# zrc0622/HIRL4UCAV

Hardware: AMD Instinct MI355X
Metric: env steps/sec (whole node) + HIRL update steps/sec at 4096 envs/GPU (higher is better)
Workload: dtype f32

## Files before the change

hirl4ucav_amd/_lib.py:

```python
import ctypes
import os

_HERE = os.path.dirname(os.path.abspath(__file__))
SO_PATH = os.environ.get("HX_LIBRARY") or os.path.join(_HERE, "libhx_mi355.so")

ENV_WORDS, OBS_DIM, ACT_DIM, ROW_WORDS = 37, 13, 4, 32
STAT_NAMES = ("episodes", "kills", "fire_success_episodes", "time_limit", "fires", "good_fires", "locked_steps", "env_steps", "nonfinite_actions")
STAT_WAYS, STAT_PITCH = 32, 16

F_LOCKED_PREV, F_LOCKED, F_SLOT_PREV, F_SLOT, F_FIRED, F_FIRE_SUCCESS, F_EPISODE_SUCCESS, F_DONE = (1 << i for i in range(8))
F_SCEN_SHIFT = 8
F_SERP_POS, F_SERP_LONG, F_M_ACTIVE, F_M_GUIDED, F_SIM_SLOT = (1 << i for i in range(10, 15))

_vp, _i32, _i64, _u32, _u64, _f32 = ctypes.c_void_p, ctypes.c_int32, ctypes.c_int64, ctypes.c_uint32, ctypes.c_uint64, ctypes.c_float


class HxStepOpts(ctypes.Structure):
    _fields_ = [("max_step", _i32), ("auto_reset", _i32), ("randomize", _i32), ("env_id0", _u32), ("seed", _u64),
                ("episode_ctr", _vp), ("ring", _vp), ("ring_success", _vp), ("cap", _i64), ("total", _vp), ("stats", _vp),
                ("ev_start", _vp), ("ev_stop", _vp), ("layout", _i32)]


LAYOUT_ORDERED_SLOTS = 1 << 16


def layout(pair, envs_per_block):
    return ((1 if pair else 0) << 8) | (int(envs_per_block) // 4)


class HxError(RuntimeError):
    pass


_SIGNATURES = {
    "hx_env_reset": [_vp, _i64, _i64, _vp, _vp, _i32, _i32, _u64, _u32, _vp, _vp, _vp],
    "hx_env_step": [_vp, _i64, _i64, _vp, _vp, _vp, _vp, _vp, ctypes.POINTER(HxStepOpts), _vp],
    "hx_env_rearm": [_vp, _i64, _i64, _vp, _vp],
    "hx_label_transitions": [_vp, _vp, _vp, _i64, _vp, _vp, _vp, _vp],
    "hx_event_destroy": [_vp],
    "hx_event_elapsed_us": [_vp, _vp, ctypes.POINTER(ctypes.c_float)],
}

_lib = None
ABI_VERSION = 117
_ABI_STRUCTS = {}


def check_struct(index, cls):
    sizes = (ctypes.c_int32 * 8)()
    L = load()
    L.hx_abi_sizes.argtypes = [ctypes.POINTER(ctypes.c_int32)]
    if L.hx_abi_sizes(sizes) != 0 or sizes[index] != ctypes.sizeof(cls):
        raise HxError(f"ABI mismatch: {cls.__name__} is {ctypes.sizeof(cls)} bytes here, {sizes[index]} in {SO_PATH}")
    if sizes[7] != STAT_WAYS * STAT_PITCH:
        raise HxError(f"ABI mismatch: a statistics buffer is {STAT_WAYS * STAT_PITCH} words here, {sizes[7]} in {SO_PATH}")


def load():
    global _lib
    if _lib is not None:
        return _lib
    if not os.path.exists(SO_PATH):
        raise HxError(f"{SO_PATH} not found: the HIP extension is not built (run __graft_entry__.build() or "
                      f"`make -C hirl4ucav_amd/csrc`). There is no CPU fallback.")
    import torch

    L = ctypes.CDLL(SO_PATH)
    L.hx_last_error.restype = ctypes.c_char_p
    L.hx_version.restype = ctypes.c_int
    if L.hx_version() != ABI_VERSION:
        raise HxError(f"{SO_PATH} implements ABI version {L.hx_version()}, this binding was written for {ABI_VERSION} (include/hirl4ucav.h "
                      f"HX_ABI_VERSION): rebuild the library (make -C hirl4ucav_amd/csrc)")
    L.hx_event_create.restype = ctypes.c_void_p
    L.hx_event_create.argtypes = []
    for name, args in _SIGNATURES.items():
        fn = getattr(L, name)
        fn.argtypes = args
        fn.restype = ctypes.c_int
    _lib = L
    return L


def register(name, argtypes):
    _SIGNATURES[name] = argtypes
    if _lib is not None:
        fn = getattr(_lib, name)
        fn.argtypes = argtypes
        fn.restype = ctypes.c_int


def call(name, *args):
    L = load()
    rc = getattr(L, name)(*args)
    if rc != 0:
        raise HxError(f"{name} failed ({rc}): {L.hx_last_error().decode()}")


def ptr(t):
    return None if t is None else t.data_ptr()


def stream_ptr():
    import torch

    return torch.cuda.current_stream().cuda_stream
```

hirl4ucav_amd/agents/engine.py:

```python
import ctypes
import os

import numpy as np
import torch

from .. import _lib

H1, H2 = 256, 512
_vp, _i32, _f32 = ctypes.c_void_p, ctypes.c_int32, ctypes.c_float


class HxBatch(ctypes.Structure):
    _fields_ = [("rows", _vp), ("bc_rows", _vp), ("batch", _i32), ("noise", _vp)]


class HxSample(ctypes.Structure):
    _fields_ = [("total", _vp), ("cap", ctypes.c_int64), ("ring", _vp), ("expert_ring", _vp), ("expert_len", ctypes.c_int64),
                ("bc_table", _vp), ("bc_len", ctypes.c_int64), ("n_main", _i32), ("seed", ctypes.c_uint64), ("call", ctypes.c_uint32),
                ("sigma", _f32), ("idx", _vp), ("idx_bc", _vp), ("guard", ctypes.c_uint32)]


class HxFront(ctypes.Structure):
    _fields_ = [("flags", _vp), ("status", _vp), ("epoch", ctypes.c_uint32), ("with_c", ctypes.c_uint32)]


class HxNets(ctypes.Structure):
    _fields_ = [(k, _vp) for k in ("actor", "critic", "target_actor", "target_critic", "bc_actor", "grad_actor", "grad_critic",
                                   "m_actor", "v_actor", "m_critic", "v_critic", "losses", "soft_count", "wstate", "ws", "actor_w2_bf16", "actor_w2_f32i",
                                   "w2_bf16_all", "xchg_status", "actor_w2_x9")]


class HxHyper(ctypes.Structure):
    _fields_ = [(k, _f32) for k in ("gamma", "tau", "lr_actor", "lr_critic", "slope", "noise_clamp", "loss_lambda")] + [("use_bc", _i32), ("no_layernorm", _i32)]


_P = ctypes.POINTER
_lib.register("hx_actor_act", [_vp, _vp, ctypes.c_int64, _vp, _i32, _vp, _f32, ctypes.c_uint64, ctypes.c_uint32, ctypes.c_uint32, _f32, _vp, _vp])
_lib.register("hx_actor_act_step", [_vp, _vp, ctypes.c_int64, ctypes.c_int64, _vp, _vp, _i32, _vp, _f32, ctypes.c_uint64, ctypes.c_uint32,
                                     ctypes.c_uint32, _f32, _vp, _vp, _vp, _P(_lib.HxStepOpts), _vp])
_lib.register("hx_pack_w2_bf16", [_vp, _i32, _vp, _vp])
_lib.register("hx_pack_w2_f32i", [_vp, _i32, _vp, _vp])
_lib.register("hx_pack_update_images", [_P(HxNets), _vp])
_lib.register("hx_pack_w2_x9", [_vp, _i32, _vp, _vp])
_lib.register("hx_actor_act_x9", [_vp, _vp, _vp, ctypes.c_int64, _vp, _i32, _vp, _f32, ctypes.c_uint64, ctypes.c_uint32, ctypes.c_uint32, _f32, _vp])
_lib.register("hx_actor_act_step_x9", [_vp, _vp, _vp, ctypes.c_int64, ctypes.c_int64, _vp, _vp, _i32, _vp, _f32, ctypes.c_uint64, ctypes.c_uint32,
                                        ctypes.c_uint32, _f32, _vp, _vp, _vp, _P(_lib.HxStepOpts), _vp])
_lib.register("hx_actor_act_f32i", [_vp, _vp, _vp, ctypes.c_int64, _vp, _i32, _vp, _f32, ctypes.c_uint64, ctypes.c_uint32, ctypes.c_uint32, _f32, _vp])
_lib.register("hx_actor_act_step_f32i", [_vp, _vp, _vp, ctypes.c_int64, ctypes.c_int64, _vp, _vp, _i32, _vp, _f32, ctypes.c_uint64, ctypes.c_uint32,
                                          ctypes.c_uint32, _f32, _vp, _vp, _vp, _P(_lib.HxStepOpts), _vp])
_lib.register("hx_actor_act_bf16", [_vp, _vp, _vp, ctypes.c_int64, _vp, _i32, _vp, _f32, ctypes.c_uint64, ctypes.c_uint32, ctypes.c_uint32, _f32, _vp])
_lib.register("hx_actor_act_step_bf16", [_vp, _vp, _vp, ctypes.c_int64, ctypes.c_int64, _vp, _vp, _i32, _vp, _f32, ctypes.c_uint64, ctypes.c_uint32,
                                          ctypes.c_uint32, _f32, _vp, _vp, _vp, _P(_lib.HxStepOpts), _vp])
_lib.register("hx_hirl_critic_grads", [_P(HxNets), _P(HxBatch), _P(HxHyper), _i32, _vp])
_lib.register("hx_hirl_actor_backward", [_P(HxNets), _P(HxBatch), _P(HxHyper), _i32, _i32, _vp])
_lib.register("hx_hirl_actor_wgrad", [_P(HxNets), _P(HxHyper), _i32, _i32, _i32, _f32, _f32, _vp])
_lib.register("hx_adam", [_P(HxNets), _P(HxHyper), _i32, _i32, _f32, _i32, _f32, _f32, _i32, _vp])
_lib.register("hx_polyak", [_P(HxNets), _P(HxHyper), _vp])
_lib.register("hx_hirl_actor_wgrad_split", [_P(HxNets), _P(HxHyper), _i32, _vp, _vp])
_lib.register("hx_adam_mixed", [_P(HxNets), _P(HxHyper), _i32, _i32, _f32, _i32, _f32, _f32, _i32, _vp, _vp])
from .exchange import OneShotExchange, RcclDirect, _DeviceWords, negotiate_rccl_direct


_lib.register("hx_bc_train_actor", [_P(HxNets), _P(HxBatch), _P(HxHyper), _i32, _vp])
_lib.register("hx_hirl_learn", [_P(HxNets), _P(HxBatch), _P(HxHyper), _i32, _i32, _i32, _i32, _i32, _f32, _f32, _vp])
_lib.register("hx_hirl_learn_sampled", [_P(HxNets), _P(HxBatch), _P(HxHyper), _P(HxSample), _i32, _i32, _i32, _i32, _i32, _f32, _f32, _vp])
_lib.register("hx_hirl_front", [_vp, ctypes.c_int64, ctypes.c_int64, _vp, _vp, _i32, _vp, _f32, ctypes.c_uint64, ctypes.c_uint32, ctypes.c_uint32, _vp, _vp, _vp,
                                 _P(_lib.HxStepOpts), _P(HxNets), _P(HxBatch), _P(HxHyper), _i32, _i32, _P(HxFront), _vp])
_lib.register("hx_hirl_learn_back", [_P(HxNets), _P(HxBatch), _P(HxHyper), _i32, _i32, _i32, _i32, _i32, _f32, _f32, _P(HxSample), _P(HxBatch), _i32, _vp])
_lib.register("hx_hirl_critic_grads_back", [_P(HxNets), _P(HxBatch), _P(HxHyper), _P(HxSample), _P(HxBatch), _i32, _vp])
_lib.register("hx_sample_batch_guarded", [_vp, ctypes.c_int64, _vp, _vp, ctypes.c_int64, _vp, ctypes.c_int64, _i32, _i32, _i32, ctypes.c_uint64,
                                           ctypes.c_uint32, _f32, _vp, _vp, _vp, _vp, _vp, ctypes.c_uint32, _vp])
_lib.register("hx_hirl_critic_grads_sampled", [_P(HxNets), _P(HxBatch), _P(HxHyper), _P(HxSample), _i32, _vp])
_lib.register("hx_sample_batch", [_vp, ctypes.c_int64, _vp, _vp, ctypes.c_int64, _vp, ctypes.c_int64, _i32, _i32, _i32, ctypes.c_uint64,
                                   ctypes.c_uint32, _f32, _vp, _vp, _vp, _vp, _vp, _vp])



def _block_layout(in_dim, out_dim, names):
    fa, la, fb, lb, fin = names
    shapes = [(fa + ".weight", (H1, in_dim)), (fa + ".bias", (H1,)), (la + ".weight", (H1,)), (la + ".bias", (H1,)),
              (fb + ".weight", (H2, H1)), (fb + ".bias", (H2,)), (lb + ".weight", (H2,)), (lb + ".bias", (H2,)),
              (fin + ".weight", (out_dim, H2)), (fin + ".bias", (out_dim,))]
    out, off = [], 0
    for k, shp in shapes:
        out.append((k, off, shp))
        off += int(np.prod(shp))
    return out, off


ACTOR_LAYOUT, ACTOR_SIZE = _block_layout(13, 4, ("full1", "layernorm1", "full2", "layernorm2", "final"))
_q1, _qsize = _block_layout(17, 1, ("full1", "layernorm1", "full2", "layernorm2", "final1"))
_q2, _ = _block_layout(17, 1, ("full3", "layernorm3", "full4", "layernorm4", "final2"))
Q_PADDED = (_qsize + 3) & ~3
CRITIC_LAYOUT = _q1 + [(k, off + Q_PADDED, shp) for k, off, shp in _q2]
CRITIC_SIZE = 2 * Q_PADDED


def pack(params, layout, size, device):
    flat = torch.zeros(size, dtype=torch.float32, device=device)
    for k, off, shp in layout:
        v = torch.as_tensor(np.asarray(params[k].detach().cpu() if torch.is_tensor(params[k]) else params[k]), dtype=torch.float32)
        assert tuple(v.shape) == tuple(shp), (k, v.shape, shp)
        flat[off:off + v.numel()] = v.reshape(-1).to(device)
    return flat


def unpack(flat, layout):
    return {k: flat[off:off + int(np.prod(shp))].reshape(shp) for k, off, shp in layout}


def force_plain_layernorm(flat, layout):
    for k, off, shp in layout:
        if k.startswith("layernorm"):
            flat[off:off + int(np.prod(shp))] = 1.0 if k.endswith(".weight") else 0.0


def len_of(replay):
    return 0 if replay is None else int(getattr(replay, "fixed_len", replay.capacity))


def carve(sizes, device):
    offs, tot = [], 0
    for n in sizes:
        offs.append(tot)
        tot += (n + 63) & ~63
    arena = torch.zeros(tot, dtype=torch.float32, device=device)
    return arena, [arena[o:o + n] for o, n in zip(offs, sizes)]


def _noise_mode(noise, sigma):
    if noise is not None:
        return 1 if noise.numel() == 4 else 2
    return 3 if sigma > 0 else 0


def _bc_weight_kind(bc_weight_now):
    if bc_weight_now is None:
        return 2, 0.0
    if bc_weight_now == 100:
        return 1, 0.0
    return 0, float(bc_weight_now)


class HirlEngine:
    def __init__(self, batch=128, lr_actor=1e-3, lr_critic=1e-3, tau=0.005, gamma=0.99, slope=0.0, use_bc=True,
                 device="cuda", group=None, layer_norm=True):
        self.device = torch.device(device)
        if self.device.type != "cuda":
            raise _lib.HxError("HirlEngine runs on the GPU only (no CPU path in the product)")
        L = _lib.load()
        for i, cls in ((0, _lib.HxStepOpts), (1, HxNets), (2, HxHyper), (3, HxBatch), (4, HxSample)):
            _lib.check_struct(i, cls)
        assert L.hx_actor_param_count() == ACTOR_SIZE and L.hx_critic_param_count() == CRITIC_SIZE
        L.hx_hirl_workspace_floats.restype = ctypes.c_int64
        self.batch = int(batch)
        ws_floats = int(L.hx_hirl_workspace_floats(self.batch))
        self.arena, views = carve([ACTOR_SIZE] * 3 + [CRITIC_SIZE] * 2 + [CRITIC_SIZE + ACTOR_SIZE] + [ACTOR_SIZE] * 2 + [CRITIC_SIZE] * 2 +
                                  [64, 64, 64, ws_floats, self.batch * 32, self.batch * 32, self.batch, self.batch, 64], self.device)
        (self.actor, self.target_actor, self.bc_actor, self.critic, self.target_critic, self.grad, self.m_actor, self.v_actor,
         self.m_critic, self.v_critic, self.losses, sc, self.wstate, self.ws, self.rows, self.bc_rows, ix, ixb, self._noise) = views
        self.grad_critic, self.grad_actor = self.grad[:CRITIC_SIZE], self.grad[CRITIC_SIZE:]
        self.soft_count, self._idx, self._idx_bc = sc.view(torch.int32), ix.view(torch.int32), ixb.view(torch.int32)
        self.losses, self.wstate, self._noise = self.losses[:8], self.wstate[:1], self._noise[:4]
        self.soft_count = self.soft_count[:1]
        self.sample_calls = 0
        self._pending = None
        self.front_c = False
        self._front = None
        self._front_enqueued = False
        self.needs_reload = False
        self._front_epoch = 0
        self._front_c_epoch = 0
        self._front_tiles = None
        self._front_drawn = None
        self.nets = HxNets(*(t.data_ptr() for t in (self.actor, self.critic, self.target_actor, self.target_critic, self.bc_actor,
                                                     self.grad_actor, self.grad_critic, self.m_actor, self.v_actor, self.m_critic,
                                                     self.v_critic, self.losses, self.soft_count, self.wstate, self.ws)), None, None, None, None, None)
        self.act_dtype, self.w2_bf16, self.w2_x9, self._x9_live = "f32", None, None, False
        self.x9_rows = 4096
        self.front_x9 = True
        self.update_dtype, self.images = "f32", None
        self.w2_f32i = torch.zeros(H2 * H1, dtype=torch.float32, device=self.device)
        self.nets.actor_w2_f32i = self.w2_f32i.data_ptr()
        self.layer_norm = bool(layer_norm)
        self._mode_bits = 0 if self.layer_norm else 16
        self.hyper = HxHyper(gamma, tau, lr_actor, lr_critic, slope, 0.5, 10000.0, int(use_bc), 0 if self.layer_norm else 1)
        self.use_bc, self.slope = bool(use_bc), float(slope)
        self.actor_trainable, self.update_count = True, 0
        self.critic_step, self.actor_step = 0, 0
        self.target_update_freq = 3
        self.group = group
        self.world = torch.distributed.get_world_size(group) if (torch.distributed.is_available() and torch.distributed.is_initialized()) else 1
        self.act_calls = 0
        self.staged = self.world > 1
        self.actor_msg = torch.zeros(int(L.hx_actor_message_floats()), dtype=torch.float32, device=self.device) if self.world > 1 else None
        self.sharded_sequence = False
        self.exchange_name, self.xchg, self.rccl = "rccl", None, None

    def load_params(self, actor, critic, bc_actor=None, hard_update_targets=True):
        self.actor.copy_(pack(actor, ACTOR_LAYOUT, ACTOR_SIZE, self.device))
        self.critic.copy_(pack(critic, CRITIC_LAYOUT, CRITIC_SIZE, self.device))
        if bc_actor is not None:
            self.bc_actor.copy_(pack(bc_actor, ACTOR_LAYOUT, ACTOR_SIZE, self.device))
        if not self.layer_norm:
            for flat, layout in ((self.actor, ACTOR_LAYOUT), (self.critic, CRITIC_LAYOUT), (self.bc_actor, ACTOR_LAYOUT)):
                force_plain_layernorm(flat, layout)
        if hard_update_targets:
            self.target_actor.copy_(self.actor)
            self.target_critic.copy_(self.critic)
        self.refresh_bf16()

    def set_act_dtype(self, dtype):
        if dtype not in ("f32", "bf16", "f32x9"):
            raise ValueError(dtype)
        if dtype == "f32x9" and self.update_dtype != "f32":
            raise ValueError("act dtype f32x9 goes with the fp32 update path")
        self.act_dtype = dtype
        self._bind_images()
        self.refresh_bf16()

    def set_update_dtype(self, dtype):
        if dtype not in ("f32", "bf16"):
            raise ValueError(dtype)
        if dtype == "bf16" and self.act_dtype == "f32x9":
            raise ValueError("act dtype f32x9 goes with the fp32 update path")
        self.update_dtype = dtype
        self._bind_images()
        self.refresh_bf16()

    def _bind_images(self):
        self.nets.actor_w2_x9 = None
        self._x9_live = False
        if self.update_dtype == "bf16":
            if self.images is None:
                L = _lib.load()
                L.hx_bf16_images_elems.restype = ctypes.c_int64
                self.images = torch.zeros(int(L.hx_bf16_images_elems()), dtype=torch.bfloat16, device=self.device)
            self.nets.w2_bf16_all = self.images.data_ptr()
            self.w2_bf16 = self.images[:H2 * H1]
            self.nets.actor_w2_bf16 = self.w2_bf16.data_ptr() if self.act_dtype == "bf16" else None
            return
        self.nets.w2_bf16_all = None
        if self.act_dtype == "f32x9":
            if self.w2_x9 is None:
                self.w2_x9 = torch.zeros(3 * H2 * H1, dtype=torch.bfloat16, device=self.device)
            self.nets.actor_w2_x9 = self.w2_x9.data_ptr()
            self.nets.actor_w2_bf16 = None
            return
        if self.act_dtype == "bf16":
            if self.w2_bf16 is None or (self.images is not None and self.w2_bf16.data_ptr() == self.images.data_ptr()):
                self.w2_bf16 = torch.zeros(H2 * H1, dtype=torch.bfloat16, device=self.device)
            self.nets.actor_w2_bf16 = self.w2_bf16.data_ptr()
        else:
            self.nets.actor_w2_bf16 = None

    def refresh_bf16(self):
        _lib.call("hx_pack_w2_f32i", self.actor.data_ptr(), 13, self.w2_f32i.data_ptr(), _lib.stream_ptr())
        if self.update_dtype == "bf16":
            _lib.call("hx_pack_update_images", ctypes.byref(self.nets), _lib.stream_ptr())
        elif self.act_dtype == "bf16":
            _lib.call("hx_pack_w2_bf16", self.actor.data_ptr(), 13, self.w2_bf16.data_ptr(), _lib.stream_ptr())
        elif self.act_dtype == "f32x9" or (self.act_dtype == "f32" and self._x9_live):
            _lib.call("hx_pack_w2_x9", self.actor.data_ptr(), 13, self.w2_x9.data_ptr(), _lib.stream_ptr())

    def _x9_for(self, n, front=False):
        if self.act_dtype == "f32x9":
            return True
        if self.act_dtype != "f32" or self.update_dtype != "f32":
            return False
        if not (front and self.front_x9) and (self.x9_rows is None or n < self.x9_rows):
            return False
        if not self._x9_live:
            if self.w2_x9 is None:
                self.w2_x9 = torch.zeros(3 * H2 * H1, dtype=torch.bfloat16, device=self.device)
            self.nets.actor_w2_x9 = self.w2_x9.data_ptr()
            _lib.call("hx_pack_w2_x9", self.actor.data_ptr(), 13, self.w2_x9.data_ptr(), _lib.stream_ptr())
            self._x9_live = True
        return True

    def _act_format(self, n):
        if self.act_dtype == "bf16":
            return "_bf16", self.w2_bf16.data_ptr()
        if self._x9_for(n):
            return "_x9", self.w2_x9.data_ptr()
        return "_f32i", self.w2_f32i.data_ptr()

    refresh_images = refresh_bf16

    def acting_format(self):
        return {"act_dtype": self.act_dtype, "update_dtype": self.update_dtype, "x9_rows": self.x9_rows, "front_x9": bool(self.front_x9), "x9_terms": 6}

    def replica_checksum(self):
        if self.xchg is not None:
            self.xchg.check()
        t = torch.cat([self.actor, self.target_actor, self.critic, self.target_critic, self.m_actor, self.v_actor, self.m_critic, self.v_critic])
        return int(t.view(torch.int32).to(torch.int64).sum().item())

    def close(self):
        if self.rccl is not None:
            r, self.rccl = self.rccl, None
            r.close()
        if self.xchg is not None:
            x, self.xchg = self.xchg, None
            self.nets.xchg_status = None
            try:
                x.check()
            finally:
                x.close()

    def state_dicts(self):
        return {"actor": unpack(self.actor, ACTOR_LAYOUT), "critic": unpack(self.critic, CRITIC_LAYOUT),
                "targetActor": unpack(self.target_actor, ACTOR_LAYOUT), "targetCritic": unpack(self.target_critic, CRITIC_LAYOUT),
                "bc_actor": unpack(self.bc_actor, ACTOR_LAYOUT)}

    def act(self, obs, noise=None, sigma=0.0, seed=0, row0=0, out=None, net=None):
        n = obs.shape[0]
        if out is None:
            out = torch.empty((n, 4), dtype=torch.float32, device=self.device)
        mode = _noise_mode(noise, sigma) | self._mode_bits
        self.act_calls += 1
        if net is None:
            fmt, image = self._act_format(n)
            _lib.call("hx_actor_act" + fmt, self.actor.data_ptr(), image, obs.data_ptr(), n, out.data_ptr(), mode, _lib.ptr(noise), float(sigma), int(seed),
                      int(row0), self.act_calls, self.slope, _lib.stream_ptr())
            return out
        _lib.call("hx_actor_act", net.data_ptr(), obs.data_ptr(), n, out.data_ptr(), mode, _lib.ptr(noise), float(sigma), int(seed), int(row0), self.act_calls,
                  self.slope, None, _lib.stream_ptr())
        return out

    def act_step(self, env, noise=None, sigma=0.0, seed=0, out=None):
        n = env.n
        if out is None:
            out = torch.empty((n, 4), dtype=torch.float32, device=self.device)
        mode = _noise_mode(noise, sigma) | self._mode_bits
        self.act_calls += 1
        env.steps_issued += 1
        fmt, image = self._act_format(n)
        _lib.call("hx_actor_act_step" + fmt, self.actor.data_ptr(), image, env.state.data_ptr(), n, env.pitch, env.obs.data_ptr(), out.data_ptr(), mode,
                  _lib.ptr(noise), float(sigma), int(seed), int(env.env_id0), self.act_calls, self.slope, env.reward.data_ptr(), env.done.data_ptr(),
                  env.success.data_ptr(), ctypes.byref(env._opts), _lib.stream_ptr())
        return out, env.obs, env.reward, env.done, env.success

    def use_oneshot_exchange(self, timeout_ms=5000, two_stage=False, bf16=False):
        if self.world <= 1:
            return
        self.xchg = OneShotExchange({"critic": CRITIC_SIZE, "actor": self.actor_msg.numel()}, self.device, self.group, timeout_ms, two_stage, bf16)
        self.nets.xchg_status = self.xchg.status_ptr
        self.exchange_name = "oneshot" if not two_stage else ("twostage-bf16" if bf16 else "twostage")

    def use_rccl_direct(self, bf16=False):
        dist = torch.distributed
        if not (dist.is_available() and dist.is_initialized()):
            raise _lib.HxError("use_rccl_direct needs an initialised torch.distributed process group (it carries the communicator id)")
        import sys

        def connect(uid, world, rank):
            r = RcclDirect(uid, world, rank, bf16=bf16)
            r.probe(self.device)
            return r

        r, _why = negotiate_rccl_direct(self.group, self.device if dist.get_backend(self.group) == "nccl" else "cpu", connect=connect,
                                        log=lambda m: print(m, file=sys.stderr, flush=True))
        if r is None:
            return False
        self.rccl = r
        self.exchange_name = "rccl-direct-bf16" if bf16 else "rccl-direct"
        return True

    def _allreduce(self, t, kind=None):
        if self.world <= 1 and not (self.sharded_sequence and torch.distributed.is_available() and torch.distributed.is_initialized()):
            return t
        if self.xchg is not None and kind is not None:
            return self.xchg.allreduce(kind)
        if self.rccl is not None:
            return self.rccl.allreduce(t)
        torch.distributed.all_reduce(t, group=self.group)
        return t

    def assemble(self, ring, idx, expert_ring=None, n_main=None, bc_table=None, idx_bc=None):
        B = self.batch
        n_main = B if n_main is None else int(n_main)
        _lib.call("hx_sample_batch", None, 0, ring.data_ptr(), _lib.ptr(expert_ring), 0, _lib.ptr(bc_table), 0, B, n_main, 0, 0, 0, 0.0,
                  idx.data_ptr(), _lib.ptr(idx_bc), None, self.rows.data_ptr(), self.bc_rows.data_ptr() if bc_table is not None else None,
                  _lib.stream_ptr())

    def sample(self, replay, expert=None, bc_table=None, n_main=None, seed=0, sigma=0.2, defer=False):
        B = self.batch
        self.sample_calls += 1
        if defer:
            self._pending = (HxSample(replay.total.data_ptr(), replay.capacity, replay.ring.data_ptr(),
                                      expert.ring.data_ptr() if expert is not None else None, len_of(expert), _lib.ptr(bc_table),
                                      bc_table.shape[0] if bc_table is not None else 0, B if n_main is None else int(n_main), int(seed),
                                      self.sample_calls, float(sigma), self._idx.data_ptr(),
                                      self._idx_bc.data_ptr() if bc_table is not None else None), replay, expert, bc_table)
            return self._idx, self._idx_bc, self._noise
        self._pending = None
        _lib.call("hx_sample_batch", replay.total.data_ptr(), replay.capacity, replay.ring.data_ptr(),
                  expert.ring.data_ptr() if expert is not None else None, len_of(expert), _lib.ptr(bc_table),
                  bc_table.shape[0] if bc_table is not None else 0, B, B if n_main is None else int(n_main), 1, int(seed),
                  self.sample_calls, float(sigma), self._idx.data_ptr(), self._idx_bc.data_ptr() if bc_table is not None else None,
                  self._noise.data_ptr(), self.rows.data_ptr(), self.bc_rows.data_ptr() if bc_table is not None else None, _lib.stream_ptr())
        return self._idx, self._idx_bc, self._noise

    def learn(self, noise=None, bc_weight_now=0.0, bc_warm_up_weight=0.0, before_exchange=None):
        B = self.batch
        if self.needs_reload:
            raise _lib.HxError("this engine failed after a front launch had been enqueued: load a snapshot before learn()")
        st = _lib.stream_ptr()
        pending, self._pending = self._pending, None
        pipe = getattr(before_exchange, "__self__", None) if before_exchange is not None else None
        if pending is not None and pipe is not None and (getattr(pipe, "_armed", None) is not None or getattr(pipe, "issued", False)):
            raise _lib.HxError("sample(defer=True) cannot be combined with an armed VectorStepPipeline: use sample(defer=False) when the "
                               "next env step may run beside learn()")
        if pending is not None and noise is not None:
            raise _lib.HxError("learn(noise=...) after sample(defer=True): the deferred draw produces the smoothing noise itself")
        noise = self._noise if noise is None else noise
        batch = HxBatch(self.rows.data_ptr(), self.bc_rows.data_ptr() if self.use_bc else None, B, noise.data_ptr())
        smp = ctypes.byref(pending[0]) if pending is not None else None
        nets, hyper = ctypes.byref(self.nets), ctypes.byref(self.hyper)
        w_kind, w_given = _bc_weight_kind(bc_weight_now)
        actor_phase = self.actor_trainable
        self.critic_step += 1
        if actor_phase:
            self.actor_step += 1
            self.update_count += 1
        do_polyak = actor_phase and self.update_count % self.target_update_freq == 0
        if not self.staged:
            _lib.call("hx_hirl_learn_sampled", nets, ctypes.byref(batch), hyper, smp, self.critic_step, int(actor_phase), self.actor_step,
                      int(do_polyak), w_kind, w_given, float(bc_warm_up_weight), st)
        else:
            actor_fwd = (2 if w_kind == 1 else 1) if actor_phase else 0
            if smp is not None:
                grads = lambda: _lib.call("hx_hirl_critic_grads_sampled", nets, ctypes.byref(batch), hyper, smp, actor_fwd, st)
            else:
                grads = lambda: _lib.call("hx_hirl_critic_grads", nets, ctypes.byref(batch), hyper, actor_fwd, st)
            self._learn_staged(grads, batch, actor_phase, do_polyak, w_kind, w_given, bc_warm_up_weight, before_exchange)
        self.actor_trainable = not self.actor_trainable

    def _learn_staged(self, critic_grads, batch, actor_phase, do_polyak, w_kind, w_given, bc_warm_up_weight, before_exchange=None):
        B, st = self.batch, _lib.stream_ptr()
        nets, hyper = ctypes.byref(self.nets), ctypes.byref(self.hyper)
        gs = 1.0 / self.world
        own_critic = self.grad_critic.data_ptr()
        if self.xchg is not None:
            self.nets.grad_critic = self.xchg.write_buffer("critic").data_ptr()
        critic_grads()
        if before_exchange is not None:
            before_exchange()
        summed = self._allreduce(self.grad_critic, "critic")
        self.nets.grad_critic = summed.data_ptr()
        pk = 16 if do_polyak else 0
        _lib.call("hx_adam", nets, hyper, 0 | pk, self.critic_step, gs, 0, 0.0, 0.0, B, st)
        self.nets.grad_critic = own_critic
        if actor_phase:
            _lib.call("hx_hirl_actor_backward", nets, ctypes.byref(batch), hyper, int(w_kind == 1), 1, st)
            if self.world > 1 or self.sharded_sequence:
                if self.actor_msg is None:
                    self.actor_msg = torch.zeros(int(_lib.load().hx_actor_message_floats()), dtype=torch.float32, device=self.device)
                msg = self.xchg.write_buffer("actor") if self.xchg is not None else self.actor_msg
                _lib.call("hx_hirl_actor_wgrad_split", nets, hyper, B, msg.data_ptr(), st)
                summed = self._allreduce(msg, "actor")
                _lib.call("hx_adam_mixed", nets, hyper, int(do_polyak), self.actor_step, gs, w_kind, w_given, float(bc_warm_up_weight),
                          B * self.world, summed.data_ptr(), st)
            else:
                _lib.call("hx_hirl_actor_wgrad", nets, hyper, B, B, w_kind, w_given, float(bc_warm_up_weight), st)
                _lib.call("hx_adam", nets, hyper, 1 | pk, self.actor_step, gs, w_kind, w_given, float(bc_warm_up_weight), B, st)

    def step_learn(self, env, expert=None, bc_table=None, n_main=None, act_noise=None, act_sigma=0.0, act_seed=0, out=None, sample_seed=0,
                   smooth_sigma=0.2, bc_weight_now=0.0, bc_warm_up_weight=0.0):
        replay, n, B = env.replay, env.n, self.batch
        bf16 = self.update_dtype == "bf16"
        if replay is None or (self.act_dtype != "bf16" if bf16 else self.act_dtype not in ("f32", "f32x9")):
            raise _lib.HxError("step_learn: the front launch exists for the fp32 networks (acting format 'f32' or 'f32x9') and for the bf16 update path with "
                               "the bf16 acting format, with a replay ring attached to the env")
        if self._pending is not None:
            raise _lib.HxError("step_learn draws its own minibatch: a sample(defer=True) is still pending")
        if self._front is None:
            buf = torch.zeros(96, dtype=torch.int32, device=self.device)
            self._front = (buf[0:64], buf[64:65])
            second = torch.zeros(2 * B * 32 + 2 * B + 64, dtype=torch.float32, device=self.device)
            t2 = (second[:B * 32], second[B * 32:2 * B * 32], second[2 * B * 32:2 * B * 32 + B].view(torch.int32),
                  second[2 * B * 32 + B:2 * B * 32 + 2 * B].view(torch.int32), second[2 * B * 32 + 2 * B:2 * B * 32 + 2 * B + 4])
            self._front_tiles = [(self.rows, self.bc_rows, self._idx, self._idx_bc, self._noise), t2]
        flags, status = self._front
        cur, nxt = self._front_tiles
        n_main = B if n_main is None else int(n_main)
        if self.needs_reload:
            raise _lib.HxError("this engine failed after a front launch had been enqueued (host and device state may disagree): load a snapshot "
                               "(utils/checkpoint.load_run) before stepping it again")
        held = (self._front_epoch, self._front_c_epoch, self.critic_step, self.actor_step, self.update_count, self.sample_calls, self.act_calls, env.steps_issued)
        self._front_enqueued = False
        try:
            return self._step_learn(env, expert, bc_table, n_main, act_noise, act_sigma, act_seed, out, sample_seed, smooth_sigma, bc_weight_now,
                                    bc_warm_up_weight, bf16, flags, status, cur, nxt)
        except _lib.HxError:
            if self._front_enqueued:
                self.needs_reload = True
                raise
            (self._front_epoch, self._front_c_epoch, self.critic_step, self.actor_step, self.update_count, self.sample_calls, self.act_calls, env.steps_issued) = held
            self.front_reset()
            raise

    def _step_learn(self, env, expert, bc_table, n_main, act_noise, act_sigma, act_seed, out, sample_seed, smooth_sigma, bc_weight_now, bc_warm_up_weight,
                    bf16, flags, status, cur, nxt):
        replay, n, B = env.replay, env.n, self.batch
        self.sample_calls += 1

        def draw(tiles, call):
            return HxSample(replay.total.data_ptr(), replay.capacity, replay.ring.data_ptr(), expert.ring.data_ptr() if expert is not None else None,
                            len_of(expert), _lib.ptr(bc_table), bc_table.shape[0] if bc_table is not None else 0, n_main, int(sample_seed), call,
                            float(smooth_sigma), tiles[2].data_ptr(), tiles[3].data_ptr() if bc_table is not None else None, n)

        def tiles_of(t):
            return HxBatch(t[0].data_ptr(), t[1].data_ptr() if self.use_bc else None, B, t[4].data_ptr())

        want = (env, env.steps_issued, replay, expert, bc_table, n_main, int(sample_seed), float(smooth_sigma), self.sample_calls, n)
        if self._front_drawn != want:
            _lib.call("hx_sample_batch_guarded", replay.total.data_ptr(), replay.capacity, replay.ring.data_ptr(), expert.ring.data_ptr() if expert is not None else None,
                      len_of(expert), _lib.ptr(bc_table), bc_table.shape[0] if bc_table is not None else 0, B, n_main, 1, int(sample_seed), self.sample_calls,
                      float(smooth_sigma), cur[2].data_ptr(), cur[3].data_ptr() if bc_table is not None else None, cur[4].data_ptr(), cur[0].data_ptr(),
                      cur[1].data_ptr() if bc_table is not None else None, n, _lib.stream_ptr())
        if out is None:
            out = torch.empty((n, 4), dtype=torch.float32, device=self.device)
        mode = _noise_mode(act_noise, act_sigma) | self._mode_bits
        self.act_calls += 1
        if self._front_epoch >= 200_000_000:
            flags.zero_()
            self._front_epoch = self._front_c_epoch = 0
        self._front_epoch += 1
        batch, nets, hyper, st = tiles_of(cur), ctypes.byref(self.nets), ctypes.byref(self.hyper), _lib.stream_ptr()
        w_kind, w_given = _bc_weight_kind(bc_weight_now)
        actor_phase = self.actor_trainable
        self.critic_step += 1
        if actor_phase:
            self.actor_step += 1
            self.update_count += 1
        do_polyak = actor_phase and self.update_count % self.target_update_freq == 0
        with_c = int(self.front_c_for(n, actor_phase, w_kind, bf16))
        knob = os.environ.get("HX_FRONT_C")
        carries_c = knob == "1" or (bool(with_c) and knob != "0")
        if carries_c:
            self._front_c_epoch += 1
        front = HxFront(flags.data_ptr(), status.data_ptr(), self._front_epoch, self._front_c_epoch if carries_c else 0)
        _lib.call("hx_hirl_front", env.state.data_ptr(), n, env.pitch, env.obs.data_ptr(), out.data_ptr(), mode | (32 if (not bf16 and self._x9_for(n, front=True)) else 0),
                  _lib.ptr(act_noise), float(act_sigma), int(act_seed), int(env.env_id0), self.act_calls, env.reward.data_ptr(), env.done.data_ptr(),
                  env.success.data_ptr(), ctypes.byref(env._opts), nets, ctypes.byref(batch), hyper, int(actor_phase), w_kind, ctypes.byref(front), st)
        self._front_enqueued = True
        env.steps_issued += 1
        nxt_draw, nxt_tiles = draw(nxt, self.sample_calls + 1), tiles_of(nxt)
        if not self.staged:
            _lib.call("hx_hirl_learn_back", nets, ctypes.byref(batch), hyper, self.critic_step, int(actor_phase), self.actor_step, int(do_polyak), w_kind, w_given,
                      float(bc_warm_up_weight), ctypes.byref(nxt_draw), ctypes.byref(nxt_tiles), with_c, st)
        else:
            self._learn_staged(lambda: _lib.call("hx_hirl_critic_grads_back", nets, ctypes.byref(batch), hyper, ctypes.byref(nxt_draw), ctypes.byref(nxt_tiles), with_c, st),
                               batch, actor_phase, do_polyak, w_kind, w_given, bc_warm_up_weight)
        self._front_drawn = (env, env.steps_issued, replay, expert, bc_table, n_main, int(sample_seed), float(smooth_sigma), self.sample_calls + 1, n)
        self._front_tiles = [nxt, cur]
        self.rows, self.bc_rows, self._idx, self._idx_bc, self._noise = cur
        self.actor_trainable = not self.actor_trainable
        return out, env.obs, env.reward, env.done, env.success

    @staticmethod
    def front_waiting_workgroups(batch, with_c=False):
        tiles = (int(batch) + 15) // 16
        return 2 * tiles * 8 + (2 * ((int(batch) + 7) // 8) * 8 if with_c else 0)

    def front_c_for(self, n, actor_phase, w_kind, bf16):
        if self.front_c != "auto":
            return bool(self.front_c)
        if bf16 or not self._x9_for(n, front=True) or n < 8192 or n > 16384:
            return False
        acting = (n + 63) // 64
        jobs = (3 + 2) + (1 + (0 if not self.use_bc else (2 if w_kind == 1 else 1)))
        tiles = (self.batch + 15) // 16
        need = jobs * tiles * 8 * 6.0 + 2 * ((self.batch + 7) // 8) * 8 * 7.6
        return (256 - acting) * 37.0 >= need

    def front_reset(self):
        if self._front is not None:
            self._front[0].zero_()
            self._front[1].zero_()
        self._front_epoch = self._front_c_epoch = 0
        self._front_drawn = None

    def front_status(self):
        return 0 if self._front is None else int(self._front[1].item())

    def front_check(self):
        code = self.front_status()
        if code != 0:
            which = [w for bit, w in ((1, "launch B for the target actor's rows (launch A)"), (2, "launch C for the rows of launches A / B")) if code & bit]
            raise _lib.HxError(f"front launch: an in-launch wait timed out (status word {code}: " + "; ".join(which) + ") - the minibatches read since are "
                               "suspect; the reference-order loop (train_all --loop reference) has no in-launch waits")

    def bc_train_actor(self):
        batch = HxBatch(self.rows.data_ptr(), self.bc_rows.data_ptr(), self.batch, self._noise.data_ptr())
        self.actor_step += 1
        _lib.call("hx_bc_train_actor", ctypes.byref(self.nets), ctypes.byref(batch), ctypes.byref(self.hyper), self.actor_step, _lib.stream_ptr())

    def losses_host(self):
        v = self.losses.tolist()
        return v[0], v[1], v[2], v[3], v[4], v[5]
```

hirl4ucav_amd/csrc/hx_core.hip:

```cpp
#include "hx_common.h"

namespace hx {
char* error_buffer() {
    static thread_local char buf[512] = "";
    return buf;
}
}

__global__ void calib_copy_dword(const float* __restrict__ src, float* __restrict__ dst, long long n) {
    const long long i = (long long)blockIdx.x * blockDim.x + threadIdx.x;
    if (i < n) dst[i] = src[i];
}

extern "C" {
int hx_debug_stamps(float* host_out) {
#ifdef HX_STAMPS
    if (hipDeviceSynchronize() != hipSuccess) return -2;
    for (int i = 0; i < 80; ++i) host_out[i] = 0.0f;
    if (int rc = hx::dbg_stamps_fwdbwd(host_out)) return rc;
    if (int rc = hx::dbg_stamps_wgrad(host_out)) return rc;
    return hx::dbg_stamps_act(host_out);
#else
    (void)host_out;
    return -1;
#endif
}
int hx_debug_stamps_actp(float* host_out) {
#ifdef HX_STAMPS
    if (hipDeviceSynchronize() != hipSuccess) return -2;
    for (int i = 0; i < 80; ++i) host_out[i] = 0.0f;
    return hx::dbg_stamps_actp(host_out);
#else
    (void)host_out;
    return -1;
#endif
}
int hx_debug_stamps_front(float* host_out) {
#ifdef HX_STAMPS
    if (hipDeviceSynchronize() != hipSuccess) return -2;
    for (int i = 0; i < 80; ++i) host_out[i] = 0.0f;
    return hx::dbg_stamps_front(host_out);
#else
    (void)host_out;
    return -1;
#endif
}
int hx_debug_spans(unsigned long long* host_spans , unsigned* host_tags , unsigned* host_n) {
#ifdef HX_STAMPS
    if (hipDeviceSynchronize() != hipSuccess) return -2;
    *host_n = 0;
    if (int rc = hx::dbg_spans_fwdbwd(host_spans, host_tags, host_n, 8192u)) return rc;
    if (int rc = hx::dbg_spans_wgrad(host_spans, host_tags, host_n, 8192u)) return rc;
    if (int rc = hx::dbg_spans_front(host_spans, host_tags, host_n, 8192u)) return rc;
    return hx::dbg_spans_act(host_spans, host_tags, host_n, 8192u);
#else
    (void)host_spans; (void)host_tags; (void)host_n;
    return -1;
#endif
}
int hx_debug_copy_dword(const float* src, float* dst, int64_t n, void* stream) {
    HX_REQUIRE(src && dst && n > 0, "hx_debug_copy_dword: bad arguments");
    hipLaunchKernelGGL(calib_copy_dword, dim3((unsigned)((n + 255) / 256)), dim3(256), 0, (hipStream_t)stream, src, dst, (long long)n);
    HX_CHECK_LAUNCH("hx_debug_copy_dword");
    return 0;
}
void* hx_event_create(void) {
    hipEvent_t e = nullptr;
    if (hipEventCreate(&e) != hipSuccess) {
        hx::fail(HX_ERR_ARG, "hx_event_create: hipEventCreate failed");
        return nullptr;
    }
    return (void*)e;
}
int hx_event_destroy(void* ev) {
    HX_REQUIRE(ev, "hx_event_destroy: null event");
    HX_REQUIRE(hipEventDestroy((hipEvent_t)ev) == hipSuccess, "hx_event_destroy: hipEventDestroy failed");
    return 0;
}
int hx_event_elapsed_us(void* start, void* stop, float* us) {
    HX_REQUIRE(start && stop && us, "hx_event_elapsed_us: bad arguments");
    float ms = 0.0f;
    HX_REQUIRE(hipEventElapsedTime(&ms, (hipEvent_t)start, (hipEvent_t)stop) == hipSuccess, "hx_event_elapsed_us: events not complete");
    *us = ms * 1000.0f;
    return 0;
}
const char* hx_last_error(void) { return hx::error_buffer(); }
int hx_version(void) { return HX_ABI_VERSION; }
int hx_abi_sizes(int32_t* sizes8) {
    HX_REQUIRE(sizes8, "hx_abi_sizes: null");
    const int32_t v[8] = {(int32_t)sizeof(HxStepOpts), (int32_t)sizeof(HxNets), (int32_t)sizeof(HxHyper), (int32_t)sizeof(HxBatch), (int32_t)sizeof(HxSample),
                          (int32_t)sizeof(HxSacNets), (int32_t)sizeof(HxSacBatch), HX_STAT_WAYS * HX_STAT_PITCH};
    for (int i = 0; i < 8; ++i) sizes8[i] = v[i];
    return 0;
}
}
```

hirl4ucav_amd/csrc/hx_hirl.hip:

```cpp
#include <cmath>

#include "hx_act.h"

using namespace hxnn;
using namespace hxu;

extern "C" {

int hx_actor_param_count(void) { return kActor.size(); }
int hx_critic_param_count(void) { return 2 * kQ.padded(); }
int64_t hx_hirl_workspace_floats(int32_t batch) { return (int64_t)S_COUNT * kSlotFloats * batch + 64; }
int64_t hx_actor_message_floats(void) { return 2 * (int64_t)kActor.padded() + 64; }
int64_t hx_bf16_images_elems(void) { return (int64_t)IM_COUNT * (int64_t)kImgElems; }

int hx_pack_update_images(const HxNets* N, void* stream) {
    HX_REQUIRE(N && N->w2_bf16_all && (reinterpret_cast<uintptr_t>(N->w2_bf16_all) & 15u) == 0, "hx_pack_update_images: w2_bf16_all must be a 16-byte aligned buffer");
    HX_REQUIRE(N->actor && N->critic && N->target_actor && N->target_critic, "hx_pack_update_images: null network");
    hipStream_t st = (hipStream_t)stream;
    uint16_t* im = N->w2_bf16_all;
    launch_pack_bf16(N->actor + kActor.W2(), im + IM_ACTOR * kImgElems, false, st);
    launch_pack_bf16(N->actor + kActor.W2(), im + IM_ACTOR_T * kImgElems, true, st);
    launch_pack_bf16(N->target_actor + kActor.W2(), im + IM_TA * kImgElems, false, st);
    if (N->bc_actor) launch_pack_bf16(N->bc_actor + kActor.W2(), im + IM_BC * kImgElems, false, st);
    for (int h = 0; h < 2; ++h) {
        launch_pack_bf16(N->critic + h * kQ.padded() + kQ.W2(), im + (IM_C1 + h) * kImgElems, false, st);
        launch_pack_bf16(N->critic + h * kQ.padded() + kQ.W2(), im + (IM_C1_T + h) * kImgElems, true, st);
        launch_pack_bf16(N->target_critic + h * kQ.padded() + kQ.W2(), im + (IM_TC1 + h) * kImgElems, false, st);
    }
    HX_CHECK_LAUNCH("hx_pack_update_images");
    return 0;
}

static void make_slots(const HxNets* N, int B, Slot* s) {
    for (int i = 0; i < S_COUNT; ++i) s[i] = carve_slot(N->ws + (size_t)i * kSlotFloats * B, B);
}

static WgAdam make_adam(const HxNets* N, const HxHyper* Hy, float lr, int step, bool finish_actor) {
    WgAdam a{};
    set_adam_scalars(a, lr, step);
    a.tau = Hy->tau;
    a.finish_actor = finish_actor ? 1 : 0;
    a.use_bc = Hy->use_bc;
    a.losses = N->losses;
    a.wstate = N->wstate;
    return a;
}

static void make_launch_a(const HxNets* N, const HxBatch* Bt, const HxHyper* Hy, int32_t actor_fwd, FwdArgs& F) {
    const Mlp mA{13, 4, Hy->no_layernorm ? 1 : 0}, mQ{17, 1, Hy->no_layernorm ? 1 : 0};
    const int B = Bt->batch;
    Slot s[S_COUNT];
    make_slots(N, B, s);
    const RowSrc src{Bt->rows, nullptr, nullptr, 0, 32};
    F = FwdArgs{};
    F.njobs = 3; F.slope = Hy->slope;
    F.zero_f = N->losses; F.zero_nf = 1;
    F.job[0] = FwdJob{N->target_actor, mA, src, 17, 0, Head{}, nullptr, 0.f, s[S_TA], B, 0, IM_TA};
    F.job[1] = FwdJob{N->critic, mQ, src, 0, 0, Head{}, nullptr, 0.f, s[S_C1], B, 1, IM_C1};
    F.job[2] = FwdJob{N->critic + mQ.padded(), mQ, src, 0, 0, Head{}, nullptr, 0.f, s[S_C2], B, 1, IM_C2};
    if (actor_fwd) {
        F.zero_nf = 5; F.zero_i = N->soft_count;
        F.job[3] = FwdJob{N->actor, mA, src, 0, 0, Head{}, nullptr, 0.f, s[S_API], B, 1, IM_ACTOR};
        F.njobs = 4;
    }
    F.images = N->w2_bf16_all;
}
static void make_launch_b(const HxNets* N, const HxBatch* Bt, const HxHyper* Hy, int32_t actor_fwd, FwdArgs& F) {
    const Mlp mA{13, 4, Hy->no_layernorm ? 1 : 0}, mQ{17, 1, Hy->no_layernorm ? 1 : 0};
    const int B = Bt->batch;
    Slot s[S_COUNT];
    make_slots(N, B, s);
    const RowSrc src{Bt->rows, nullptr, nullptr, 0, 32};
    const float* tc1 = N->target_critic;
    const float* tc2 = N->target_critic + mQ.padded();
    F = FwdArgs{};
    F.njobs = 2; F.slope = Hy->slope;
    const Head prev{N->target_actor, mA, s[S_TA]};
    F.job[0] = FwdJob{tc1, mQ, src, 17, 1, prev, Bt->noise, Hy->noise_clamp, s[S_TC1], B, 0, IM_TC1};
    F.job[1] = FwdJob{tc2, mQ, src, 17, 1, prev, Bt->noise, Hy->noise_clamp, s[S_TC2], B, 0, IM_TC2};
    if (actor_fwd && Hy->use_bc) {
        const RowSrc bcsrc{Bt->bc_rows ? Bt->bc_rows : Bt->rows, nullptr, nullptr, 0, 32};
        int n = 2;
        F.job[n++] = FwdJob{N->actor, mA, bcsrc, 0, 0, Head{}, nullptr, 0.f, s[S_ABC], B, 1, IM_ACTOR};
        if (actor_fwd == 2) F.job[n++] = FwdJob{N->bc_actor, mA, src, 0, 0, Head{}, nullptr, 0.f, s[S_BCS], B, 0, IM_BC};
        F.njobs = n;
    }
    F.images = N->w2_bf16_all;
}
static void make_launch_c(const HxNets* N, const HxBatch* Bt, const HxHyper* Hy, BwdArgs& G) {
    const Mlp mQ{17, 1, Hy->no_layernorm ? 1 : 0};
    const int B = Bt->batch;
    Slot s[S_COUNT];
    make_slots(N, B, s);
    const RowSrc src{Bt->rows, nullptr, nullptr, 0, 32};
    const float* tc1 = N->target_critic;
    const float* tc2 = N->target_critic + mQ.padded();
    G = BwdArgs{};
    G.njobs = 2; G.slope = Hy->slope; G.inv_batch = 1.0f / B; G.losses = N->losses; G.soft_count = N->soft_count;
    for (int h = 0; h < 2; ++h) {
        BwdJob& J = G.job[h];
        J = BwdJob{};
        J.net = N->critic + h * mQ.padded(); J.m = mQ; J.ws = s[S_C1 + h]; J.rows = B; J.mode = BM_CRITIC_TD;
        J.t1 = Head{tc1, mQ, s[S_TC1]}; J.t2 = Head{tc2, mQ, s[S_TC2]}; J.src = src; J.gamma = Hy->gamma;
        J.img_t = IM_C1_T + h;
    }
    G.images = N->w2_bf16_all;
}
static bool front_has_c(bool asked) {
    static const int force = getenv("HX_FRONT_C") ? atoi(getenv("HX_FRONT_C")) : -1;
    return force < 0 ? asked : force != 0;
}
static int critic_back(const HxNets* N, const HxBatch* Bt, const HxHyper* Hy, void* stream, int adam_step, bool polyak, const SampleDev* predraw = nullptr, bool skip_c = false) {
    hipStream_t st = (hipStream_t)stream;
    const Mlp mQ{17, 1, Hy->no_layernorm ? 1 : 0};
    const int B = Bt->batch;
    Slot s[S_COUNT];
    make_slots(N, B, s);
    if (!skip_c) {
        BwdArgs G;
        make_launch_c(N, Bt, Hy, G);
        launch_bwd(0, G, st);
    }
    {
        WgArgs W{};
        W.njobs = 2; W.slope = Hy->slope; W.w_kind = 0; W.w_given = 0.f; W.inv_batch = 1.0f / B;
        W.soft_count = N->soft_count; W.wstate = N->wstate;
        for (int h = 0; h < 2; ++h) {
            WgJob& J = W.job[h];
            J = WgJob{};
            J.net = N->critic + h * mQ.padded(); J.grad = N->grad_critic + h * mQ.padded(); J.m = mQ;
            J.ws[0] = s[S_C1 + h]; J.rows[0] = B; J.nslots = 1; J.wmode[0] = 0;
            if (adam_step > 0) {
                J.p = N->critic + h * mQ.padded();
                J.mom = N->m_critic + h * mQ.padded(); J.var = N->v_critic + h * mQ.padded();
                J.target = polyak ? N->target_critic + h * mQ.padded() : nullptr;
                if (uint16_t* im = N->w2_bf16_all) {
                    J.w2b = im + (IM_C1 + h) * kImgElems; J.w2tb = im + (IM_C1_T + h) * kImgElems; J.tgt_w2b = im + (IM_TC1 + h) * kImgElems;
                }
            }
        }
        W.bf16 = N->w2_bf16_all != nullptr;
        W.predraw = predraw; W.predraw_batch = B;
        if (adam_step > 0) {
            W.ad = make_adam(N, Hy, Hy->lr_critic, adam_step, false);
            launch_wg(W, true, st);
        } else {
            launch_wg(W, false, st);
        }
    }
    HX_CHECK_LAUNCH("hx_hirl_critic_grads");
    return 0;
}
static int critic_grads_impl(const HxNets* N, const HxBatch* Bt, const HxHyper* Hy, int32_t actor_fwd, void* stream, int adam_step, bool polyak,
                             const HxSample* S = nullptr) {
    HX_REQUIRE(N && Bt && Hy && Bt->batch > 0 && Bt->batch % 16 == 0, "hx_hirl_critic_grads: batch must be a positive multiple of 16");
    hipStream_t st = (hipStream_t)stream;
    const int B = Bt->batch;
    SampleDev SD{};
    bool fused = false;
    if (S) {
        HX_REQUIRE(Bt->noise, "hx_hirl_*_sampled: the draw needs the output word noise[4]");
        if (int rc = prepare_draw(S, B, const_cast<float*>(Bt->rows), const_cast<float*>(Bt->bc_rows), const_cast<float*>(Bt->noise), stream, &SD, &fused)) return rc;
    }
    FwdArgs F;
    make_launch_a(N, Bt, Hy, actor_fwd, F);
    F.sample = fused ? &SD : nullptr;
    launch_fwd(F, st);
    make_launch_b(N, Bt, Hy, actor_fwd, F);
    launch_fwd(F, st);
    return critic_back(N, Bt, Hy, stream, adam_step, polyak);
}
int hx_hirl_critic_grads(const HxNets* N, const HxBatch* Bt, const HxHyper* Hy, int32_t actor_fwd, void* stream) {
    return critic_grads_impl(N, Bt, Hy, actor_fwd, stream, 0, false);
}
int hx_hirl_critic_grads_sampled(const HxNets* N, const HxBatch* Bt, const HxHyper* Hy, const HxSample* S, int32_t actor_fwd, void* stream) {
    HX_REQUIRE(S, "hx_hirl_critic_grads_sampled: null sample description");
    return critic_grads_impl(N, Bt, Hy, actor_fwd, stream, 0, false, S);
}

int hx_hirl_actor_backward(const HxNets* N, const HxBatch* Bt, const HxHyper* Hy, int32_t estimate_soft, int32_t fwd_done, void* stream) {
    HX_REQUIRE(N && Bt && Hy && Bt->batch > 0 && Bt->batch % 16 == 0, "hx_hirl_actor_backward: batch must be a positive multiple of 16");
    hipStream_t st = (hipStream_t)stream;
    const Mlp mA{13, 4, Hy->no_layernorm ? 1 : 0}, mQ{17, 1, Hy->no_layernorm ? 1 : 0};
    (void)mA; (void)mQ;
    const int B = Bt->batch;
    Slot s[S_COUNT];
    make_slots(N, B, s);
    const RowSrc src{Bt->rows, nullptr, nullptr, 0, 32};
    const RowSrc bcsrc{Bt->bc_rows ? Bt->bc_rows : Bt->rows, nullptr, nullptr, 0, 32};
    const bool bc = Hy->use_bc != 0, soft = bc && estimate_soft;
    if (!fwd_done) {
        FwdArgs F{};
        F.slope = Hy->slope;
        F.zero_f = N->losses + 1; F.zero_nf = 4; F.zero_i = N->soft_count;
        int n = 0;
        F.job[n++] = FwdJob{N->actor, mA, src, 0, 0, Head{}, nullptr, 0.f, s[S_API], B, 1, IM_ACTOR};
        if (bc) F.job[n++] = FwdJob{N->actor, mA, bcsrc, 0, 0, Head{}, nullptr, 0.f, s[S_ABC], B, 1, IM_ACTOR};
        if (soft) F.job[n++] = FwdJob{N->bc_actor, mA, src, 0, 0, Head{}, nullptr, 0.f, s[S_BCS], B, 0, IM_BC};
        F.njobs = n;
        F.images = N->w2_bf16_all;
        launch_fwd(F, st);
    }
    {
        FwdArgs F{};
        F.slope = Hy->slope;
        int n = 0;
        F.job[n++] = FwdJob{N->critic, mQ, src, 0, 1, Head{N->actor, mA, s[S_API]}, nullptr, 0.f, s[S_CPI], B, 1, IM_C1};
        if (soft) F.job[n++] = FwdJob{N->critic, mQ, src, 0, 1, Head{N->bc_actor, mA, s[S_BCS]}, nullptr, 0.f, s[S_CSOFT], B, 0, IM_C1};
        F.njobs = n;
        F.images = N->w2_bf16_all;
        launch_fwd(F, st);
    }
    {
        BwdArgs G{};
        G.njobs = 1; G.slope = Hy->slope; G.inv_batch = 1.0f / B; G.losses = N->losses; G.soft_count = N->soft_count;
        BwdJob& J = G.job[0];
        J = BwdJob{};
        J.net = N->critic; J.m = mQ; J.ws = s[S_CPI]; J.rows = B; J.mode = BM_CRITIC_PI;
        if (soft) J.soft = Head{N->critic, mQ, s[S_CSOFT]};
        J.img_t = IM_C1_T;
        G.images = N->w2_bf16_all;
        launch_bwd(1, G, st);
    }
    {
        BwdArgs G{};
        G.slope = Hy->slope; G.inv_batch = 1.0f / B; G.losses = N->losses; G.soft_count = N->soft_count;
        int n = 0;
        {
            BwdJob& J = G.job[n++];
            J = BwdJob{};
            J.net = N->actor; J.m = mA; J.ws = s[S_API]; J.rows = B; J.mode = BM_ACTOR_PI;
            J.crit = Head{N->critic, mQ, s[S_CPI]};
            J.img_t = IM_ACTOR_T;
        }
        if (bc) {
            BwdJob& J = G.job[n++];
            J = BwdJob{};
            J.net = N->actor; J.m = mA; J.ws = s[S_ABC]; J.rows = B; J.mode = BM_ACTOR_BC;
            J.src = bcsrc; J.lambda = Hy->loss_lambda;
            J.img_t = IM_ACTOR_T;
        }
        G.njobs = n;
        G.images = N->w2_bf16_all;
        launch_bwd(2, G, st);
    }
    HX_CHECK_LAUNCH("hx_hirl_actor_backward");
    return 0;
}

static int actor_wgrad_impl(const HxNets* N, const HxHyper* Hy, int32_t batch, int32_t count_batch, int32_t w_kind, float w_given,
                            float warm, void* stream, int adam_step, bool polyak) {
    HX_REQUIRE(N && Hy && batch > 0 && count_batch > 0, "hx_hirl_actor_wgrad: bad arguments");
    const Mlp mA{13, 4, Hy->no_layernorm ? 1 : 0}, mQ{17, 1, Hy->no_layernorm ? 1 : 0};
    (void)mA; (void)mQ;
    Slot s[S_COUNT];
    make_slots(N, batch, s);
    const bool bc = Hy->use_bc != 0;
    WgArgs W{};
    W.njobs = 1; W.slope = Hy->slope; W.w_kind = bc ? w_kind : 0; W.w_given = bc ? w_given : 0.0f; W.warm = warm;
    W.inv_batch = 1.0f / count_batch; W.soft_count = N->soft_count; W.wstate = N->wstate;
    WgJob& J = W.job[0];
    J = WgJob{};
    J.net = N->actor; J.grad = N->grad_actor; J.m = mA;
    J.ws[0] = s[S_API]; J.rows[0] = batch; J.wmode[0] = 1;
    J.nslots = 1;
    if (bc) { J.ws[1] = s[S_ABC]; J.rows[1] = batch; J.wmode[1] = 2; J.nslots = 2; }
    W.bf16 = N->w2_bf16_all != nullptr;
    if (adam_step > 0) {
        J.p = N->actor; J.mom = N->m_actor; J.var = N->v_actor;
        J.target = polyak ? N->target_actor : nullptr;
        J.w2b = N->actor_w2_bf16;
        J.w2f = N->actor_w2_f32i;
        if (N->actor_w2_x9) {
            HX_REQUIRE(!N->actor_w2_bf16 && !N->w2_bf16_all, "hx_hirl_learn: actor_w2_x9 excludes the plain bf16 images (one acting format at a time)");
            J.w2b = N->actor_w2_x9; J.w2b_x9 = 1;
        }
        if (uint16_t* im = N->w2_bf16_all) {
            HX_REQUIRE(!N->actor_w2_bf16 || N->actor_w2_bf16 == im + IM_ACTOR * kImgElems, "hx_hirl_learn: with w2_bf16_all set, actor_w2_bf16 must be NULL or its first image");
            J.w2b = im + IM_ACTOR * kImgElems; J.w2tb = im + IM_ACTOR_T * kImgElems; J.tgt_w2b = im + IM_TA * kImgElems;
        }
        W.ad = make_adam(N, Hy, Hy->lr_actor, adam_step, true);
        launch_wg(W, true, (hipStream_t)stream);
    } else {
        launch_wg(W, false, (hipStream_t)stream);
    }
    HX_CHECK_LAUNCH("hx_hirl_actor_wgrad");
    return 0;
}
int hx_hirl_actor_wgrad(const HxNets* N, const HxHyper* Hy, int32_t batch, int32_t count_batch, int32_t w_kind, float w_given,
                        float warm, void* stream) {
    return actor_wgrad_impl(N, Hy, batch, count_batch, w_kind, w_given, warm, stream, 0, false);
}

int hx_hirl_actor_wgrad_split(const HxNets* N, const HxHyper* Hy, int32_t batch, float* msg, void* stream) {
    HX_REQUIRE(N && Hy && batch > 0 && msg && (reinterpret_cast<uintptr_t>(msg) & 15u) == 0, "hx_hirl_actor_wgrad_split: bad arguments");
    const Mlp mA{13, 4, Hy->no_layernorm ? 1 : 0}, mQ{17, 1, Hy->no_layernorm ? 1 : 0};
    (void)mA; (void)mQ;
    Slot s[S_COUNT];
    make_slots(N, batch, s);
    const bool bc = Hy->use_bc != 0;
    WgArgs W{};
    W.njobs = bc ? 2 : 1; W.slope = Hy->slope; W.w_kind = 0; W.w_given = 0.0f; W.inv_batch = 1.0f / batch;
    W.soft_count = N->soft_count; W.wstate = N->wstate;
    for (int j = 0; j < W.njobs; ++j) {
        WgJob& J = W.job[j];
        J = WgJob{};
        J.net = N->actor; J.grad = msg + j * mA.padded(); J.m = mA;
        J.ws[0] = s[j == 0 ? S_API : S_ABC]; J.rows[0] = batch; J.wmode[0] = 0; J.nslots = 1;
    }
    W.bf16 = N->w2_bf16_all != nullptr;
    W.soft_count = bc ? N->soft_count : nullptr;
    W.count_out = msg + 2 * mA.padded();
    launch_wg(W, false, (hipStream_t)stream);
    HX_CHECK_LAUNCH("hx_hirl_actor_wgrad_split");
    return 0;
}

int hx_hirl_learn(const HxNets* N, const HxBatch* Bt, const HxHyper* Hy, int32_t critic_step, int32_t actor_phase,
                  int32_t actor_step, int32_t do_polyak, int32_t w_kind, float w_given, float warm, void* stream) {
    return hx_hirl_learn_sampled(N, Bt, Hy, nullptr, critic_step, actor_phase, actor_step, do_polyak, w_kind, w_given, warm, stream);
}
int hx_hirl_learn_sampled(const HxNets* N, const HxBatch* Bt, const HxHyper* Hy, const HxSample* S, int32_t critic_step, int32_t actor_phase,
                          int32_t actor_step, int32_t do_polyak, int32_t w_kind, float w_given, float warm, void* stream) {
    HX_REQUIRE(critic_step >= 1 && (!actor_phase || actor_step >= 1), "hx_hirl_learn: Adam steps are 1-based");
    int rc = critic_grads_impl(N, Bt, Hy, actor_phase ? (w_kind == 1 ? 2 : 1) : 0, stream, critic_step, do_polyak != 0, S);
    if (rc || !actor_phase) return rc;
    if ((rc = hx_hirl_actor_backward(N, Bt, Hy, w_kind == 1, 1, stream))) return rc;
    return actor_wgrad_impl(N, Hy, Bt->batch, Bt->batch, w_kind, w_given, warm, stream, actor_step, do_polyak != 0);
}

int hx_hirl_front(float* state, int64_t n, int64_t stride, float* obs_io, float* actions, int32_t noise_mode, const float* noise,
                  float sigma, uint64_t seed, uint32_t row0, uint32_t call, float* reward, uint8_t* done, int8_t* success, const HxStepOpts* opts,
                  const HxNets* N, const HxBatch* Bt, const HxHyper* Hy, int32_t actor_phase, int32_t w_kind, const HxFront* front, void* stream) {
    HX_REQUIRE(N && Bt && Hy && front && opts && Bt->batch > 0 && Bt->batch % 16 == 0 && Bt->batch <= kFusedBatchMax && Bt->rows && Bt->noise,
               "hx_hirl_front: the minibatch tiles (a positive multiple of 16 rows, at most 256) and noise[4] must be there");
    HX_REQUIRE(front->flags && front->status && front->epoch >= 1, "hx_hirl_front: flags, status and a 1-based epoch are required");
    const bool bf16 = N->w2_bf16_all != nullptr;
    HX_REQUIRE(bf16 ? N->actor_w2_bf16 != nullptr : (!N->actor_w2_bf16 && (N->actor_w2_f32i || N->actor_w2_x9)),
               "hx_hirl_front: fp32 networks with HxNets.actor_w2_f32i / actor_w2_x9, or the bf16 update path (w2_bf16_all) with actor_w2_bf16");
    const int actor_fwd = actor_phase ? (w_kind == 1 ? 2 : 1) : 0;
    FwdArgs FA, FB;
    make_launch_a(N, Bt, Hy, actor_fwd, FA);
    make_launch_b(N, Bt, Hy, actor_fwd, FB);
    const bool x9 = !bf16 && (noise_mode & 32) != 0;
    HX_REQUIRE(bf16 || (x9 ? N->actor_w2_x9 != nullptr : N->actor_w2_f32i != nullptr), "hx_hirl_front: the image of the chosen acting format is missing from HxNets");
    noise_mode &= ~32;
    BwdArgs GC;
    const bool with_c = front_has_c(front->with_c != 0);
    HX_REQUIRE(!with_c || front->with_c != 0, "hx_hirl_front: HX_FRONT_C=1 needs a caller that counts its launches with launch C (HxFront.with_c = 1, 2, ...)");
    if (with_c) make_launch_c(N, Bt, Hy, GC);
    if (int rc = hxact::check_noise_mode(noise_mode, noise, "hx_hirl_front")) return rc;
    const hxact::ActEnv E{state, stride, reward, done, success, *opts};
    if (int rc = hxact::check_step_args(obs_io, n, actions, E, "hx_hirl_front")) return rc;
    const hxact::ActImages im{(x9 || bf16) ? nullptr : N->actor_w2_f32i, x9 ? N->actor_w2_x9 : nullptr, bf16 ? N->actor_w2_bf16 : nullptr};
    return launch_front(hxact::act_args_det(N->actor, obs_io, n, actions, noise_mode, noise, sigma, seed, row0, call, Hy->slope, im, &E), FA, FB, with_c ? &GC : nullptr,
                        *front, (hipStream_t)stream);
}
static int make_predraw(const HxNets* N, const HxBatch* Bt, const HxSample* next, const HxBatch* next_tiles, void* stream, SampleDev* SD) {
    HX_REQUIRE(next_tiles && next_tiles->batch == Bt->batch && next_tiles->rows && next_tiles->noise && next_tiles->rows != Bt->rows && next_tiles->noise != Bt->noise,
               "hx_hirl_learn_back: the next minibatch needs tiles of its own (this call still reads the current ones)");
    (void)N;
    bool fused = false;
    if (int rc = prepare_draw(next, Bt->batch, const_cast<float*>(next_tiles->rows), const_cast<float*>(next_tiles->bc_rows), const_cast<float*>(next_tiles->noise),
                              stream, SD, &fused, false)) return rc;
    HX_REQUIRE(fused, "hx_hirl_learn_back: the predraw covers minibatches of at most 256 rows");
    return 0;
}
int hx_hirl_critic_grads_back(const HxNets* N, const HxBatch* Bt, const HxHyper* Hy, const HxSample* next, const HxBatch* next_tiles, int32_t c_in_front,
                              void* stream) {
    HX_REQUIRE(N && Bt && Hy && Bt->batch > 0 && Bt->batch % 16 == 0, "hx_hirl_critic_grads_back: batch must be a positive multiple of 16");
    SampleDev SD{};
    if (next) if (int rc = make_predraw(N, Bt, next, next_tiles, stream, &SD)) return rc;
    return critic_back(N, Bt, Hy, stream, 0, false, next ? &SD : nullptr, front_has_c(c_in_front != 0));
}
int hx_hirl_learn_back(const HxNets* N, const HxBatch* Bt, const HxHyper* Hy, int32_t critic_step, int32_t actor_phase, int32_t actor_step, int32_t do_polyak,
                       int32_t w_kind, float w_given, float warm, const HxSample* next, const HxBatch* next_tiles, int32_t c_in_front, void* stream) {
    HX_REQUIRE(N && Bt && Hy && Bt->batch > 0 && Bt->batch % 16 == 0, "hx_hirl_learn_back: batch must be a positive multiple of 16");
    HX_REQUIRE(critic_step >= 1 && (!actor_phase || actor_step >= 1), "hx_hirl_learn_back: Adam steps are 1-based");
    SampleDev SD{};
    if (next) if (int rc = make_predraw(N, Bt, next, next_tiles, stream, &SD)) return rc;
    int rc = critic_back(N, Bt, Hy, stream, critic_step, do_polyak != 0, next ? &SD : nullptr, front_has_c(c_in_front != 0));
    if (rc || !actor_phase) return rc;
    if ((rc = hx_hirl_actor_backward(N, Bt, Hy, w_kind == 1, 1, stream))) return rc;
    return actor_wgrad_impl(N, Hy, Bt->batch, Bt->batch, w_kind, w_given, warm, stream, actor_step, do_polyak != 0);
}

int hx_bc_train_actor(const HxNets* N, const HxBatch* Bt, const HxHyper* Hy, int32_t step, void* stream) {
    HX_REQUIRE(N && Bt && Hy && Bt->bc_rows && Bt->batch > 0 && Bt->batch % 16 == 0 && step >= 1, "hx_bc_train_actor: bad arguments");
    hipStream_t st = (hipStream_t)stream;
    const Mlp mA{13, 4, Hy->no_layernorm ? 1 : 0}, mQ{17, 1, Hy->no_layernorm ? 1 : 0};
    (void)mA; (void)mQ;
    const int B = Bt->batch;
    Slot s[S_COUNT];
    make_slots(N, B, s);
    const RowSrc bcsrc{Bt->bc_rows, nullptr, nullptr, 0, 32};
    {
        FwdArgs F{};
        F.njobs = 1; F.slope = Hy->slope;
        F.zero_f = N->losses + 1; F.zero_nf = 4;
        F.job[0] = FwdJob{N->actor, mA, bcsrc, 0, 0, Head{}, nullptr, 0.f, s[S_ABC], B, 1, IM_ACTOR};
        F.images = N->w2_bf16_all;
        launch_fwd(F, st);
    }
    {
        BwdArgs G{};
        G.njobs = 1; G.slope = Hy->slope; G.inv_batch = 1.0f / B; G.losses = N->losses; G.soft_count = N->soft_count;
        BwdJob& J = G.job[0];
        J = BwdJob{};
        J.net = N->actor; J.m = mA; J.ws = s[S_ABC]; J.rows = B; J.mode = BM_ACTOR_BC; J.src = bcsrc; J.lambda = 1.0f;
        J.img_t = IM_ACTOR_T;
        G.images = N->w2_bf16_all;
        launch_bwd(2, G, st);
    }
    {
        WgArgs W{};
        W.njobs = 1; W.slope = Hy->slope; W.w_kind = 0; W.w_given = 0.f; W.inv_batch = 1.0f / B;
        W.soft_count = N->soft_count; W.wstate = N->wstate;
        WgJob& J = W.job[0];
        J = WgJob{};
        J.net = N->actor; J.grad = N->grad_actor; J.m = mA; J.ws[0] = s[S_ABC]; J.rows[0] = B; J.nslots = 1; J.wmode[0] = 0;
        W.bf16 = N->w2_bf16_all != nullptr;
        launch_wg(W, false, st);
    }
    HX_CHECK_LAUNCH("hx_bc_train_actor");
    return hx_adam(N, Hy, 2, step, 1.0f, 0, 0.0f, 0.0f, B, stream);
}

}
```

hirl4ucav_amd/csrc/hx_update.h:

```cpp
#pragma once
#include <cmath>
#include <cstdlib>
#include <type_traits>

#include "hx_common.h"
#include "hx_nn.h"

#ifdef HX_STAMPS
static __device__ float hx_dbg[80];
#define STAMP_DECL unsigned long long TS_[16]; int tsn_ = 0
#define STAMP() TS_[tsn_++] = __builtin_amdgcn_s_memrealtime()
#define STAMP_FLUSH(base, cond) do { if (cond) { for (int i_ = 1; i_ < tsn_; ++i_) hx_dbg[(base) + i_] = (float)(TS_[i_] - TS_[i_ - 1]); hx_dbg[(base)] = (float)tsn_; } } while (0)
constexpr int kSpanCap = 8192;
static __device__ unsigned long long hx_span[kSpanCap][2];
static __device__ unsigned hx_span_tag[kSpanCap];
static __device__ unsigned hx_span_n;
#define SPAN_LOG(tag) do { if (threadIdx.x == 0) { const unsigned long long e_ = __builtin_amdgcn_s_memrealtime(); const unsigned i_ = atomicAdd(&hx_span_n, 1u); \
    if (i_ < (unsigned)kSpanCap) { hx_span[i_][0] = TS_[0]; hx_span[i_][1] = e_; hx_span_tag[i_] = (unsigned)(tag) | (blockIdx.x << 8) | (blockIdx.y << 24); } } } while (0)
#define HX_DEFINE_DEBUG_COLLECTORS(name, lo, hi) \
    namespace hx { \
    int dbg_stamps_##name(float* host80) { \
        float tmp[80]; \
        if (hipMemcpyFromSymbol(tmp, HIP_SYMBOL(hx_dbg), sizeof(tmp)) != hipSuccess) return -2; \
        for (int i = (lo); i < (hi); ++i) host80[i] = tmp[i]; \
        return 0; \
    } \
    int dbg_spans_##name(unsigned long long* spans, unsigned* tags, unsigned* n, unsigned cap) { \
        unsigned k = 0, zero = 0u; \
        if (hipMemcpyFromSymbol(&k, HIP_SYMBOL(hx_span_n), sizeof(unsigned)) != hipSuccess) return -2; \
        if (k > (unsigned)kSpanCap) k = kSpanCap; \
        if (k > cap - *n) k = cap - *n; \
        if (k && hipMemcpyFromSymbol(spans + 2 * (size_t)*n, HIP_SYMBOL(hx_span), sizeof(unsigned long long) * 2 * k) != hipSuccess) return -2; \
        if (k && hipMemcpyFromSymbol(tags + *n, HIP_SYMBOL(hx_span_tag), sizeof(unsigned) * k) != hipSuccess) return -2; \
        *n += k; \
        return hipMemcpyToSymbol(HIP_SYMBOL(hx_span_n), &zero, sizeof(unsigned)) == hipSuccess ? 0 : -2; \
    } \
    }
#else
#define STAMP_DECL
#define STAMP()
#define STAMP_FLUSH(base, cond)
#define SPAN_LOG(tag)
#define HX_DEFINE_DEBUG_COLLECTORS(name, lo, hi)
#endif
enum { HX_SPAN_FWD = 1, HX_SPAN_ACT = 2, HX_SPAN_BWD = 3, HX_SPAN_WGRAD = 4, HX_SPAN_FRONT_A = 5, HX_SPAN_FRONT_B = 6 };

namespace hxu {
using namespace hxnn;

constexpr int kThreads = 256;
constexpr int kWide = 1024;
constexpr int kNT = 64;
constexpr int kNTB = 32, kCTB = kNTB / 16, kKSB = 16 / kCTB, kColWgB = H1 / kNTB;
constexpr int OW = 8;

struct RowSrc {
    const float* main;
    const float* exp;
    const int* idx;
    int nb;
    int pitch;
};
__device__ __forceinline__ const float* src_row(const RowSrc& s, int r) {
    if (!s.idx) return s.main + (size_t)r * s.pitch;
    const int i = s.idx[r];
    return (r < s.nb ? s.main : s.exp) + (size_t)i * s.pitch;
}

struct Slot {
    float* x;
    float* z1;
    float* st1;
    float* h1;
    float* z2;
    float* st2;
    float* outv;
    float* dz2;
    float* dh1;
    float* dout;
    float* lnp;
};

__host__ __device__ inline Slot carve_slot(float* base, int rows) {
    Slot s;
    float* p = base;
    s.x = p; p += (size_t)rows * XP;
    s.z1 = p; p += (size_t)rows * H1;
    s.st1 = p; p += (size_t)rows * 2;
    s.h1 = p; p += (size_t)rows * H1;
    s.z2 = p; p += (size_t)rows * H2;
    s.st2 = p; p += (size_t)rows * 2;
    s.outv = p; p += (size_t)rows * OW;
    s.dz2 = p; p += (size_t)rows * H2;
    s.dh1 = p; p += (size_t)rows * H1;
    s.dout = p; p += (size_t)rows * OW;
    s.lnp = p; p += (size_t)rows * (2 * kColWgB);
    return s;
}
__host__ __device__ inline uint32_t mlp_bits(const Mlp& m) { return (uint32_t)m.in | ((uint32_t)m.out << 5) | ((uint32_t)(m.no_ln ? 1 : 0) << 9); }
__host__ __device__ inline Mlp mlp_of(uint32_t b) { return Mlp{(int)(b & 31u), (int)((b >> 5) & 15u), (int)((b >> 9) & 1u)}; }

struct Head {
    const float* net;
    Mlp m;
    Slot ws;
};

__device__ __forceinline__ float ld_agent(const float* p) { return __hip_atomic_load(p, __ATOMIC_RELAXED, __HIP_MEMORY_SCOPE_AGENT); }
__device__ __forceinline__ void st_agent(float* p, float v) { __hip_atomic_store(p, v, __ATOMIC_RELAXED, __HIP_MEMORY_SCOPE_AGENT); }

template <int N>
struct RowReg {
    static constexpr int PER4 = N / 256;
    float v[PER4 * 4];
    __device__ __forceinline__ void load(const float* __restrict__ p) {
        const int lane = threadIdx.x & 63;
#pragma unroll
        for (int i = 0; i < PER4; ++i) {
            const float4 t = reinterpret_cast<const float4*>(p)[i * 64 + lane];
            v[4 * i] = t.x; v[4 * i + 1] = t.y; v[4 * i + 2] = t.z; v[4 * i + 3] = t.w;
        }
    }
    __device__ __forceinline__ void load_agent(const float* p) {
        const int lane = threadIdx.x & 63;
#pragma unroll
        for (int i = 0; i < PER4; ++i)
#pragma unroll
            for (int c = 0; c < 4; ++c) v[4 * i + c] = ld_agent(p + (i * 64 + lane) * 4 + c);
    }
    __device__ __forceinline__ void store(float* __restrict__ p) const {
        const int lane = threadIdx.x & 63;
#pragma unroll
        for (int i = 0; i < PER4; ++i) reinterpret_cast<float4*>(p)[i * 64 + lane] = make_float4(v[4 * i], v[4 * i + 1], v[4 * i + 2], v[4 * i + 3]);
    }
    __device__ __forceinline__ void store_lds(float* p) const { store(p); }
};

template <int OUTMAX, bool RELU, bool AGENT = false>
__device__ __forceinline__ void head_row(const float* __restrict__ z2row, const float* __restrict__ net, const Mlp m, float slope,
                                         RowReg<H2>& xhat, RowReg<H2>& y, float& mean, float& rstd, float (&o)[OUTMAX]) {
    RowReg<H2> z, g, be;
    if (AGENT) z.load_agent(z2row);
    else z.load(z2row);
    row_stats<8>(z.v, H2, mean, rstd);
    if (m.no_ln) { mean = 0.0f; rstd = 1.0f; }
    g.load(net + m.g2());
    be.load(net + m.be2());
#pragma unroll
    for (int i = 0; i < 8; ++i) {
        xhat.v[i] = (z.v[i] - mean) * rstd;
        y.v[i] = g.v[i] * xhat.v[i] + be.v[i];
    }
#pragma unroll
    for (int j = 0; j < OUTMAX; ++j) {
        float acc = 0.0f;
        if (j < m.out) {
            RowReg<H2> w;
            w.load(net + m.W3() + j * H2);
#pragma unroll
            for (int i = 0; i < 8; ++i) acc += act_f<RELU>(y.v[i], slope) * w.v[i];
            acc = wave_sum(acc) + net[m.b3() + j];
        }
        o[j] = acc;
    }
}

template <bool RELU, bool AGENT = false>
__device__ __forceinline__ void head_row4(const float* __restrict__ z2row, const float* __restrict__ net, const Mlp m, float slope,
                                          RowReg<H2>& xhat, RowReg<H2>& y, float& mean, float& rstd, float (&o)[4]) {
    RowReg<H2> z, g, be, w0, w1, w2, w3;
    if (AGENT) z.load_agent(z2row);
    else z.load(z2row);
    g.load(net + m.g2());
    be.load(net + m.be2());
    w0.load(net + m.W3());
    w1.load(net + m.W3() + H2);
    w2.load(net + m.W3() + 2 * H2);
    w3.load(net + m.W3() + 3 * H2);
    const int lane = threadIdx.x & 63;
    const float b3 = net[m.b3() + (lane & 3)];
    row_stats<8>(z.v, H2, mean, rstd);
    if (m.no_ln) { mean = 0.0f; rstd = 1.0f; }
    float a0 = 0.f, a1 = 0.f, a2 = 0.f, a3 = 0.f;
#pragma unroll
    for (int i = 0; i < 8; ++i) {
        xhat.v[i] = (z.v[i] - mean) * rstd;
        y.v[i] = g.v[i] * xhat.v[i] + be.v[i];
    }
#pragma unroll
    for (int i = 0; i < 8; ++i) a0 += act_f<RELU>(y.v[i], slope) * w0.v[i];
#pragma unroll
    for (int i = 0; i < 8; ++i) a1 += act_f<RELU>(y.v[i], slope) * w1.v[i];
#pragma unroll
    for (int i = 0; i < 8; ++i) a2 += act_f<RELU>(y.v[i], slope) * w2.v[i];
#pragma unroll
    for (int i = 0; i < 8; ++i) a3 += act_f<RELU>(y.v[i], slope) * w3.v[i];
    o[0] = wave_sum(a0) + __shfl(b3, 0);
    o[1] = wave_sum(a1) + __shfl(b3, 1);
    o[2] = wave_sum(a2) + __shfl(b3, 2);
    o[3] = wave_sum(a3) + __shfl(b3, 3);
}

__device__ __forceinline__ void philox4x32_10(uint32_t c0, uint32_t c1, uint32_t c2, uint32_t c3, uint32_t k0, uint32_t k1, uint32_t out[4]) {
#pragma unroll
    for (int r = 0; r < 10; ++r) {
        const uint32_t h0 = __umulhi(0xD2511F53u, c0), l0 = 0xD2511F53u * c0;
        const uint32_t h1 = __umulhi(0xCD9E8D57u, c2), l1 = 0xCD9E8D57u * c2;
        const uint32_t n0 = h1 ^ c1 ^ k0, n2 = h0 ^ c3 ^ k1;
        c0 = n0; c1 = l1; c2 = n2; c3 = l0;
        k0 += 0x9E3779B9u; k1 += 0xBB67AE85u;
    }
    out[0] = c0; out[1] = c1; out[2] = c2; out[3] = c3;
}
__device__ __forceinline__ float u01(uint32_t u) { return ((float)(u >> 8) + 0.5f) * (1.0f / 16777216.0f); }

struct SampleDev {
    const unsigned long long* total;
    const float* ring; const float* expert_ring; const float* bc_table;
    float* rows; float* bc_rows; float* noise; int* idx; int* idx_bc;
    long long cap;
    uint32_t expert_len, bc_len;
    int32_t n_main;
    uint32_t call;
    uint64_t seed;
    float sigma;
    uint32_t guard;
};
struct DrawMap {
    uint32_t live, e0, h, jump;
};
__device__ __forceinline__ DrawMap draw_map(unsigned long long tot, unsigned long long cap, uint32_t guard) {
    DrawMap m;
    if (guard == 0u) {
        m.live = (uint32_t)(tot < cap ? tot : cap);
        m.e0 = 0u; m.h = 0xFFFFFFFFu; m.jump = 0u;
        return m;
    }
    if (tot < cap) {
        const unsigned long long over = tot + guard > cap ? tot + guard - cap : 0ull;
        m.e0 = (uint32_t)(over < tot ? over : tot);
        m.live = (uint32_t)tot - m.e0;
        m.h = 0xFFFFFFFFu; m.jump = 0u;
    } else {
        const uint32_t g = guard < cap ? guard : (uint32_t)cap;
        m.h = (uint32_t)(tot % cap);
        const unsigned long long over = (unsigned long long)m.h + g > cap ? (unsigned long long)m.h + g - cap : 0ull;
        m.e0 = (uint32_t)over;
        m.live = (uint32_t)cap - g;
        m.jump = g - m.e0;
        if (g == 0u) m.h = 0xFFFFFFFFu;
    }
    return m;
}
__device__ __forceinline__ uint32_t slot_of_draw(const DrawMap& m, uint32_t k) {
    uint32_t s = k + m.e0;
    if (s >= m.h) s += m.jump;
    return s;
}
template <typename S>
__device__ __forceinline__ float smoothing_noise(const S& SA, int k) {
    uint32_t uu[4];
    philox4x32_10(0xFFFFFFF0u, SA.call, 2u, 0u, (uint32_t)SA.seed, (uint32_t)(SA.seed >> 32), uu);
    const float ua = u01(uu[k & 2]), ub = u01(uu[(k & 2) + 1]);
    const float rad = sqrtf(-2.0f * __logf(ua)), ang = 6.28318530717958647692f * ub;
    return SA.sigma * ((k & 1) ? rad * __sinf(ang) : rad * __cosf(ang));
}
constexpr int kFusedSlots = 1024, kFusedBatchMax = 256;
__device__ __forceinline__ uint32_t fused_hash(uint32_t k) { return (k * 2654435761u) >> 22; }

__device__ __forceinline__ void draw_fused(const SampleDev& S, int B, uint32_t (*hkey)[kFusedSlots], int (*hown)[kFusedSlots], int (*fin)[kFusedBatchMax]) {
    const int tid = threadIdx.x;
    const int t = tid & 511, stream = tid >> 9;
    const unsigned long long tot = *S.total;
    const DrawMap dm = draw_map(tot, (unsigned long long)S.cap, S.guard);
    const uint32_t len_main = dm.live;
    const uint32_t k0 = (uint32_t)S.seed, k1 = (uint32_t)(S.seed >> 32);
    const bool live = (stream == 0 || S.idx_bc != nullptr) && t < B;
    const bool main_grp = t < S.n_main;
    const uint32_t len = stream == 1 ? S.bc_len : (main_grp ? len_main : S.expert_len);
    const uint32_t grp = (stream == 1 || main_grp) ? 0u : 0x80000000u;
    uint32_t* keys = hkey[stream];
    int* owns = hown[stream];
    for (int e = t; e < kFusedSlots; e += 512) {
        keys[e] = 0xFFFFFFFFu;
        owns[e] = 0x7FFFFFFF;
    }
    __syncthreads();
    uint32_t key = 0;
    bool dup = live;
    for (int round = 0; round < 128; ++round) {
        if (dup) {
            uint32_t u[4];
            philox4x32_10((uint32_t)t, S.call, (uint32_t)stream, (uint32_t)round, k0, k1, u);
            key = grp | (len ? __umulhi(u[0], len) : 0u);
            uint32_t h = fused_hash(key);
            for (int probe = 0; probe < kFusedSlots; ++probe) {
                const uint32_t k = atomicCAS(&keys[h], 0xFFFFFFFFu, key);
                if (k == 0xFFFFFFFFu || k == key) break;
                h = (h + 1) & (kFusedSlots - 1);
            }
            atomicMin(&owns[h], t);
        }
        __syncthreads();
        if (live) {
            uint32_t h = fused_hash(key);
            for (int probe = 0; probe < kFusedSlots && keys[h] != key; ++probe) h = (h + 1) & (kFusedSlots - 1);
            dup = owns[h] != t;
        }
        if (!__syncthreads_or(dup)) break;
    }
    if (live) fin[stream][t] = (stream == 0 && main_grp) ? (int)slot_of_draw(dm, key & 0x7FFFFFFFu) : (int)(key & 0x7FFFFFFFu);
    __syncthreads();
}

__device__ __forceinline__ void predraw_wg(const SampleDev& S, int B, float* scratch) {
    auto hkey = reinterpret_cast<uint32_t (*)[kFusedSlots]>(scratch);
    auto hown = reinterpret_cast<int (*)[kFusedSlots]>(scratch + 2 * kFusedSlots);
    auto fin = reinterpret_cast<int (*)[kFusedBatchMax]>(scratch + 4 * kFusedSlots);
    draw_fused(S, B, hkey, hown, fin);
    const int tid = threadIdx.x;
    if (tid < B) {
        S.idx[tid] = fin[0][tid];
        if (S.idx_bc) S.idx_bc[tid] = fin[1][tid];
    }
    if (tid < 4 && S.noise) S.noise[tid] = smoothing_noise(S, tid);
    const bool bc = S.bc_rows && S.bc_table && S.idx_bc;
    for (int e = tid; e < B * 8; e += kWide) {
        const int r = e >> 3, c = e & 7;
        const float4 m = reinterpret_cast<const float4*>((r < S.n_main ? S.ring : S.expert_ring) + (size_t)fin[0][r] * 32)[c];
        float4 q = make_float4(0.f, 0.f, 0.f, 0.f);
        if (bc) q = reinterpret_cast<const float4*>(S.bc_table + (size_t)fin[1][r] * 32)[c];
        reinterpret_cast<float4*>(S.rows)[e] = m;
        if (bc) reinterpret_cast<float4*>(S.bc_rows)[e] = q;
    }
}

struct FwdJob {
    const float* net;
    Mlp m;
    RowSrc src;
    int col0;
    int act_mode;
    Head prev;
    const float* noise;
    float noise_clamp;
    Slot ws;
    int rows;
    int save;
    int img;
};
struct FwdArgs {
    FwdJob job[6];
    int njobs;
    float slope;
    float* zero_f;
    int zero_nf;
    int* zero_i;
    const SampleDev* sample;
    const uint16_t* images;
};

template <int OUTMAX>
struct HeadImage {
    static constexpr int kStride = (2 + OUTMAX) * H2 + 8;
    static constexpr int kPer = ((2 + OUTMAX) * (H2 / 4) + kWide - 1) / kWide;
    v4f v[kPer];
    float b3v;
    __device__ __forceinline__ void fetch(const float* __restrict__ net, const Mlp& m, int tid) {
        const int w0 = __builtin_amdgcn_readfirstlane(tid);
        if (w0 < m.out) b3v = net[m.b3() + (tid < m.out ? tid : 0)];
#pragma unroll
        for (int i = 0; i < kPer; ++i) {
            const int e = tid + i * kWide;
            if (w0 + i * kWide < (2 + m.out) * (H2 / 4)) v[i] = reinterpret_cast<const v4f*>(net + m.g2())[e < (2 + m.out) * (H2 / 4) ? e : 0];
        }
    }
    __device__ __forceinline__ void store(float* hp, const float* __restrict__ net, const Mlp& m, int tid) const {
#pragma unroll
        for (int i = 0; i < kPer; ++i) {
            const int e = tid + i * kWide;
            if (e < (2 + m.out) * (H2 / 4)) reinterpret_cast<v4f*>(hp)[e] = v[i];
        }
        (void)net;
        if (tid < m.out) hp[(2 + OUTMAX) * H2 + tid] = b3v;
    }
};
template <int OUTMAX, int IMG, bool RELU>
__device__ __forceinline__ void head_regs(const RowReg<H2>& z, const float* hp, int out, float slope, RowReg<H2>& xhat, RowReg<H2>& y,
                                          float& mean, float& rstd, float (&o)[OUTMAX], int no_ln = 0) {
    RowReg<H2> g, be;
    row_stats<8>(z.v, H2, mean, rstd);
    if (no_ln) { mean = 0.0f; rstd = 1.0f; }
    g.load(hp);
    be.load(hp + H2);
#pragma unroll
    for (int i = 0; i < 8; ++i) {
        xhat.v[i] = (z.v[i] - mean) * rstd;
        y.v[i] = g.v[i] * xhat.v[i] + be.v[i];
    }
#pragma unroll
    for (int j = 0; j < OUTMAX; ++j) {
        float acc = 0.0f;
        if (j < out) {
            RowReg<H2> w;
            w.load(hp + (2 + j) * H2);
#pragma unroll
            for (int i = 0; i < 8; ++i) acc += act_f<RELU>(y.v[i], slope) * w.v[i];
            acc = wave_sum(acc) + hp[(2 + IMG) * H2 + j];
        }
        o[j] = acc;
    }
}

typedef __bf16 v8bf __attribute__((ext_vector_type(8)));
__host__ __device__ inline uint32_t w2f_image_index(uint32_t col, uint32_t k) {
    return ((((col >> 4) * 16u + (k >> 4)) * 4u + ((k >> 2) & 3u)) * 16u + (col & 15u)) * 4u + (k & 3u);
}
__host__ __device__ inline uint32_t w2_image_index(uint32_t col, uint32_t k) {
    return ((((col >> 4) * 8u + (k >> 5)) * 4u + ((k >> 3) & 3u)) * 16u + (col & 15u)) * 8u + (k & 7u);
}
__host__ __device__ inline uint32_t w2t_image_index(uint32_t k1, uint32_t n) {
    return ((((k1 >> 4) * 16u + (n >> 5)) * 4u + ((n >> 3) & 3u)) * 16u + (k1 & 15u)) * 8u + (n & 7u);
}
constexpr int LDB1 = H1 + 16;
constexpr int LDB2 = H2 + 16;
enum { IM_ACTOR = 0, IM_C1, IM_C2, IM_TA, IM_TC1, IM_TC2, IM_BC, IM_ACTOR_T, IM_C1_T, IM_C2_T, IM_COUNT };
constexpr size_t kImgElems = (size_t)H2 * H1;
__device__ __forceinline__ void split3_bf16(float x, uint16_t& hi, uint16_t& mid, uint16_t& lo) {
    const __bf16 h = (__bf16)x;
    const float r1 = x - (float)h;
    const __bf16 m = (__bf16)r1;
    const float r2 = r1 - (float)m;
    const __bf16 l = (__bf16)r2;
    hi = __builtin_bit_cast(uint16_t, h); mid = __builtin_bit_cast(uint16_t, m); lo = __builtin_bit_cast(uint16_t, l);
}
__device__ __forceinline__ v8bf as_v8bf(const uint4& q) { return __builtin_bit_cast(v8bf, q); }
__device__ __forceinline__ v4f mfma16_bf16(const uint4& a, const uint4& b, v4f c) {
    return __builtin_amdgcn_mfma_f32_16x16x32_bf16(as_v8bf(a), as_v8bf(b), c, 0, 0, 0);
}
__device__ __forceinline__ uint4 pack8_bf16(const float (&v)[8]) {
    typedef __bf16 v2bf __attribute__((ext_vector_type(2)));
    uint4 q;
    q.x = __builtin_bit_cast(unsigned, v2bf{(__bf16)v[0], (__bf16)v[1]});
    q.y = __builtin_bit_cast(unsigned, v2bf{(__bf16)v[2], (__bf16)v[3]});
    q.z = __builtin_bit_cast(unsigned, v2bf{(__bf16)v[4], (__bf16)v[5]});
    q.w = __builtin_bit_cast(unsigned, v2bf{(__bf16)v[6], (__bf16)v[7]});
    return q;
}

enum { BM_CRITIC_TD = 0, BM_CRITIC_PI = 1, BM_ACTOR_PI = 2, BM_ACTOR_BC = 3, BM_GIVEN = 4,
       BM_SAC_QMIN = 5,
       BM_SAC_POLICY = 6 };

#pragma clang fp contract(off)
__device__ __forceinline__ void sac_policy_dout(float da, float a, float se, float mask, float ab, float& d_mean, float& d_logstd) {
    const float t = 1.0f - a * a;
    const float dHdx = (-2.0f * a * t) / (t + 1e-6f);
    const float dLdx = da * t - ab * dHdx;
    d_mean = dLdx;
    d_logstd = (dLdx * se - ab) * mask;
}
#pragma clang fp contract(fast)

struct BwdJob {
    const float* net;
    Mlp m;
    Slot ws;
    int rows;
    int mode;
    Head t1, t2;
    RowSrc src;
    float gamma;
    Head soft;
    Head crit;
    float lambda;
    const float* bonus;
    const float* bonus_scale;
    int loss_slot;
    int img_t;
};
struct BwdArgs {
    BwdJob job[2];
    int njobs;
    float slope;
    float inv_batch;
    float* losses;
    int* soft_count;
    const uint16_t* images;
};

struct WgJob {
    const float* net;
    float* grad;
    Mlp m;
    Slot ws[2];
    int rows[2];
    int nslots;
    int wmode[2];
    float* p; float* mom; float* var;
    float* target;
    uint16_t* w2b;
    float* w2f;
    uint16_t* w2tb;
    uint16_t* tgt_w2b;
    int w2b_x9;
};
struct WgAdam {
    float b1, b2, eps, step_size, bc2_sqrt, tau;
    int finish_actor, use_bc;
    float* losses;
    float* wstate;
    float* alpha_state;
    float target_entropy, alpha_step_size;
};
struct WgArgs {
    WgJob job[2];
    int njobs;
    float slope;
    WgAdam ad;
    int w_kind;
    float w_given, warm, inv_batch;
    const int* soft_count;
    const float* wstate;
    int bf16;
    float* count_out;
    const SampleDev* predraw;
    int predraw_batch;
};

#pragma clang fp contract(off)
__device__ __forceinline__ void adam_update(float& p, float& m, float& v, float g, float b1, float b2, float eps, float step_size, float bc2_sqrt) {
    m = __builtin_fmaf(g, 1.0f - b1, m * b1);
    v = __builtin_fmaf(g * g, 1.0f - b2, v * b2);
    const float denom = __builtin_amdgcn_sqrtf(v) * __builtin_amdgcn_rcpf(bc2_sqrt) + eps;
    p = p - step_size * (m * __builtin_amdgcn_rcpf(denom));
}
__device__ __forceinline__ float polyak_update(float target, float p, float tau) { return target * (1.0f - tau) + p * tau; }
#pragma clang fp contract(fast)
__device__ __forceinline__ float effective_w(int kind, float given, float warm, float inv_batch, const int* count, const float* wstate) {
    float w = given;
    if (kind == 1) w = (float)(*count) * inv_batch + warm;
    if (kind == 2) w = *wstate;
    return w > 1.0f ? 1.0f : w;
}

struct AdamArgs {
    float* p; const float* g; float* m; float* v;
    int n;
    float b1, b2, eps, step_size, bc2_sqrt, gscale;
    int finish_actor;
    int w_kind; float w_given, warm, inv_batch;
    const int* soft_count; float* wstate; float* losses; int use_bc;
    float* alpha_state;
    float target_entropy, alpha_step_size;
    float* target;
    float tau;
    uint16_t* w2b;
    float* w2f;
    int w2b_x9;
    int w2_lo;
    int nseg;
    int seg_lo[2];
    uint16_t* seg_w2b[2];
    uint16_t* seg_w2tb[2];
    uint16_t* seg_tgt_w2b[2];
    const float* g2;
    const float* countf;
    const uint32_t* guard;
};
template <typename A>
inline void set_adam_scalars(A& a, double lr, int step) {
    const double b1 = 0.9, b2 = 0.999;
    const double bc1 = 1.0 - pow(b1, step), bc2 = 1.0 - pow(b2, step);
    a.b1 = (float)b1; a.b2 = (float)b2; a.eps = 1e-8f;
    a.step_size = (float)(lr / bc1);
    a.bc2_sqrt = (float)sqrt(bc2);
}

constexpr size_t kSlotFloats = XP + H1 + 2 + H1 + H2 + 2 + OW + H2 + H1 + OW + 2 * kColWgB;

enum { S_TA = 0, S_C1, S_C2, S_TC1, S_TC2, S_API, S_ABC, S_BCS, S_CPI, S_CSOFT, S_COUNT };

const Mlp kActor{13, 4, 0};
const Mlp kQ{17, 1, 0};
const Mlp kPolicy{13, 8, 1};
const Mlp kQs{17, 1, 1};

__device__ __forceinline__ float pick8(const float (&o)[8], int i) {
    return i == 0 ? o[0] : i == 1 ? o[1] : i == 2 ? o[2] : i == 3 ? o[3] : i == 4 ? o[4] : i == 5 ? o[5] : i == 6 ? o[6] : o[7];
}

inline int prepare_draw(const HxSample* S, int B, float* rows, float* bc_rows, float* noise, void* stream, SampleDev* SD, bool* fused, bool launch_now = true) {
    HX_REQUIRE(S->total && S->cap > 0 && S->ring && S->idx && rows && S->n_main >= 0 && S->n_main <= B,
               "hx_*_sampled: the draw needs total, cap, ring, idx and the output tile rows");
    HX_REQUIRE(S->n_main == B || S->expert_ring, "hx_*_sampled: expert rows requested without an expert ring");
    HX_REQUIRE(!S->bc_table == !S->idx_bc && (!S->bc_table || bc_rows), "hx_*_sampled: bc_table, idx_bc and bc_rows go together");
    *fused = B <= kFusedBatchMax;
    HX_REQUIRE(!S->guard || *fused, "hx_*_sampled: HxSample.guard is honoured by the fused draw only (batch <= 256)");
    HX_REQUIRE(!S->guard || 2 * (int64_t)S->guard <= S->cap, "hx_*_sampled: a guard of more than half the ring leaves too little to draw from (cap >= 2 n)");
    if (*fused) {
        *SD = SampleDev{(const unsigned long long*)S->total, S->ring, S->expert_ring ? S->expert_ring : S->ring, S->bc_table, rows,
                        S->bc_table ? bc_rows : nullptr, noise, S->idx, S->idx_bc, (long long)S->cap, (uint32_t)S->expert_len, (uint32_t)S->bc_len,
                        S->n_main, S->call, S->seed, S->sigma, S->guard};
        return 0;
    }
    if (!launch_now) return 0;
    return hx_sample_batch(S->total, S->cap, S->ring, S->expert_ring, S->expert_len, S->bc_table, S->bc_len, B, S->n_main, 1, S->seed, S->call,
                           S->sigma, S->idx, S->idx_bc, noise, rows, S->bc_table ? bc_rows : nullptr, stream);
}

inline int sac_check_formats(const HxSacNets* N, const char* who) {
    const uint16_t* im = N->w2_bf16_all;
    HX_REQUIRE(!im || (reinterpret_cast<uintptr_t>(im) & 15u) == 0, "%s: w2_bf16_all must be a 16-byte aligned buffer", who);
    HX_REQUIRE(!N->policy_w2_bf16 || (reinterpret_cast<uintptr_t>(N->policy_w2_bf16) & 15u) == 0, "%s: policy_w2_bf16 must be 16-byte aligned", who);
    HX_REQUIRE(!im || (!N->policy_w2_x9 && !N->policy_w2_f32i && (!N->policy_w2_bf16 || N->policy_w2_bf16 == im + IM_ACTOR * kImgElems)),
               "%s: w2_bf16_all excludes policy_w2_x9 and policy_w2_f32i, and policy_w2_bf16 must be NULL or its first image (one acting format at a time)", who);
    HX_REQUIRE(!N->policy_w2_bf16 || !N->policy_w2_x9, "%s: policy_w2_bf16 excludes policy_w2_x9 (one acting format at a time)", who);
    return 0;
}
inline const uint16_t* sac_act_image(const HxSacNets* N) { return N->w2_bf16_all ? N->w2_bf16_all + IM_ACTOR * kImgElems : N->policy_w2_bf16; }

void launch_fwd(const FwdArgs& F, hipStream_t st);
void set_fwd_nt(int nt, int skip, int count);
int launch_bwd(int grp, const BwdArgs& G, hipStream_t st);
void launch_wg(const WgArgs& W, bool adam, hipStream_t st);
void launch_adam(const AdamArgs& A, hipStream_t st);
void launch_polyak(float* target, const float* source, int n, float tau, float* target2, const float* source2, int n2, hipStream_t st,
                   const uint32_t* guard = nullptr);
void launch_pack_bf16(const float* w2, uint16_t* image, bool transposed, hipStream_t st);

}
```

hirl4ucav_amd/csrc/hx_wgrad.hip:

```cpp
#include <cmath>

#include "hx_update.h"

using namespace hxnn;
using namespace hxu;

namespace {

struct WgJobC {
    const float* net; float* grad;
    float* ws0; float* ws1;
    float* mom; float* var; float* target; uint16_t* w2b; float* w2f;
    uint32_t cfg;
    int32_t rows0, rows1;
    float slope, w_given, warm, inv_batch;
    float b1, b2, eps, step_size, bc2_sqrt, tau;
    uint32_t pad_;
    const int* soft_count; float* wstate; float* losses;
    uint16_t* w2tb; uint16_t* tgt_w2b;
    float* count_out;
};
static_assert(sizeof(WgJobC) == 176, "WgJobC layout");
struct WgArgsC {
    WgJobC job[2];
    int has_pre, pre_batch;
    SampleDev pre;
};

struct AdamElem {
    float p, m, v, t;
    __device__ __forceinline__ void fetch(const WgJob& J, unsigned idx) {
        p = J.p[idx];
        m = J.mom[idx];
        v = J.var[idx];
        t = J.target ? J.target[idx] : 0.0f;
    }
    __device__ __forceinline__ void apply(const WgJob& J, const WgAdam& a, unsigned idx, float g) {
        adam_update(p, m, v, g, a.b1, a.b2, a.eps, a.step_size, a.bc2_sqrt);
        J.p[idx] = p;
        J.mom[idx] = m;
        J.var[idx] = v;
        if (J.target) {
            t = polyak_update(t, p, a.tau);
            J.target[idx] = t;
        }
    }
};

constexpr int kWgTilesPerBlock = 2 * (H2 / 16);
constexpr int kWgCols = 16;
constexpr int kWgVecWgs = H2 / kWgCols;
constexpr int kWgL1Wgs = H1 / kWgCols;
constexpr int kWgRG = kWide / kWgCols;
constexpr int kWgPerJob = kWgTilesPerBlock + kWgVecWgs + kWgL1Wgs;
constexpr int kWgRowChunk = 256;

constexpr int kRedP = 21;
__device__ __forceinline__ float sum_groups(const float* p, int half) {
    constexpr int N = kWgRG / 2;
    float v[N];
#pragma unroll
    for (int g = 0; g < N; ++g) v[g] = p[(2 * g + half) * kWgCols * kRedP];
#pragma unroll
    for (int w = 1; w < N; w *= 2)
#pragma unroll
        for (int g = 0; g < N; g += 2 * w) v[g] += v[g + w];
    const float other = __int_as_float(__builtin_amdgcn_mov_dpp(__float_as_int(v[0]), 0xB1, 0xf, 0xf, true));
    return half ? other + v[0] : v[0] + other;
}

__device__ __forceinline__ void expand_wg(const WgJobC& c, WgJob& J, WgArgs& A) {
    J.net = c.net; J.grad = c.grad; J.m = mlp_of(c.cfg & 1023u);
    J.nslots = (int)((c.cfg >> 10) & 3u);
    J.wmode[0] = (int)((c.cfg >> 12) & 3u); J.wmode[1] = (int)((c.cfg >> 14) & 3u);
    J.ws[0] = carve_slot(c.ws0, c.rows0); J.ws[1] = carve_slot(c.ws1, c.rows1);
    J.rows[0] = c.rows0; J.rows[1] = c.rows1;
    J.p = const_cast<float*>(c.net); J.mom = c.mom; J.var = c.var; J.target = c.target; J.w2b = c.w2b; J.w2f = c.w2f;
    J.w2tb = c.w2tb; J.tgt_w2b = c.tgt_w2b; J.w2b_x9 = (int)((c.cfg >> 20) & 1u);
    A.slope = c.slope; A.w_kind = (int)((c.cfg >> 16) & 3u); A.w_given = c.w_given; A.warm = c.warm; A.inv_batch = c.inv_batch;
    A.soft_count = c.soft_count; A.wstate = c.wstate;
    A.ad.b1 = c.b1; A.ad.b2 = c.b2; A.ad.eps = c.eps; A.ad.step_size = c.step_size; A.ad.bc2_sqrt = c.bc2_sqrt; A.ad.tau = c.tau;
    A.ad.finish_actor = (int)((c.cfg >> 18) & 1u); A.ad.use_bc = (int)((c.cfg >> 19) & 1u);
    A.ad.losses = c.losses; A.ad.wstate = c.wstate;
    A.count_out = c.count_out;
    A.ad.alpha_state = nullptr; A.ad.target_entropy = 0.0f; A.ad.alpha_step_size = 0.0f;
    if ((c.cfg >> 21) & 1u) {
        A.ad.alpha_state = c.wstate; A.ad.target_entropy = c.w_given; A.ad.alpha_step_size = c.warm;
        A.ad.wstate = nullptr; A.wstate = nullptr; A.w_given = 0.0f; A.warm = 0.0f;
    }
}
inline WgJobC pack_wg(const WgJob& J, const WgArgs& A) {
    WgJobC c{};
    c.net = J.net; c.grad = J.grad; c.ws0 = J.ws[0].x; c.ws1 = J.nslots > 1 ? J.ws[1].x : J.ws[0].x;
    c.mom = J.mom; c.var = J.var; c.target = J.target; c.w2b = J.w2b; c.w2f = J.w2f; c.w2tb = J.w2tb; c.tgt_w2b = J.tgt_w2b;
    c.cfg = mlp_bits(J.m) | ((uint32_t)J.nslots << 10) | ((uint32_t)J.wmode[0] << 12) | ((uint32_t)J.wmode[1] << 14) | ((uint32_t)A.w_kind << 16) |
            ((uint32_t)(A.ad.finish_actor ? 1 : 0) << 18) | ((uint32_t)(A.ad.use_bc ? 1 : 0) << 19) | ((uint32_t)(J.w2b_x9 ? 1 : 0) << 20) |
            ((uint32_t)(A.ad.alpha_state ? 1 : 0) << 21);
    c.rows0 = J.rows[0]; c.rows1 = J.nslots > 1 ? J.rows[1] : J.rows[0];
    c.slope = A.slope; c.w_given = A.w_given; c.warm = A.warm; c.inv_batch = A.inv_batch;
    c.b1 = A.ad.b1; c.b2 = A.ad.b2; c.eps = A.ad.eps; c.step_size = A.ad.step_size; c.bc2_sqrt = A.ad.bc2_sqrt; c.tau = A.ad.tau;
    c.soft_count = A.soft_count; c.wstate = const_cast<float*>(A.wstate); c.losses = A.ad.losses; c.count_out = A.count_out;
    if (A.ad.alpha_state) { c.wstate = A.ad.alpha_state; c.w_given = A.ad.target_entropy; c.warm = A.ad.alpha_step_size; }
    return c;
}

#ifdef HX_STAMPS_L1
#define STAMP_L1() STAMP()
#else
#define STAMP_L1()
#endif
template <bool ADAM, bool RELU, bool BF16 = false>
__global__ __launch_bounds__(kWide) void wgrad_kernel(WgArgsC AC) {
    __shared__ __attribute__((aligned(16))) float lds[kWgRowChunk * XP + kWgRowChunk * 12 + kWgRG * kWgCols * kRedP];
    float* xs = lds;
    float* rinfo = lds + kWgRowChunk * XP;
    float* red = rinfo + kWgRowChunk * 12;

    {
        static_assert(sizeof(lds) >= (4 * kFusedSlots + 2 * kFusedBatchMax) * 4, "predraw_wg's tables fit");
        if (AC.has_pre && blockIdx.x >= kWgPerJob) {
            if (blockIdx.x == kWgPerJob && blockIdx.y == 0) predraw_wg(AC.pre, AC.pre_batch, lds);
            return;
        }
    }
    const int j = blockIdx.y, b = blockIdx.x;
    WgJob J;
    WgArgs A;
    expand_wg(AC.job[j], J, A);
    const int tid = threadIdx.x, wave = tid >> 6, lane = tid & 63;
    const float slope = A.slope;
    STAMP_DECL;
    STAMP();
    const float w = effective_w(A.w_kind, A.w_given, A.warm, A.inv_batch, A.soft_count, A.wstate);
    float scale[2];
#pragma unroll
    for (int s = 0; s < 2; ++s) scale[s] = J.wmode[s] == 0 ? 1.0f : (J.wmode[s] == 1 ? 1.0f - w : w);
#ifdef HX_STAMPS
    asm volatile("" ::"v"(w));
    STAMP();
#endif
    if (A.count_out && blockIdx.x == 0 && blockIdx.y == 0 && tid == 0) *A.count_out = A.soft_count ? (float)*A.soft_count : 0.0f;
    if (ADAM && A.ad.finish_actor && blockIdx.x == 0 && blockIdx.y == 0 && tid == 0) {
        if (A.ad.use_bc) {
            A.ad.losses[1] = A.ad.losses[2] * w + A.ad.losses[3] * (1.0f - w);
            A.ad.losses[5] = w;
            *A.ad.wstate = w;
        } else {
            A.ad.losses[1] = A.ad.losses[3];
        }
    }
    if (ADAM && A.ad.alpha_state && blockIdx.x == 0 && blockIdx.y == 0 && tid == 0) {
        const float mean_h = A.ad.losses[4];
        float la = A.ad.alpha_state[0], m = A.ad.alpha_state[1], v = A.ad.alpha_state[2];
        A.ad.losses[3] = -(la * (A.ad.target_entropy - mean_h));
        adam_update(la, m, v, mean_h - A.ad.target_entropy, A.ad.b1, A.ad.b2, A.ad.eps, A.ad.alpha_step_size, A.ad.bc2_sqrt);
        A.ad.alpha_state[0] = la; A.ad.alpha_state[1] = m; A.ad.alpha_state[2] = v;
        A.ad.alpha_state[3] = expf(la);
        A.ad.losses[5] = A.ad.alpha_state[3];
    }

    if (b < kWgTilesPerBlock) {
        const int n0 = (b >> 1) * 16, k0 = (b & 1) * (H1 / 2) + (wave & 7) * 16, half = wave >> 3;
        const int r = lane & 15, g = lane >> 4;
        v4f acc = {0.f, 0.f, 0.f, 0.f};
        #pragma unroll
        for (int s = 0; s < 2; ++s) if (s < J.nslots) {
            const float sc = scale[s];
            const float* dz = J.ws[s].dz2;
            const float* h1 = J.ws[s].h1;
            const unsigned dzo = (unsigned)(n0 + r), h1o = (unsigned)(k0 + r);
            const int rows = J.rows[s];
            const int hr = ((rows + 7) >> 3) << 2;
            const int rbeg = half * hr, rend = min(rows, rbeg + hr);
            if constexpr (BF16) {
                v4f accs = {0.f, 0.f, 0.f, 0.f};
                for (int c0 = rbeg; c0 < rend; c0 += 64) {
                    float av[2][8], hv[2][8];
#pragma unroll
                    for (int m = 0; m < 2; ++m)
#pragma unroll
                        for (int j = 0; j < 8; ++j) {
                            const int row = c0 + 32 * m + 8 * g + j;
                            const unsigned rc = (unsigned)(row < rows ? row : rows - 1);
                            av[m][j] = dz[rc * (unsigned)H2 + dzo];
                            hv[m][j] = h1[rc * (unsigned)H1 + h1o];
                        }
#pragma unroll
                    for (int m = 0; m < 2; ++m) {
#pragma unroll
                        for (int j = 0; j < 8; ++j)
                            if (c0 + 32 * m + 8 * g + j >= rend) av[m][j] = 0.0f;
                        accs = mfma16_bf16(pack8_bf16(av[m]), pack8_bf16(hv[m]), accs);
                    }
                }
#pragma unroll
                for (int q = 0; q < 4; ++q) acc[q] = __builtin_fmaf(sc, accs[q], acc[q]);
            } else {
                for (int c0 = rbeg; c0 < rend; c0 += 64) {
                    float av[16], hv[16];
#pragma unroll
                    for (int i = 0; i < 16; ++i) {
                        const int row = c0 + 4 * i + g;
                        const unsigned rc = (unsigned)(row < rows ? row : rows - 1);
                        av[i] = dz[rc * (unsigned)H2 + dzo];
                        hv[i] = h1[rc * (unsigned)H1 + h1o];
                    }
#pragma unroll
                    for (int i = 0; i < 16; ++i) acc = mfma16(av[i] * (c0 + 4 * i + g < rend ? sc : 0.0f), hv[i], acc);
                }
            }
        }
        STAMP();
        const int q0 = 2 * half;
        AdamElem ae[2];
        if (ADAM) {
#pragma unroll
            for (int q = 0; q < 2; ++q) ae[q].fetch(J, J.m.W2() + (n0 + 4 * g + q0 + q) * H1 + k0 + r);
        }
        float2* xch = reinterpret_cast<float2*>(red);
        xch[((wave & 7) * 2 + half) * 64 + lane] = half ? make_float2(acc[0], acc[1]) : make_float2(acc[2], acc[3]);
        __syncthreads();
        const float2 got = xch[((wave & 7) * 2 + (half ^ 1)) * 64 + lane];
        const float fin[2] = {half ? got.x + acc[2] : acc[0] + got.x, half ? got.y + acc[3] : acc[1] + got.y};
        float* out = J.grad + J.m.W2();
#pragma unroll
        for (int q = 0; q < 2; ++q) out[(unsigned)((n0 + 4 * g + q0 + q) * H1 + k0 + r)] = fin[q];
        if (ADAM) {
#pragma unroll
            for (int q = 0; q < 2; ++q) {
                const int idx = J.m.W2() + (n0 + 4 * g + q0 + q) * H1 + k0 + r;
                ae[q].apply(J, A.ad, idx, fin[q]);
                if (J.w2b) {
                    const uint32_t ix = w2_image_index((uint32_t)(n0 + 4 * g + q0 + q), (uint32_t)(k0 + r));
                    uint16_t hi, mid, lo;
                    split3_bf16(ae[q].p, hi, mid, lo);
                    J.w2b[ix] = hi;
                    if (J.w2b_x9) { J.w2b[kImgElems + ix] = mid; J.w2b[2 * kImgElems + ix] = lo; }
                }
                if (J.w2f) J.w2f[w2f_image_index((uint32_t)(n0 + 4 * g + q0 + q), (uint32_t)(k0 + r))] = ae[q].p;
                if (J.w2tb) {
                    const __bf16 bv = (__bf16)ae[q].p;
                    J.w2tb[w2t_image_index((uint32_t)(k0 + r), (uint32_t)(n0 + 4 * g + q0 + q))] = __builtin_bit_cast(uint16_t, bv);
                }
                if (J.target && J.tgt_w2b) {
                    const __bf16 bv = (__bf16)ae[q].t;
                    J.tgt_w2b[w2_image_index((uint32_t)(n0 + 4 * g + q0 + q), (uint32_t)(k0 + r))] = __builtin_bit_cast(uint16_t, bv);
                }
            }
        }
        STAMP();
        STAMP_FLUSH(32, blockIdx.x == 0 && blockIdx.y == 0 && tid == 0);
        SPAN_LOG(HX_SPAN_WGRAD);
        return;
    }
    const int cl = lane & (kWgCols - 1);
    const int rg = tid / kWgCols;
    const int ohalf = tid & 1, oitem = (tid >> 1) / kWgCols, ocol = (tid >> 1) % kWgCols;
    if (b < kWgTilesPerBlock + kWgVecWgs) {
        constexpr int RP = 12;
        const int vb = b - kWgTilesPerBlock;
        const int n = vb * kWgCols + cl;
        const float g2 = J.net[J.m.g2() + n], be2 = J.net[J.m.be2() + n];
        float w3[OW];
#pragma unroll
        for (int jj = 0; jj < OW; ++jj) w3[jj] = jj < J.m.out ? J.net[J.m.W3() + jj * H2 + n] : 0.0f;
        float db2 = 0.f, dg = 0.f, dbe = 0.f, dw3[OW] = {}, db3 = 0.f;
        const int on = vb * kWgCols + ocol;
        const unsigned vidx = (unsigned)(oitem == 0 ? J.m.b2() + on : oitem == 1 ? J.m.g2() + on : oitem == 2 ? J.m.be2() + on : J.m.W3() + (oitem - 3) * H2 + on);
        const bool vlive = oitem < 3 + J.m.out;
        const bool b3live = vb == 0 && oitem == 3 + OW && ocol < J.m.out;
        const unsigned b3idx = (unsigned)(J.m.b3() + (ocol < J.m.out ? ocol : 0));
        AdamElem vae;
        bool vae_pending = ADAM && (vlive || b3live) && ohalf == 0;
        #pragma unroll
        for (int s = 0; s < 2; ++s) if (s < J.nslots) {
            const Slot& S = J.ws[s];
            const float sc = scale[s];
            for (int c0 = 0; c0 < J.rows[s]; c0 += kWgRowChunk) {
                const int nr = min(kWgRowChunk, J.rows[s] - c0);
                float zv[4], dv[4];
#pragma unroll
                for (int i = 0; i < 4; ++i) if (kWgRG * i < nr) {
                    const int r = rg + kWgRG * i;
                    const unsigned o = (unsigned)(c0 + (r < nr ? r : nr - 1)) * (unsigned)H2 + (unsigned)n;
                    zv[i] = S.z2[o];
                    dv[i] = S.dz2[o];
                }
                static_assert(kWgRowChunk <= kWide, "staging: one row per thread");
                const int er = tid < nr ? tid : 0;
                v2f st2v;
                v4f d4, d5;
                if (__builtin_amdgcn_readfirstlane(tid) < nr) {
                    st2v = *reinterpret_cast<const v2f*>(S.st2 + (size_t)(c0 + er) * 2);
                    d4 = *reinterpret_cast<const v4f*>(S.dout + (size_t)(c0 + er) * OW);
                    d5 = *reinterpret_cast<const v4f*>(S.dout + (size_t)(c0 + er) * OW + 4);
                }
                if (vae_pending) {
                    vae.fetch(J, b3live ? b3idx : vidx);
                    vae_pending = false;
                }
                __syncthreads();
                if (tid < nr) {
                    float4* r4 = reinterpret_cast<float4*>(rinfo + tid * RP);
                    r4[0] = make_float4(st2v[0], st2v[1], d4[0], d4[1]);
                    r4[1] = make_float4(d4[2], d4[3], d5[0], d5[1]);
                    r4[2] = make_float4(d5[2], d5[3], 0.0f, 0.0f);
                }
                __syncthreads();
                for (int rb0 = 0; rb0 < nr; rb0 += kWgRG * 4) {
                    const int rb = rg + rb0;
                    if (rb0 != 0) {
#pragma unroll
                        for (int i = 0; i < 4; ++i) if (rb0 + kWgRG * i < nr) {
                            const int r = rb + kWgRG * i;
                            const unsigned o = (unsigned)(c0 + (r < nr ? r : nr - 1)) * (unsigned)H2 + (unsigned)n;
                            zv[i] = S.z2[o];
                            dv[i] = S.dz2[o];
                        }
                    }
#pragma unroll
                    for (int i = 0; i < 4; ++i) {
                        const int r = rb + kWgRG * i;
                        if (r < nr) {
                            float ri[RP];
                            {
                                const float4* r4 = reinterpret_cast<const float4*>(rinfo + r * RP);
                                const float4 a = r4[0], b4 = r4[1], c4 = r4[2];
                                ri[0] = a.x; ri[1] = a.y; ri[2] = a.z; ri[3] = a.w; ri[4] = b4.x; ri[5] = b4.y; ri[6] = b4.z; ri[7] = b4.w;
                                ri[8] = c4.x; ri[9] = c4.y; ri[10] = c4.z; ri[11] = c4.w;
                            }
                            const float xh = (zv[i] - ri[0]) * ri[1];
                            const float y = g2 * xh + be2;
                            float dh2 = (ri[2] * w3[0] + ri[3] * w3[1]) + (ri[4] * w3[2] + ri[5] * w3[3]);
                            if (J.m.out > 4) dh2 += (ri[6] * w3[4] + ri[7] * w3[5]) + (ri[8] * w3[6] + ri[9] * w3[7]);
                            const float dy = act_bwd<RELU>(dh2, y, slope);
                            const float h2 = act_f<RELU>(y, slope);
                            db2 += sc * dv[i];
                            dbe += sc * dy;
                            dg += sc * dy * xh;
#pragma unroll
                            for (int jj = 0; jj < OW; ++jj) dw3[jj] += sc * ri[2 + jj] * h2;
                            if (vb == 0 && cl < J.m.out) db3 += sc * rinfo[r * RP + 2 + cl];
                        }
                    }
                }
            }
        }
        STAMP();
        float* my = red + (rg * kWgCols + cl) * kRedP;
        my[0] = db2; my[1] = dg; my[2] = dbe;
#pragma unroll
        for (int jj = 0; jj < OW; ++jj) my[3 + jj] = dw3[jj];
        my[3 + OW] = db3;
        __syncthreads();
        if (vlive || b3live) {
            float v = sum_groups(red + ocol * kRedP + oitem, ohalf);
            if ((oitem == 1 || oitem == 2) && J.m.no_ln) v = 0.0f;
            const unsigned idx = b3live ? b3idx : vidx;
            if (ohalf == 0) {
                J.grad[idx] = v;
                if (ADAM) vae.apply(J, A.ad, idx, v);
            }
        }
        STAMP();
        STAMP_FLUSH(40, b == kWgTilesPerBlock && j == 0 && tid == 0);
        SPAN_LOG(HX_SPAN_WGRAD);
        return;
    }
    {
        const int kb = (b - kWgTilesPerBlock - kWgVecWgs) * kWgCols;
        const int k = kb + cl;
        const int in = J.m.in;
        const float g1 = J.net[J.m.g1() + k], be1 = J.net[J.m.be1() + k];
        STAMP_L1();
        float db1 = 0.f, dg = 0.f, dbe = 0.f, dw1[17];
#pragma unroll
        for (int i = 0; i < 17; ++i) dw1[i] = 0.f;
        const int ok = kb + ocol;
        const unsigned lidx = (unsigned)(oitem == 0 ? J.m.b1() + ok : oitem == 1 ? J.m.g1() + ok : oitem == 2 ? J.m.be1() + ok : J.m.W1() + ok * in + (oitem - 3));
        const bool llive = oitem < 3 + in;
        AdamElem lae;
        bool lae_pending = ADAM && llive && ohalf == 0;
        #pragma unroll
        for (int s = 0; s < 2; ++s) if (s < J.nslots) {
            const Slot& S = J.ws[s];
            const float sc = scale[s];
            for (int c0 = 0; c0 < J.rows[s]; c0 += kWgRowChunk) {
                const int nr = min(kWgRowChunk, J.rows[s] - c0);
                float zv[4], dv[4];
#pragma unroll
                for (int i = 0; i < 4; ++i) if (kWgRG * i < nr) {
                    const int r = rg + kWgRG * i;
                    const unsigned o = (unsigned)(c0 + (r < nr ? r : nr - 1)) * (unsigned)H1 + (unsigned)k;
                    zv[i] = S.z1[o];
                    dv[i] = S.dh1[o];
                }
                STAMP_L1();
                static_assert(kWgRowChunk * XP <= 5 * kWide && kWgRowChunk <= kWide && kColWgB == 8, "staging: five words + one row per thread");
                const int w0 = __builtin_amdgcn_readfirstlane(tid);
                float xst[5];
#pragma unroll
                for (int q = 0; q < 5; ++q) {
                    const int e = tid + q * kWide;
                    if (w0 + q * kWide < nr * XP) xst[q] = S.x[(size_t)c0 * XP + (e < nr * XP ? e : 0)];
                }
                STAMP_L1();
                const int er = tid < nr ? tid : 0;
                v2f st1v;
                v4f l0, l1, l2, l3;
                if (w0 < nr) {
                    st1v = *reinterpret_cast<const v2f*>(S.st1 + (size_t)(c0 + er) * 2);
                    const v4f* lp4 = reinterpret_cast<const v4f*>(S.lnp + (size_t)(c0 + er) * (2 * kColWgB));
                    l0 = lp4[0]; l1 = lp4[1]; l2 = lp4[2]; l3 = lp4[3];
                }
                STAMP_L1();
                if (lae_pending) {
                    lae.fetch(J, lidx);
                    lae_pending = false;
                }
                STAMP_L1();
                __syncthreads();
                STAMP_L1();
#pragma unroll
                for (int q = 0; q < 5; ++q) {
                    const int e = tid + q * kWide;
                    if (e < nr * XP) xs[e] = xst[q];
                }
                if (tid < nr) {
                    const float s1 = ((l0[0] + l0[2]) + (l1[0] + l1[2])) + ((l2[0] + l2[2]) + (l3[0] + l3[2]));
                    const float s2 = ((l0[1] + l0[3]) + (l1[1] + l1[3])) + ((l2[1] + l2[3]) + (l3[1] + l3[3]));
                    *reinterpret_cast<float4*>(rinfo + tid * 8) = make_float4(st1v[0], st1v[1], s1 * (1.0f / H1), s2 * (1.0f / H1));
                }
                __syncthreads();
                STAMP_L1();
                for (int rb0 = 0; rb0 < nr; rb0 += kWgRG * 4) {
                    const int rb = rg + rb0;
                    if (rb0 != 0) {
#pragma unroll
                        for (int i = 0; i < 4; ++i) if (rb0 + kWgRG * i < nr) {
                            const int r = rb + kWgRG * i;
                            const unsigned o = (unsigned)(c0 + (r < nr ? r : nr - 1)) * (unsigned)H1 + (unsigned)k;
                            zv[i] = S.z1[o];
                            dv[i] = S.dh1[o];
                        }
                    }
#pragma unroll
                    for (int i = 0; i < 4; ++i) {
                        const int r = rb + kWgRG * i;
                        if (r < nr) {
                            const float4 ri = *reinterpret_cast<const float4*>(rinfo + r * 8);
                            const float xh = (zv[i] - ri.x) * ri.y;
                            const float dy = act_bwd<RELU>(dv[i], g1 * xh + be1, slope);
                            const float dz = sc * (ri.y * (dy * g1 - ri.z - xh * ri.w));
                            db1 += dz;
                            dbe += sc * dy;
                            dg += sc * dy * xh;
                            const float4* xr4 = reinterpret_cast<const float4*>(xs + r * XP);
#pragma unroll
                            for (int q = 0; q < 4; ++q) {
                                const float4 x4 = xr4[q];
                                dw1[4 * q] += dz * x4.x; dw1[4 * q + 1] += dz * x4.y; dw1[4 * q + 2] += dz * x4.z; dw1[4 * q + 3] += dz * x4.w;
                            }
                            dw1[16] += dz * xs[r * XP + 16];
                        }
                    }
                }
            }
        }
        STAMP_L1();
        float* my = red + (rg * kWgCols + cl) * kRedP;
        my[0] = db1; my[1] = dg; my[2] = dbe;
#pragma unroll
        for (int i = 0; i < 17; ++i) my[3 + i] = dw1[i];
        STAMP_L1();
        __syncthreads();
        STAMP_L1();
        if (llive) {
            float v = sum_groups(red + ocol * kRedP + oitem, ohalf);
            if ((oitem == 1 || oitem == 2) && J.m.no_ln) v = 0.0f;
#ifdef HX_STAMPS
            asm volatile("" ::"v"(v));
            STAMP_L1();
#endif
            if (ohalf == 0) {
                J.grad[lidx] = v;
                if (ADAM) lae.apply(J, A.ad, lidx, v);
            }
        }
        STAMP_L1();
        STAMP_FLUSH(48, b == kWgTilesPerBlock + kWgVecWgs && j == 0 && tid == 0);
        SPAN_LOG(HX_SPAN_WGRAD);
    }
}

__device__ __forceinline__ float adam_w(const AdamArgs& A) {
    if (A.countf && A.w_kind == 1) {
        const float w = *A.countf * A.inv_batch + A.warm;
        return w > 1.0f ? 1.0f : w;
    }
    return effective_w(A.w_kind, A.w_given, A.warm, A.inv_batch, A.soft_count, A.wstate);
}

__global__ __launch_bounds__(kThreads) void adam_kernel(AdamArgs A) {
    if (A.guard && __hip_atomic_load(A.guard, __ATOMIC_RELAXED, __HIP_MEMORY_SCOPE_SYSTEM) != 0u) return;
    if (A.alpha_state && blockIdx.x == 0 && threadIdx.x == 0) {
        const float mean_h = A.losses[4];
        float la = A.alpha_state[0], m = A.alpha_state[1], v = A.alpha_state[2];
        A.losses[3] = -(la * (A.target_entropy - mean_h));
        adam_update(la, m, v, mean_h - A.target_entropy, A.b1, A.b2, A.eps, A.alpha_step_size, A.bc2_sqrt);
        A.alpha_state[0] = la; A.alpha_state[1] = m; A.alpha_state[2] = v;
        A.alpha_state[3] = expf(la);
        A.losses[5] = A.alpha_state[3];
    }
    const float wmix = A.g2 ? adam_w(A) : 0.0f;
    if (A.finish_actor && blockIdx.x == 0 && threadIdx.x == 0) {
        if (A.use_bc) {
            const float w = adam_w(A);
            A.losses[1] = A.losses[2] * w + A.losses[3] * (1.0f - w);
            A.losses[5] = w;
            *A.wstate = w;
        } else {
            A.losses[1] = A.losses[3];
        }
    }
    const int i = (blockIdx.x * kThreads + threadIdx.x) * 4;
    if (i >= A.n) return;
    if (i + 4 <= A.n) {
        float4 p4 = *reinterpret_cast<const float4*>(A.p + i), g4 = *reinterpret_cast<const float4*>(A.g + i);
        float4 m4 = *reinterpret_cast<const float4*>(A.m + i), v4 = *reinterpret_cast<const float4*>(A.v + i);
        if (A.g2) {
            const float4 b4 = *reinterpret_cast<const float4*>(A.g2 + i);
            g4.x = wmix * b4.x + (1.0f - wmix) * g4.x;
            g4.y = wmix * b4.y + (1.0f - wmix) * g4.y;
            g4.z = wmix * b4.z + (1.0f - wmix) * g4.z;
            g4.w = wmix * b4.w + (1.0f - wmix) * g4.w;
        }
        adam_update(p4.x, m4.x, v4.x, g4.x * A.gscale, A.b1, A.b2, A.eps, A.step_size, A.bc2_sqrt);
        adam_update(p4.y, m4.y, v4.y, g4.y * A.gscale, A.b1, A.b2, A.eps, A.step_size, A.bc2_sqrt);
        adam_update(p4.z, m4.z, v4.z, g4.z * A.gscale, A.b1, A.b2, A.eps, A.step_size, A.bc2_sqrt);
        adam_update(p4.w, m4.w, v4.w, g4.w * A.gscale, A.b1, A.b2, A.eps, A.step_size, A.bc2_sqrt);
        *reinterpret_cast<float4*>(A.p + i) = p4;
        *reinterpret_cast<float4*>(A.m + i) = m4;
        *reinterpret_cast<float4*>(A.v + i) = v4;
        if (A.w2b && i >= A.w2_lo && i < A.w2_lo + H2 * H1) {
            typedef __bf16 v4bf __attribute__((ext_vector_type(4)));
            const v4bf r = {(__bf16)p4.x, (__bf16)p4.y, (__bf16)p4.z, (__bf16)p4.w};
            const uint32_t e = (uint32_t)(i - A.w2_lo);
            const uint32_t ix = w2_image_index(e / H1, e % H1);
            *reinterpret_cast<uint2*>(A.w2b + ix) = __builtin_bit_cast(uint2, r);
            if (A.w2b_x9) {
                const float pv[4] = {p4.x, p4.y, p4.z, p4.w};
                uint16_t md[4], lw[4];
#pragma unroll
                for (int q = 0; q < 4; ++q) { uint16_t h; split3_bf16(pv[q], h, md[q], lw[q]); }
                *reinterpret_cast<uint2*>(A.w2b + kImgElems + ix) = make_uint2((uint32_t)md[0] | ((uint32_t)md[1] << 16), (uint32_t)md[2] | ((uint32_t)md[3] << 16));
                *reinterpret_cast<uint2*>(A.w2b + 2 * kImgElems + ix) = make_uint2((uint32_t)lw[0] | ((uint32_t)lw[1] << 16), (uint32_t)lw[2] | ((uint32_t)lw[3] << 16));
            }
        }
        if (A.w2f && i >= A.w2_lo && i < A.w2_lo + H2 * H1) {
            const uint32_t e = (uint32_t)(i - A.w2_lo);
            *reinterpret_cast<float4*>(A.w2f + w2f_image_index(e / H1, e % H1)) = p4;
        }
        float4 t4 = make_float4(0.f, 0.f, 0.f, 0.f);
        if (A.target) {
            t4 = *reinterpret_cast<const float4*>(A.target + i);
            t4.x = polyak_update(t4.x, p4.x, A.tau);
            t4.y = polyak_update(t4.y, p4.y, A.tau);
            t4.z = polyak_update(t4.z, p4.z, A.tau);
            t4.w = polyak_update(t4.w, p4.w, A.tau);
            *reinterpret_cast<float4*>(A.target + i) = t4;
        }
        for (int sg = 0; sg < A.nseg; ++sg) {
            if (i < A.seg_lo[sg] || i >= A.seg_lo[sg] + H2 * H1) continue;
            typedef __bf16 v4bf __attribute__((ext_vector_type(4)));
            const uint32_t e = (uint32_t)(i - A.seg_lo[sg]), col = e / H1, k = e % H1;
            const v4bf r = {(__bf16)p4.x, (__bf16)p4.y, (__bf16)p4.z, (__bf16)p4.w};
            if (A.seg_w2b[sg]) *reinterpret_cast<uint2*>(A.seg_w2b[sg] + w2_image_index(col, k)) = __builtin_bit_cast(uint2, r);
            if (A.seg_w2tb[sg]) {
                const uint2 q = __builtin_bit_cast(uint2, r);
                uint16_t* tb = A.seg_w2tb[sg];
                tb[w2t_image_index(k, col)] = (uint16_t)(q.x & 0xFFFFu);
                tb[w2t_image_index(k + 1, col)] = (uint16_t)(q.x >> 16);
                tb[w2t_image_index(k + 2, col)] = (uint16_t)(q.y & 0xFFFFu);
                tb[w2t_image_index(k + 3, col)] = (uint16_t)(q.y >> 16);
            }
            if (A.target && A.seg_tgt_w2b[sg]) {
                const v4bf rt = {(__bf16)t4.x, (__bf16)t4.y, (__bf16)t4.z, (__bf16)t4.w};
                *reinterpret_cast<uint2*>(A.seg_tgt_w2b[sg] + w2_image_index(col, k)) = __builtin_bit_cast(uint2, rt);
            }
        }
        return;
    }
    for (int c = 0; c < A.n - i; ++c) {
        float pv = A.p[i + c], mv = A.m[i + c], vv = A.v[i + c];
        const float gv = A.g2 ? wmix * A.g2[i + c] + (1.0f - wmix) * A.g[i + c] : A.g[i + c];
        adam_update(pv, mv, vv, gv * A.gscale, A.b1, A.b2, A.eps, A.step_size, A.bc2_sqrt);
        A.p[i + c] = pv; A.m[i + c] = mv; A.v[i + c] = vv;
        if (A.target) A.target[i + c] = polyak_update(A.target[i + c], pv, A.tau);
    }
}

__global__ __launch_bounds__(kThreads) void polyak_kernel(float* target, const float* source, int n, float tau, float* target2 = nullptr,
                                                          const float* source2 = nullptr, int n2 = 0, const uint32_t* guard = nullptr) {
    if (guard && *guard != 0u) return;
    const int nb1 = (n / 4 + kThreads) / kThreads;
    int blk = blockIdx.x;
    if (blk >= nb1) {
        blk -= nb1; target = target2; source = source2; n = n2;
    }
    const int i = (blk * kThreads + threadIdx.x) * 4;
    if (i >= n) return;
    if (i + 4 <= n) {
        float4 t4 = *reinterpret_cast<const float4*>(target + i);
        const float4 s4 = *reinterpret_cast<const float4*>(source + i);
        t4.x = polyak_update(t4.x, s4.x, tau);
        t4.y = polyak_update(t4.y, s4.y, tau);
        t4.z = polyak_update(t4.z, s4.z, tau);
        t4.w = polyak_update(t4.w, s4.w, tau);
        *reinterpret_cast<float4*>(target + i) = t4;
        return;
    }
    for (int c = 0; c < n - i; ++c) target[i + c] = polyak_update(target[i + c], source[i + c], tau);
}

}

namespace hxu {

void launch_wg(const WgArgs& W, bool adam, hipStream_t st) {
    WgArgsC C{};
    for (int j = 0; j < W.njobs; ++j) C.job[j] = pack_wg(W.job[j], W);
    const bool pre = W.predraw != nullptr;
    C.has_pre = pre ? 1 : 0;
    if (pre) { C.pre = *W.predraw; C.pre_batch = W.predraw_batch; }
    const dim3 grid(kWgPerJob + (pre ? 8 : 0), W.njobs);
    const bool relu = W.slope == 0.0f;
#define HX_WG(ADAM_, RELU_, BF16_) hipLaunchKernelGGL((wgrad_kernel<ADAM_, RELU_, BF16_>), grid, dim3(kWide), 0, st, C)
    static const int dbg_off = getenv("HX_DBG_BF16_OFF") ? atoi(getenv("HX_DBG_BF16_OFF")) : 0;
    if (W.bf16 && !(dbg_off & 4)) {
        if (adam) { if (relu) HX_WG(true, true, true); else HX_WG(true, false, true); }
        else { if (relu) HX_WG(false, true, true); else HX_WG(false, false, true); }
    } else {
        if (adam) { if (relu) HX_WG(true, true, false); else HX_WG(true, false, false); }
        else { if (relu) HX_WG(false, true, false); else HX_WG(false, false, false); }
    }
#undef HX_WG
}
void launch_adam(const AdamArgs& A, hipStream_t st) {
    hipLaunchKernelGGL(adam_kernel, dim3((A.n / 4 + kThreads) / kThreads), dim3(kThreads), 0, st, A);
}
void launch_polyak(float* target, const float* source, int n, float tau, float* target2, const float* source2, int n2, hipStream_t st, const uint32_t* guard) {
    const int nb = (n / 4 + kThreads) / kThreads + (target2 ? (n2 / 4 + kThreads) / kThreads : 0);
    hipLaunchKernelGGL(polyak_kernel, dim3(nb), dim3(kThreads), 0, st, target, source, n, tau, target2, source2, n2, guard);
}

}

extern "C" {

static int adam_impl(const HxNets* N, const HxHyper* Hy, int32_t which, int32_t step, float grad_scale, int32_t w_kind, float w_given,
                     float warm, int32_t batch, const float* msg, void* stream) {
    const bool polyak = (which & 16) != 0;
    which &= 15;
    HX_REQUIRE(N && Hy && step >= 1 && which >= 0 && which <= 2, "hx_adam: bad arguments");
    AdamArgs A{};
    A.n = which == 0 ? 2 * kQ.padded() : kActor.size();
    A.p = which == 0 ? N->critic : N->actor;
    A.g = which == 0 ? N->grad_critic : N->grad_actor;
    A.m = which == 0 ? N->m_critic : N->m_actor;
    A.v = which == 0 ? N->v_critic : N->v_actor;
    set_adam_scalars(A, which == 0 ? Hy->lr_critic : Hy->lr_actor, step);
    A.gscale = grad_scale;
    A.finish_actor = which == 1;
    A.w_kind = w_kind; A.w_given = w_given; A.warm = warm; A.inv_batch = 1.0f / (batch > 0 ? batch : 1);
    A.soft_count = N->soft_count; A.wstate = N->wstate; A.losses = N->losses; A.use_bc = Hy->use_bc;
    if (polyak) {
        A.target = which == 0 ? N->target_critic : N->target_actor;
        A.tau = Hy->tau;
    }
    if (which != 0 && N->actor_w2_f32i) {
        A.w2f = N->actor_w2_f32i;
        A.w2_lo = kActor.W2();
    }
    if (which != 0 && N->actor_w2_bf16 && !N->w2_bf16_all) {
        A.w2b = N->actor_w2_bf16;
        A.w2_lo = kActor.W2();
    }
    if (which != 0 && N->actor_w2_x9) {
        HX_REQUIRE(!N->actor_w2_bf16 && !N->w2_bf16_all, "hx_adam: actor_w2_x9 excludes the plain bf16 images (one acting format at a time)");
        A.w2b = N->actor_w2_x9;
        A.w2b_x9 = 1;
        A.w2_lo = kActor.W2();
    }
    if (uint16_t* im = N->w2_bf16_all) {
        HX_REQUIRE(!N->actor_w2_bf16 || N->actor_w2_bf16 == im + IM_ACTOR * kImgElems, "hx_adam: with w2_bf16_all set, actor_w2_bf16 must be NULL or its first image");
        if (which == 0) {
            A.nseg = 2;
            for (int h = 0; h < 2; ++h) {
                A.seg_lo[h] = h * kQ.padded() + kQ.W2();
                A.seg_w2b[h] = im + (IM_C1 + h) * kImgElems;
                A.seg_w2tb[h] = im + (IM_C1_T + h) * kImgElems;
                A.seg_tgt_w2b[h] = im + (IM_TC1 + h) * kImgElems;
            }
        } else {
            A.nseg = 1;
            A.seg_lo[0] = kActor.W2();
            A.seg_w2b[0] = im + IM_ACTOR * kImgElems;
            A.seg_w2tb[0] = im + IM_ACTOR_T * kImgElems;
            A.seg_tgt_w2b[0] = im + IM_TA * kImgElems;
        }
    }
    A.guard = N->xchg_status;
    if (msg) {
        HX_REQUIRE(which == 1 && (reinterpret_cast<uintptr_t>(msg) & 15u) == 0, "hx_adam_mixed: actor step only, 16-byte aligned message");
        A.g = msg;
        if (Hy->use_bc) {
            A.g2 = msg + kActor.padded();
            A.countf = msg + 2 * kActor.padded();
        }
    }
    HX_REQUIRE((((uintptr_t)A.p | (uintptr_t)A.g | (uintptr_t)A.m | (uintptr_t)A.v) & 15u) == 0, "hx_adam: buffers must be 16-byte aligned");
    launch_adam(A, (hipStream_t)stream);
    HX_CHECK_LAUNCH("hx_adam");
    return 0;
}
int hx_adam(const HxNets* N, const HxHyper* Hy, int32_t which, int32_t step, float grad_scale, int32_t w_kind, float w_given,
            float warm, int32_t batch, void* stream) {
    return adam_impl(N, Hy, which, step, grad_scale, w_kind, w_given, warm, batch, nullptr, stream);
}
int hx_adam_mixed(const HxNets* N, const HxHyper* Hy, int32_t polyak, int32_t step, float grad_scale, int32_t w_kind, float w_given,
                  float warm, int32_t batch, const float* msg, void* stream) {
    HX_REQUIRE(msg, "hx_adam_mixed: null message");
    return adam_impl(N, Hy, 1 | (polyak ? 16 : 0), step, grad_scale, w_kind, w_given, warm, batch, msg, stream);
}

int hx_polyak(const HxNets* N, const HxHyper* Hy, void* stream) {
    HX_REQUIRE(N && Hy, "hx_polyak: bad arguments");
    const int nc = 2 * kQ.padded(), na = kActor.size();
    launch_polyak(N->target_critic, N->critic, nc, Hy->tau, N->target_actor, N->actor, na, (hipStream_t)stream, N->xchg_status);
    if (uint16_t* im = N->w2_bf16_all) {
        launch_pack_bf16(N->target_actor + kActor.W2(), im + IM_TA * kImgElems, false, (hipStream_t)stream);
        for (int h = 0; h < 2; ++h)
            launch_pack_bf16(N->target_critic + h * kQ.padded() + kQ.W2(), im + (IM_TC1 + h) * kImgElems, false, (hipStream_t)stream);
    }
    HX_CHECK_LAUNCH("hx_polyak");
    return 0;
}

int hx_sac_adam(const HxSacNets* N, const HxHyper* Hy, int32_t which, int32_t step, float grad_scale, float target_entropy, void* stream) {
    HX_REQUIRE(N && Hy && step >= 1 && (which == 0 || which == 1), "hx_sac_adam: bad arguments");
    AdamArgs A{};
    A.n = which == 0 ? 2 * kQs.padded() : kPolicy.padded();
    A.p = which == 0 ? N->critic : N->policy;
    A.g = which == 0 ? N->grad_critic : N->grad_policy;
    A.m = which == 0 ? N->m_critic : N->m_policy;
    A.v = which == 0 ? N->v_critic : N->v_policy;
    set_adam_scalars(A, which == 0 ? Hy->lr_critic : Hy->lr_actor, step);
    A.gscale = grad_scale;
    A.losses = N->losses;
    if (which == 1 && N->policy_w2_f32i) {
        A.w2f = N->policy_w2_f32i;
        A.w2_lo = kPolicy.W2();
    }
    if (which == 1 && N->policy_w2_x9) {
        A.w2b = N->policy_w2_x9;
        A.w2b_x9 = 1;
        A.w2_lo = kPolicy.W2();
    }
    if (which == 1 && N->policy_w2_bf16 && !N->w2_bf16_all) {
        A.w2b = N->policy_w2_bf16;
        A.w2_lo = kPolicy.W2();
    }
    if (int rc = sac_check_formats(N, "hx_sac_adam")) return rc;
    if (uint16_t* im = N->w2_bf16_all) {
        if (which == 0) {
            A.nseg = 2;
            for (int h = 0; h < 2; ++h) {
                A.seg_lo[h] = h * kQs.padded() + kQs.W2();
                A.seg_w2b[h] = im + (IM_C1 + h) * kImgElems;
                A.seg_w2tb[h] = im + (IM_C1_T + h) * kImgElems;
            }
        } else {
            A.nseg = 1;
            A.seg_lo[0] = kPolicy.W2();
            A.seg_w2b[0] = im + IM_ACTOR * kImgElems;
            A.seg_w2tb[0] = im + IM_ACTOR_T * kImgElems;
        }
    }
    if (which == 1) {
        A.alpha_state = N->alpha_state;
        A.target_entropy = target_entropy;
        A.alpha_step_size = A.step_size;
    }
    launch_adam(A, (hipStream_t)stream);
    HX_CHECK_LAUNCH("hx_sac_adam");
    return 0;
}

}

HX_DEFINE_DEBUG_COLLECTORS(wgrad, 32, 56)
```

include/hirl4ucav.h:

```cpp
#ifndef HIRL4UCAV_H
#define HIRL4UCAV_H

#include <stdint.h>

#ifdef __cplusplus
extern "C" {
#endif

#define HX_ENV_WORDS 37
#define HX_OBS_DIM 13
#define HX_ACT_DIM 4
#define HX_ROW_WORDS 32

#define HX_F_LOCKED_PREV (1u << 0)
#define HX_F_LOCKED (1u << 1)
#define HX_F_SLOT_PREV (1u << 2)
#define HX_F_SLOT (1u << 3)
#define HX_F_FIRED (1u << 4)
#define HX_F_FIRE_SUCCESS (1u << 5)
#define HX_F_EPISODE_SUCCESS (1u << 6)
#define HX_F_DONE (1u << 7)
#define HX_F_SCEN_SHIFT 8
#define HX_F_SERP_POS (1u << 10)
#define HX_F_SERP_LONG (1u << 11)
#define HX_F_M_ACTIVE (1u << 12)
#define HX_F_M_GUIDED (1u << 13)
#define HX_F_SIM_SLOT (1u << 14)

#define HX_ERR_ARG (-1)
#define HX_ERR_HIP (-2)

enum { HX_STAT_EPISODES = 0, HX_STAT_KILLS, HX_STAT_FIRE_SUCCESS_EPISODES, HX_STAT_TIME_LIMIT, HX_STAT_FIRES,
       HX_STAT_GOOD_FIRES, HX_STAT_LOCKED_STEPS, HX_STAT_ENV_STEPS,
       HX_STAT_NONFINITE_ACTIONS,
       HX_STAT_COUNT };
#define HX_STAT_WAYS 32
#define HX_STAT_PITCH 16

const char* hx_last_error(void);
#define HX_ABI_VERSION 117
int hx_version(void);
int hx_abi_sizes(int32_t* sizes8);
void* hx_event_create(void);
int hx_event_destroy(void* ev);
int hx_event_elapsed_us(void* start, void* stop, float* us );

typedef struct HxStepOpts {
    int32_t max_step;
    int32_t auto_reset;
    int32_t randomize;
    uint32_t env_id0;
    uint64_t seed;
    uint32_t* episode_ctr;
    float* ring;
    int8_t* ring_success;
    int64_t cap;
    uint64_t* total;
    uint64_t* stats;
    void* ev_start;
    void* ev_stop;
    int32_t layout;
} HxStepOpts;
#define HX_LAYOUT(pair, envs_per_block) ((((pair) ? 1 : 0) << 8) | ((envs_per_block) / 4))
#define HX_LAYOUT_ORDERED_SLOTS (1 << 16)

int hx_env_reset(float* state, int64_t n, int64_t stride, const uint8_t* mask, const int32_t* scenario,
                 int32_t scenario_all, int32_t randomize, uint64_t seed, uint32_t env_id0, uint32_t* episode_ctr,
                 float* obs, void* stream);

int hx_env_step(float* state, int64_t n, int64_t stride, const float* actions, float* obs_io, float* reward,
                uint8_t* done, int8_t* success, const HxStepOpts* opts , void* stream);

int hx_env_rearm(float* state, int64_t n, int64_t stride, const uint8_t* mask, void* stream);

int hx_sim_tick(float* state, int64_t n, int64_t stride, const float* ally_cmd, const float* opp_cmd, const uint8_t* fire,
                void* stream);
int hx_sim_readback(const float* state, int64_t n, int64_t stride, float* out, void* stream);

int hx_env_pack_row(const float* state, int64_t n, int64_t stride, int64_t i, const float* obs, const float* reward, const uint8_t* done,
                    const int8_t* success, float* out , void* stream);

int hx_label_transitions(const float* s, const float* a, const float* ns, int64_t n, float* reward, int8_t* success,
                         uint8_t* done, void* stream);


int hx_actor_param_count(void);
int hx_critic_param_count(void);
int64_t hx_hirl_workspace_floats(int32_t batch);
int64_t hx_act_workspace_floats(int64_t rows);

int hx_actor_act(const float* actor, const float* obs, int64_t rows, float* actions, int32_t noise_mode,
                 const float* noise, float sigma, uint64_t seed, uint32_t row0, uint32_t call, float slope, float* ws,
                 void* stream);
int hx_actor_act_step(const float* actor, float* state, int64_t n, int64_t stride, float* obs_io, float* actions,
                      int32_t noise_mode, const float* noise, float sigma, uint64_t seed, uint32_t row0, uint32_t call, float slope,
                      float* reward, uint8_t* done, int8_t* success, const HxStepOpts* opts , void* stream);

int hx_pack_w2_bf16(const float* net, int32_t in_dim, uint16_t* w2_bf16, void* stream);
int hx_actor_act_bf16(const float* actor, const uint16_t* w2_bf16, const float* obs, int64_t rows, float* actions, int32_t noise_mode,
                      const float* noise, float sigma, uint64_t seed, uint32_t row0, uint32_t call, float slope, void* stream);
int hx_actor_act_step_bf16(const float* actor, const uint16_t* w2_bf16, float* state, int64_t n, int64_t stride, float* obs_io,
                           float* actions, int32_t noise_mode, const float* noise, float sigma, uint64_t seed, uint32_t row0, uint32_t call,
                           float slope, float* reward, uint8_t* done, int8_t* success, const HxStepOpts* opts ,
                           void* stream);

int hx_pack_w2_f32i(const float* net, int32_t in_dim, float* w2_f32i, void* stream);
int hx_actor_act_f32i(const float* actor, const float* w2_f32i, const float* obs, int64_t rows, float* actions, int32_t noise_mode,
                      const float* noise, float sigma, uint64_t seed, uint32_t row0, uint32_t call, float slope, void* stream);
int hx_actor_act_step_f32i(const float* actor, const float* w2_f32i, float* state, int64_t n, int64_t stride, float* obs_io,
                           float* actions, int32_t noise_mode, const float* noise, float sigma, uint64_t seed, uint32_t row0, uint32_t call,
                           float slope, float* reward, uint8_t* done, int8_t* success, const HxStepOpts* opts ,
                           void* stream);

int hx_pack_w2_x9(const float* net, int32_t in_dim, uint16_t* w2_x9, void* stream);
int hx_actor_act_x9(const float* actor, const uint16_t* w2_x9, const float* obs, int64_t rows, float* actions, int32_t noise_mode,
                    const float* noise, float sigma, uint64_t seed, uint32_t row0, uint32_t call, float slope, void* stream);
int hx_actor_act_step_x9(const float* actor, const uint16_t* w2_x9, float* state, int64_t n, int64_t stride, float* obs_io,
                         float* actions, int32_t noise_mode, const float* noise, float sigma, uint64_t seed, uint32_t row0, uint32_t call,
                         float slope, float* reward, uint8_t* done, int8_t* success, const HxStepOpts* opts ,
                         void* stream);

typedef struct HxBatch {
    const float* rows;
    const float* bc_rows;
    int32_t batch;
    const float* noise;
} HxBatch;

typedef struct HxNets {
    float* actor; float* critic; float* target_actor; float* target_critic; const float* bc_actor;
    float* grad_actor; float* grad_critic;
    float* m_actor; float* v_actor; float* m_critic; float* v_critic;
    float* losses;
    int32_t* soft_count;
    float* wstate;
    float* ws;
    uint16_t* actor_w2_bf16;
    float* actor_w2_f32i;
    uint16_t* w2_bf16_all;
    const uint32_t* xchg_status;
    uint16_t* actor_w2_x9;
} HxNets;

int64_t hx_bf16_images_elems(void);
int hx_pack_update_images(const HxNets* nets, void* stream);

typedef struct HxHyper {
    float gamma, tau, lr_actor, lr_critic, slope, noise_clamp, loss_lambda;
    int32_t use_bc;
    int32_t no_layernorm;
} HxHyper;

int hx_hirl_critic_grads(const HxNets* nets, const HxBatch* batch, const HxHyper* hyper, int32_t actor_fwd, void* stream);
int hx_hirl_actor_backward(const HxNets* nets, const HxBatch* batch, const HxHyper* hyper, int32_t estimate_soft,
                           int32_t fwd_done, void* stream);
int hx_hirl_actor_wgrad(const HxNets* nets, const HxHyper* hyper, int32_t batch, int32_t count_batch, int32_t w_kind,
                        float w_given, float warm, void* stream);
int hx_adam(const HxNets* nets, const HxHyper* hyper, int32_t which, int32_t step, float grad_scale, int32_t w_kind,
            float w_given, float warm, int32_t batch, void* stream);
int hx_polyak(const HxNets* nets, const HxHyper* hyper, void* stream);
int64_t hx_actor_message_floats(void);
int hx_hirl_actor_wgrad_split(const HxNets* nets, const HxHyper* hyper, int32_t batch, float* msg, void* stream);
int hx_adam_mixed(const HxNets* nets, const HxHyper* hyper, int32_t polyak, int32_t step, float grad_scale, int32_t w_kind, float w_given,
                  float warm, int32_t batch , const float* msg, void* stream);
int hx_bc_train_actor(const HxNets* nets, const HxBatch* batch, const HxHyper* hyper, int32_t step, void* stream);
int hx_hirl_learn(const HxNets* nets, const HxBatch* batch, const HxHyper* hyper, int32_t critic_step, int32_t actor_phase,
                  int32_t actor_step, int32_t do_polyak, int32_t w_kind, float w_given, float warm, void* stream);

int hx_sample_batch(const uint64_t* total, int64_t cap, const float* ring, const float* expert_ring, int64_t expert_len,
                    const float* bc_table, int64_t bc_len, int32_t batch, int32_t n_main, int32_t do_sample, uint64_t seed,
                    uint32_t call, float sigma, int32_t* idx, int32_t* idx_bc, float* noise, float* rows, float* bc_rows,
                    void* stream);
int hx_sample_batch_guarded(const uint64_t* total, int64_t cap, const float* ring, const float* expert_ring, int64_t expert_len,
                            const float* bc_table, int64_t bc_len, int32_t batch, int32_t n_main, int32_t do_sample, uint64_t seed,
                            uint32_t call, float sigma, int32_t* idx, int32_t* idx_bc, float* noise, float* rows, float* bc_rows,
                            uint32_t guard, void* stream);

typedef struct HxSample {
    const uint64_t* total; int64_t cap; const float* ring;
    const float* expert_ring; int64_t expert_len;
    const float* bc_table; int64_t bc_len;
    int32_t n_main;
    uint64_t seed; uint32_t call; float sigma;
    int32_t* idx; int32_t* idx_bc;
    uint32_t guard;
} HxSample;
int hx_hirl_critic_grads_sampled(const HxNets* nets, const HxBatch* batch, const HxHyper* hyper, const HxSample* sample, int32_t actor_fwd,
                                 void* stream);
int hx_hirl_learn_sampled(const HxNets* nets, const HxBatch* batch, const HxHyper* hyper, const HxSample* sample, int32_t critic_step,
                          int32_t actor_phase, int32_t actor_step, int32_t do_polyak, int32_t w_kind, float w_given, float warm, void* stream);

typedef struct HxFront {
    uint32_t* flags;
    uint32_t* status;
    uint32_t epoch;
    uint32_t with_c;
} HxFront;
int hx_hirl_front(float* state, int64_t n, int64_t stride, float* obs_io, float* actions, int32_t noise_mode,
                  const float* noise, float sigma, uint64_t seed, uint32_t row0, uint32_t call, float* reward, uint8_t* done, int8_t* success,
                  const HxStepOpts* opts, const HxNets* nets, const HxBatch* batch, const HxHyper* hyper, int32_t actor_phase, int32_t w_kind,
                  const HxFront* front, void* stream);
int hx_hirl_learn_back(const HxNets* nets, const HxBatch* batch, const HxHyper* hyper, int32_t critic_step, int32_t actor_phase, int32_t actor_step,
                       int32_t do_polyak, int32_t w_kind, float w_given, float warm, const HxSample* next, const HxBatch* next_tiles, int32_t c_in_front,
                       void* stream);
int hx_hirl_critic_grads_back(const HxNets* nets, const HxBatch* batch, const HxHyper* hyper, const HxSample* next, const HxBatch* next_tiles, int32_t c_in_front,
                              void* stream);


typedef struct HxSacNets {
    float* policy; float* critic; float* target_critic;
    float* grad_policy; float* grad_critic;
    float* m_policy; float* v_policy; float* m_critic; float* v_critic;
    float* losses;
    float* alpha_state;
    float* ws;
    float* policy_w2_f32i;
    uint16_t* policy_w2_x9;
    uint16_t* w2_bf16_all;
    uint16_t* policy_w2_bf16;
} HxSacNets;

int hx_sac_pack_update_images(const HxSacNets* nets, void* stream);

typedef struct HxSacBatch {
    const float* rows;
    int32_t batch;
    const float* eps_next;
    const float* eps_cur;
    uint64_t seed;
    uint32_t call;
} HxSacBatch;

int hx_sac_policy_param_count(void);
int64_t hx_sac_workspace_floats(int32_t batch);
int hx_sac_act(const float* policy, const float* obs, int64_t rows, float* actions, int32_t mode, const float* eps,
               uint64_t seed, uint32_t row0, uint32_t call, float* ws, void* stream);
int hx_sac_act_f32i(const float* policy, const float* w2_f32i, const float* obs, int64_t rows, float* actions, int32_t mode, const float* eps,
                    uint64_t seed, uint32_t row0, uint32_t call, void* stream);
int hx_sac_act_step_f32i(const float* policy, const float* w2_f32i, float* state, int64_t n, int64_t stride, float* obs_io, float* actions,
                         int32_t mode, const float* eps, uint64_t seed, uint32_t row0, uint32_t call, float* reward, uint8_t* done,
                         int8_t* success, const HxStepOpts* opts , void* stream);
int hx_sac_act_x9(const float* policy, const uint16_t* w2_x9, const float* w2_f32i, const float* obs, int64_t rows, float* actions, int32_t mode,
                  const float* eps, uint64_t seed, uint32_t row0, uint32_t call, void* stream);
int hx_sac_act_step_x9(const float* policy, const uint16_t* w2_x9, const float* w2_f32i, float* state, int64_t n, int64_t stride, float* obs_io,
                       float* actions, int32_t mode, const float* eps, uint64_t seed, uint32_t row0, uint32_t call, float* reward, uint8_t* done,
                       int8_t* success, const HxStepOpts* opts, void* stream);
int hx_sac_act_step(const float* policy, float* state, int64_t n, int64_t stride, float* obs_io, float* actions, int32_t mode,
                    const float* eps, uint64_t seed, uint32_t row0, uint32_t call, float* reward, uint8_t* done, int8_t* success,
                    const HxStepOpts* opts , void* stream);
int hx_sac_act_bf16(const float* policy, const uint16_t* w2_bf16, const float* obs, int64_t rows, float* actions, int32_t mode, const float* eps,
                    uint64_t seed, uint32_t row0, uint32_t call, void* stream);
int hx_sac_act_step_bf16(const float* policy, const uint16_t* w2_bf16, float* state, int64_t n, int64_t stride, float* obs_io, float* actions,
                         int32_t mode, const float* eps, uint64_t seed, uint32_t row0, uint32_t call, float* reward, uint8_t* done,
                         int8_t* success, const HxStepOpts* opts , void* stream);
int hx_sac_critic_grads(const HxSacNets* nets, const HxSacBatch* batch, const HxHyper* hyper, int32_t polyak_first, void* stream);
int hx_sac_critic_grads_sampled(const HxSacNets* nets, const HxSacBatch* batch, const HxHyper* hyper, const HxSample* sample,
                                int32_t polyak_first, void* stream);
int hx_sac_critic_step(const HxSacNets* nets, const HxSacBatch* batch, const HxHyper* hyper, const HxSample* sample, int32_t polyak_first,
                       int32_t step, void* stream);
int hx_sac_policy_grads(const HxSacNets* nets, const HxSacBatch* batch, const HxHyper* hyper, void* stream);
int hx_sac_learn(const HxSacNets* nets, const HxSacBatch* batch, const HxHyper* hyper, const HxSample* sample, int32_t polyak_first, int32_t step,
                 float target_entropy, void* stream);
int hx_sac_front(const float* policy, const uint16_t* w2_x9, const float* w2_f32i, float* state, int64_t n, int64_t stride, float* obs_io, float* actions,
                 int32_t mode, const float* eps, uint64_t seed, uint32_t row0, uint32_t call, float* reward, uint8_t* done, int8_t* success,
                 const HxStepOpts* opts, const HxSacNets* nets, const HxSacBatch* batch, void* stream);
int hx_sac_learn_back(const HxSacNets* nets, const HxSacBatch* batch, const HxHyper* hyper, int32_t polyak_first, int32_t step, float target_entropy,
                      const HxSample* next, float* next_rows, void* stream);
int hx_sac_adam(const HxSacNets* nets, const HxHyper* hyper, int32_t which, int32_t step, float grad_scale, float target_entropy,
                void* stream);

typedef struct HxSacImit {
    const float* bc_actor;
    float* expert_rows;
    float* ws;
    int32_t* count;
    float bc_slope;
} HxSacImit;
int hx_sac_imit_sizeof(void);
int64_t hx_sac_imit_workspace_floats(int32_t batch);
int hx_sac_policy_grads_imitative(const HxSacNets* nets, const HxSacBatch* batch, const HxHyper* hyper, const HxSacImit* imit, void* stream);
int hx_sac_learn_imitative(const HxSacNets* nets, const HxSacBatch* batch, const HxHyper* hyper, const HxSample* sample, const HxSacImit* imit,
                           const HxSample* expert_sample, int32_t polyak_first, int32_t step, float target_entropy, void* stream);


int hx_ipc_alloc(int64_t bytes, int32_t finegrained , void** dev_ptr);
int hx_ipc_free(void* dev_ptr);
int hx_ipc_export(void* dev_ptr, void* handle64 );
int hx_ipc_import(const void* handle64 , void** dev_ptr);
int hx_ipc_close(void* dev_ptr);
int hx_allreduce_oneshot(float* dst, const float* const* bufs, uint32_t* const* flags, uint32_t* status, int32_t world, int32_t rank,
                         int64_t n, uint32_t epoch, int32_t timeout_ms, void* stream);

int hx_allreduce_twostage(float* dst, const float* const* bufs, void* const* reds, uint32_t* const* flags, uint32_t* const* flags2, uint32_t* status,
                          int32_t world, int32_t rank, int64_t n, uint32_t epoch, int32_t timeout_ms, int32_t bf16, void* stream);

int hx_rccl_available(void);
int hx_rccl_unique_id(uint8_t* id128 );
int hx_rccl_init(const uint8_t* id128 , int32_t world, int32_t rank, void** comm );
int hx_rccl_allreduce(void* comm, void* buf, int64_t n, int32_t dtype, void* stream);
int hx_rccl_allreduce_bf16(void* comm, float* buf, uint16_t* scratch, int64_t n, void* stream);
int hx_rccl_destroy(void* comm);

#ifdef __cplusplus
}
#endif
#endif
```

Baseline: 78.21 million.

## Hoist BC actor forward into preceding critic-only front launch

On actor-phase calls the fused front launch used to run the BC-rows actor forward itself. The BC minibatch for the call after next is now drawn early by a spare workgroup in the wgrad kernel. The preceding critic-only front launch then runs that actor forward on those rows, and the actor-phase launch skips its own job when a Python-side bookkeeper confirms the result is still valid. The intent is to move work off the critical actor-phase step into otherwise lighter critic-only launches, at the cost of extra validity tracking and a risk of stale results if an actor write is missed.

Result: slower. 76.81 million (-1.8%).

```diff
diff --git a/hirl4ucav_amd/_lib.py b/hirl4ucav_amd/_lib.py
--- a/hirl4ucav_amd/_lib.py
+++ b/hirl4ucav_amd/_lib.py
@@ -42,7 +42,7 @@
 }
 
 _lib = None
-ABI_VERSION = 117
+ABI_VERSION = 118
 _ABI_STRUCTS = {}
 
 
diff --git a/hirl4ucav_amd/agents/bc_ahead.py b/hirl4ucav_amd/agents/bc_ahead.py
--- /dev/null
+++ b/hirl4ucav_amd/agents/bc_ahead.py
@@ -0,0 +1,54 @@
+import os
+
+_KNOB = ()
+
+
+def knob():
+    global _KNOB
+    if _KNOB == ():
+        v = os.environ.get("HX_FRONT_BC_AHEAD")
+        _KNOB = None if v is None or v == "" else (int(v) != 0)
+    return _KNOB
+
+
+class BcAheadBook:
+    def __init__(self):
+        self.version = 0
+        self.tile = None
+        self.slot = None
+        self.hits = 0
+        self.misses = 0
+
+    def actor_written(self):
+        self.version += 1
+        self.slot = None
+
+    def reset(self):
+        self.actor_written()
+        self.tile = None
+
+    @staticmethod
+    def want_draw(enabled, use_bc, actor_call):
+        return bool(enabled and use_bc and actor_call)
+
+    def can_hoist(self, enabled, use_bc, actor_call, next_key):
+        return bool(enabled and use_bc and not actor_call and self.tile is not None and self.tile == next_key)
+
+    def slot_ready(self, enabled, use_bc, actor_call, key):
+        if not (enabled and use_bc and actor_call):
+            return False
+        ok = self.slot is not None and self.slot == (key, self.version)
+        if ok:
+            self.hits += 1
+        else:
+            self.misses += 1
+        return ok
+
+    def drawn(self, key):
+        self.tile = key
+
+    def hoisted(self, key):
+        self.slot = (key, self.version)
+
+    def own_job_ran(self):
+        self.slot = None
diff --git a/hirl4ucav_amd/agents/engine.py b/hirl4ucav_amd/agents/engine.py
--- a/hirl4ucav_amd/agents/engine.py
+++ b/hirl4ucav_amd/agents/engine.py
@@ -5,6 +5,7 @@
 import torch
 
 from .. import _lib
+from . import bc_ahead
 
 H1, H2 = 256, 512
 _vp, _i32, _f32 = ctypes.c_void_p, ctypes.c_int32, ctypes.c_float
@@ -17,11 +18,12 @@
 class HxSample(ctypes.Structure):
     _fields_ = [("total", _vp), ("cap", ctypes.c_int64), ("ring", _vp), ("expert_ring", _vp), ("expert_len", ctypes.c_int64),
                 ("bc_table", _vp), ("bc_len", ctypes.c_int64), ("n_main", _i32), ("seed", ctypes.c_uint64), ("call", ctypes.c_uint32),
-                ("sigma", _f32), ("idx", _vp), ("idx_bc", _vp), ("guard", ctypes.c_uint32)]
+                ("sigma", _f32), ("idx", _vp), ("idx_bc", _vp), ("guard", ctypes.c_uint32), ("idx_bc_ahead", _vp), ("bc_rows_ahead", _vp)]
 
 
 class HxFront(ctypes.Structure):
-    _fields_ = [("flags", _vp), ("status", _vp), ("epoch", ctypes.c_uint32), ("with_c", ctypes.c_uint32)]
+    _fields_ = [("flags", _vp), ("status", _vp), ("epoch", ctypes.c_uint32), ("with_c", ctypes.c_uint32), ("bc_rows_ahead", _vp), ("abc_ready", ctypes.c_uint32),
+                ("pad_", ctypes.c_uint32)]
 
 
 class HxNets(ctypes.Structure):
@@ -134,6 +136,10 @@
     return 3 if sigma > 0 else 0
 
 
+def _same_draw(a, b):
+    return a is not None and len(a) == len(b) and all(x is y or (not torch.is_tensor(x) and not torch.is_tensor(y) and x == y) for x, y in zip(a, b))
+
+
 def _bc_weight_kind(bc_weight_now):
     if bc_weight_now is None:
         return 2, 0.0
@@ -151,6 +157,8 @@
         L = _lib.load()
         for i, cls in ((0, _lib.HxStepOpts), (1, HxNets), (2, HxHyper), (3, HxBatch), (4, HxSample)):
             _lib.check_struct(i, cls)
+        if L.hx_abi_size_front() != ctypes.sizeof(HxFront):
+            raise _lib.HxError(f"ABI mismatch: HxFront is {ctypes.sizeof(HxFront)} bytes here, {L.hx_abi_size_front()} in {_lib.SO_PATH}")
         assert L.hx_actor_param_count() == ACTOR_SIZE and L.hx_critic_param_count() == CRITIC_SIZE
         L.hx_hirl_workspace_floats.restype = ctypes.c_int64
         self.batch = int(batch)
@@ -173,6 +181,11 @@
         self._front_c_epoch = 0
         self._front_tiles = None
         self._front_drawn = None
+        self.front_bc_ahead = True
+        self.front_bc_ahead_used = None
+        self._bc_book = bc_ahead.BcAheadBook()
+        self._bc_ahead_tiles = None
+        self._bc_ahead_table = None
         self.nets = HxNets(*(t.data_ptr() for t in (self.actor, self.critic, self.target_actor, self.target_critic, self.bc_actor,
                                                      self.grad_actor, self.grad_critic, self.m_actor, self.v_actor, self.m_critic,
                                                      self.v_critic, self.losses, self.soft_count, self.wstate, self.ws)), None, None, None, None, None)
@@ -255,6 +268,7 @@
             self.nets.actor_w2_bf16 = None
 
     def refresh_bf16(self):
+        self._bc_book.actor_written()
         _lib.call("hx_pack_w2_f32i", self.actor.data_ptr(), 13, self.w2_f32i.data_ptr(), _lib.stream_ptr())
         if self.update_dtype == "bf16":
             _lib.call("hx_pack_update_images", ctypes.byref(self.nets), _lib.stream_ptr())
@@ -406,6 +420,7 @@
         B = self.batch
         if self.needs_reload:
             raise _lib.HxError("this engine failed after a front launch had been enqueued: load a snapshot before learn()")
+        self._bc_book.actor_written()
         st = _lib.stream_ptr()
         pending, self._pending = self._pending, None
         pipe = getattr(before_exchange, "__self__", None) if before_exchange is not None else None
@@ -482,6 +497,8 @@
             t2 = (second[:B * 32], second[B * 32:2 * B * 32], second[2 * B * 32:2 * B * 32 + B].view(torch.int32),
                   second[2 * B * 32 + B:2 * B * 32 + 2 * B].view(torch.int32), second[2 * B * 32 + 2 * B:2 * B * 32 + 2 * B + 4])
             self._front_tiles = [(self.rows, self.bc_rows, self._idx, self._idx_bc, self._noise), t2]
+            ahead = torch.zeros(B * 32 + B + 64, dtype=torch.float32, device=self.device)
+            self._bc_ahead_tiles = (ahead[:B * 32], ahead[B * 32:B * 32 + B].view(torch.int32))
         flags, status = self._front
         cur, nxt = self._front_tiles
         n_main = B if n_main is None else int(n_main)
@@ -496,6 +513,7 @@
         except _lib.HxError:
             if self._front_enqueued:
                 self.needs_reload = True
+                self._bc_book.reset()
                 raise
             (self._front_epoch, self._front_c_epoch, self.critic_step, self.actor_step, self.update_count, self.sample_calls, self.act_calls, env.steps_issued) = held
             self.front_reset()
@@ -506,16 +524,20 @@
         replay, n, B = env.replay, env.n, self.batch
         self.sample_calls += 1
 
-        def draw(tiles, call):
+        def draw(tiles, call, ahead=None):
             return HxSample(replay.total.data_ptr(), replay.capacity, replay.ring.data_ptr(), expert.ring.data_ptr() if expert is not None else None,
                             len_of(expert), _lib.ptr(bc_table), bc_table.shape[0] if bc_table is not None else 0, n_main, int(sample_seed), call,
-                            float(smooth_sigma), tiles[2].data_ptr(), tiles[3].data_ptr() if bc_table is not None else None, n)
+                            float(smooth_sigma), tiles[2].data_ptr(), tiles[3].data_ptr() if bc_table is not None else None, n,
+                            ahead[1].data_ptr() if ahead is not None else None, ahead[0].data_ptr() if ahead is not None else None)
+
+        def bc_key(call):
+            return (id(bc_table), bc_table.data_ptr(), int(bc_table.shape[0]), int(sample_seed), int(call), B)
 
         def tiles_of(t):
             return HxBatch(t[0].data_ptr(), t[1].data_ptr() if self.use_bc else None, B, t[4].data_ptr())
 
         want = (env, env.steps_issued, replay, expert, bc_table, n_main, int(sample_seed), float(smooth_sigma), self.sample_calls, n)
-        if self._front_drawn != want:
+        if not _same_draw(self._front_drawn, want):
             _lib.call("hx_sample_batch_guarded", replay.total.data_ptr(), replay.capacity, replay.ring.data_ptr(), expert.ring.data_ptr() if expert is not None else None,
                       len_of(expert), _lib.ptr(bc_table), bc_table.shape[0] if bc_table is not None else 0, B, n_main, 1, int(sample_seed), self.sample_calls,
                       float(smooth_sigma), cur[2].data_ptr(), cur[3].data_ptr() if bc_table is not None else None, cur[4].data_ptr(), cur[0].data_ptr(),
@@ -541,19 +563,38 @@
         carries_c = knob == "1" or (bool(with_c) and knob != "0")
         if carries_c:
             self._front_c_epoch += 1
-        front = HxFront(flags.data_ptr(), status.data_ptr(), self._front_epoch, self._front_c_epoch if carries_c else 0)
+        book, ahead_knob = self._bc_book, bc_ahead.knob()
+        ahead_on = bool(self.front_bc_ahead) if ahead_knob is None else ahead_knob
+        with_bc = self.use_bc and bc_table is not None and bc_table.shape[0] > 0
+        if bc_table is not self._bc_ahead_table:
+            book.reset()
+            self._bc_ahead_table = bc_table
+        abc_ready = book.slot_ready(ahead_on, with_bc, actor_phase, bc_key(self.sample_calls) if with_bc else None)
+        hoist = book.can_hoist(ahead_on, with_bc, actor_phase, bc_key(self.sample_calls + 1) if with_bc else None)
+        self.front_bc_ahead_used = abc_ready if (actor_phase and with_bc) else None
+        front = HxFront(flags.data_ptr(), status.data_ptr(), self._front_epoch, self._front_c_epoch if carries_c else 0,
+                        self._bc_ahead_tiles[0].data_ptr() if hoist else None, int(abc_ready), 0)
         _lib.call("hx_hirl_front", env.state.data_ptr(), n, env.pitch, env.obs.data_ptr(), out.data_ptr(), mode | (32 if (not bf16 and self._x9_for(n, front=True)) else 0),
                   _lib.ptr(act_noise), float(act_sigma), int(act_seed), int(env.env_id0), self.act_calls, env.reward.data_ptr(), env.done.data_ptr(),
                   env.success.data_ptr(), ctypes.byref(env._opts), nets, ctypes.byref(batch), hyper, int(actor_phase), w_kind, ctypes.byref(front), st)
         self._front_enqueued = True
+        if hoist:
+            book.hoisted(bc_key(self.sample_calls + 1))
+        elif actor_phase and with_bc and not abc_ready:
+            book.own_job_ran()
         env.steps_issued += 1
-        nxt_draw, nxt_tiles = draw(nxt, self.sample_calls + 1), tiles_of(nxt)
+        draw_ahead = book.want_draw(ahead_on, with_bc, actor_phase)
+        nxt_draw, nxt_tiles = draw(nxt, self.sample_calls + 1, self._bc_ahead_tiles if draw_ahead else None), tiles_of(nxt)
         if not self.staged:
             _lib.call("hx_hirl_learn_back", nets, ctypes.byref(batch), hyper, self.critic_step, int(actor_phase), self.actor_step, int(do_polyak), w_kind, w_given,
                       float(bc_warm_up_weight), ctypes.byref(nxt_draw), ctypes.byref(nxt_tiles), with_c, st)
         else:
             self._learn_staged(lambda: _lib.call("hx_hirl_critic_grads_back", nets, ctypes.byref(batch), hyper, ctypes.byref(nxt_draw), ctypes.byref(nxt_tiles), with_c, st),
                                batch, actor_phase, do_polyak, w_kind, w_given, bc_warm_up_weight)
+        if draw_ahead:
+            book.drawn(bc_key(self.sample_calls + 2))
+        if actor_phase:
+            book.actor_written()
         self._front_drawn = (env, env.steps_issued, replay, expert, bc_table, n_main, int(sample_seed), float(smooth_sigma), self.sample_calls + 1, n)
         self._front_tiles = [nxt, cur]
         self.rows, self.bc_rows, self._idx, self._idx_bc, self._noise = cur
@@ -582,6 +623,7 @@
             self._front[1].zero_()
         self._front_epoch = self._front_c_epoch = 0
         self._front_drawn = None
+        self._bc_book.reset()
 
     def front_status(self):
         return 0 if self._front is None else int(self._front[1].item())
@@ -596,6 +638,7 @@
     def bc_train_actor(self):
         batch = HxBatch(self.rows.data_ptr(), self.bc_rows.data_ptr(), self.batch, self._noise.data_ptr())
         self.actor_step += 1
+        self._bc_book.actor_written()
         _lib.call("hx_bc_train_actor", ctypes.byref(self.nets), ctypes.byref(batch), ctypes.byref(self.hyper), self.actor_step, _lib.stream_ptr())
 
     def losses_host(self):
diff --git a/hirl4ucav_amd/csrc/hx_core.hip b/hirl4ucav_amd/csrc/hx_core.hip
--- a/hirl4ucav_amd/csrc/hx_core.hip
+++ b/hirl4ucav_amd/csrc/hx_core.hip
@@ -93,4 +93,5 @@
     for (int i = 0; i < 8; ++i) sizes8[i] = v[i];
     return 0;
 }
+int hx_abi_size_front(void) { return (int)sizeof(HxFront); }
 }
diff --git a/hirl4ucav_amd/csrc/hx_hirl.hip b/hirl4ucav_amd/csrc/hx_hirl.hip
--- a/hirl4ucav_amd/csrc/hx_hirl.hip
+++ b/hirl4ucav_amd/csrc/hx_hirl.hip
@@ -65,7 +65,8 @@
     }
     F.images = N->w2_bf16_all;
 }
-static void make_launch_b(const HxNets* N, const HxBatch* Bt, const HxHyper* Hy, int32_t actor_fwd, FwdArgs& F) {
+static void make_launch_b(const HxNets* N, const HxBatch* Bt, const HxHyper* Hy, int32_t actor_fwd, FwdArgs& F, bool abc_ready = false,
+                          const float* ahead_rows = nullptr) {
     const Mlp mA{13, 4, Hy->no_layernorm ? 1 : 0}, mQ{17, 1, Hy->no_layernorm ? 1 : 0};
     const int B = Bt->batch;
     Slot s[S_COUNT];
@@ -81,9 +82,13 @@
     if (actor_fwd && Hy->use_bc) {
         const RowSrc bcsrc{Bt->bc_rows ? Bt->bc_rows : Bt->rows, nullptr, nullptr, 0, 32};
         int n = 2;
-        F.job[n++] = FwdJob{N->actor, mA, bcsrc, 0, 0, Head{}, nullptr, 0.f, s[S_ABC], B, 1, IM_ACTOR};
+        if (!abc_ready) F.job[n++] = FwdJob{N->actor, mA, bcsrc, 0, 0, Head{}, nullptr, 0.f, s[S_ABC], B, 1, IM_ACTOR};
         if (actor_fwd == 2) F.job[n++] = FwdJob{N->bc_actor, mA, src, 0, 0, Head{}, nullptr, 0.f, s[S_BCS], B, 0, IM_BC};
         F.njobs = n;
+    } else if (!actor_fwd && Hy->use_bc && ahead_rows) {
+        const RowSrc bcsrc{ahead_rows, nullptr, nullptr, 0, 32};
+        F.job[2] = FwdJob{N->actor, mA, bcsrc, 0, 0, Head{}, nullptr, 0.f, s[S_ABC], B, 1, IM_ACTOR};
+        F.njobs = 3;
     }
     F.images = N->w2_bf16_all;
 }
@@ -110,7 +115,8 @@
     static const int force = getenv("HX_FRONT_C") ? atoi(getenv("HX_FRONT_C")) : -1;
     return force < 0 ? asked : force != 0;
 }
-static int critic_back(const HxNets* N, const HxBatch* Bt, const HxHyper* Hy, void* stream, int adam_step, bool polyak, const SampleDev* predraw = nullptr, bool skip_c = false) {
+static int critic_back(const HxNets* N, const HxBatch* Bt, const HxHyper* Hy, void* stream, int adam_step, bool polyak, const SampleDev* predraw = nullptr, bool skip_c = false,
+                       int* ahead_idx = nullptr, float* ahead_rows = nullptr) {
     hipStream_t st = (hipStream_t)stream;
     const Mlp mQ{17, 1, Hy->no_layernorm ? 1 : 0};
     const int B = Bt->batch;
@@ -141,6 +147,7 @@
         }
         W.bf16 = N->w2_bf16_all != nullptr;
         W.predraw = predraw; W.predraw_batch = B;
+        W.ahead_idx = predraw ? ahead_idx : nullptr; W.ahead_rows = predraw ? ahead_rows : nullptr;
         if (adam_step > 0) {
             W.ad = make_adam(N, Hy, Hy->lr_critic, adam_step, false);
             launch_wg(W, true, st);
@@ -339,9 +346,13 @@
     HX_REQUIRE(bf16 ? N->actor_w2_bf16 != nullptr : (!N->actor_w2_bf16 && (N->actor_w2_f32i || N->actor_w2_x9)),
                "hx_hirl_front: fp32 networks with HxNets.actor_w2_f32i / actor_w2_x9, or the bf16 update path (w2_bf16_all) with actor_w2_bf16");
     const int actor_fwd = actor_phase ? (w_kind == 1 ? 2 : 1) : 0;
+    HX_REQUIRE(!front->abc_ready || (actor_phase && Hy->use_bc), "hx_hirl_front: HxFront.abc_ready goes with an actor call of an agent with BC");
+    HX_REQUIRE(!front->bc_rows_ahead || (!actor_phase && Hy->use_bc && (reinterpret_cast<uintptr_t>(front->bc_rows_ahead) & 15u) == 0 &&
+                                         front->bc_rows_ahead != Bt->bc_rows && front->bc_rows_ahead != Bt->rows),
+               "hx_hirl_front: HxFront.bc_rows_ahead goes with a critic-only call of an agent with BC, a 16-byte aligned tile of its own");
     FwdArgs FA, FB;
     make_launch_a(N, Bt, Hy, actor_fwd, FA);
-    make_launch_b(N, Bt, Hy, actor_fwd, FB);
+    make_launch_b(N, Bt, Hy, actor_fwd, FB, front->abc_ready != 0, front->bc_rows_ahead);
     const bool x9 = !bf16 && (noise_mode & 32) != 0;
     HX_REQUIRE(bf16 || (x9 ? N->actor_w2_x9 != nullptr : N->actor_w2_f32i != nullptr), "hx_hirl_front: the image of the chosen acting format is missing from HxNets");
     noise_mode &= ~32;
@@ -364,6 +375,11 @@
     if (int rc = prepare_draw(next, Bt->batch, const_cast<float*>(next_tiles->rows), const_cast<float*>(next_tiles->bc_rows), const_cast<float*>(next_tiles->noise),
                               stream, SD, &fused, false)) return rc;
     HX_REQUIRE(fused, "hx_hirl_learn_back: the predraw covers minibatches of at most 256 rows");
+    HX_REQUIRE(!next->idx_bc_ahead == !next->bc_rows_ahead, "hx_hirl_learn_back: HxSample.idx_bc_ahead and bc_rows_ahead go together");
+    if (next->idx_bc_ahead)
+        HX_REQUIRE(next->bc_table && next->bc_len > 0 && next->idx_bc && next_tiles->bc_rows && next->bc_rows_ahead != next_tiles->bc_rows &&
+                       next->bc_rows_ahead != Bt->bc_rows && next->idx_bc_ahead != next->idx_bc && (reinterpret_cast<uintptr_t>(next->bc_rows_ahead) & 15u) == 0,
+                   "hx_hirl_learn_back: the BC draw one call ahead needs a BC table and a 16-byte aligned tile pair of its own");
     return 0;
 }
 int hx_hirl_critic_grads_back(const HxNets* N, const HxBatch* Bt, const HxHyper* Hy, const HxSample* next, const HxBatch* next_tiles, int32_t c_in_front,
@@ -371,7 +387,7 @@
     HX_REQUIRE(N && Bt && Hy && Bt->batch > 0 && Bt->batch % 16 == 0, "hx_hirl_critic_grads_back: batch must be a positive multiple of 16");
     SampleDev SD{};
     if (next) if (int rc = make_predraw(N, Bt, next, next_tiles, stream, &SD)) return rc;
-    return critic_back(N, Bt, Hy, stream, 0, false, next ? &SD : nullptr, front_has_c(c_in_front != 0));
+    return critic_back(N, Bt, Hy, stream, 0, false, next ? &SD : nullptr, front_has_c(c_in_front != 0), next ? next->idx_bc_ahead : nullptr, next ? next->bc_rows_ahead : nullptr);
 }
 int hx_hirl_learn_back(const HxNets* N, const HxBatch* Bt, const HxHyper* Hy, int32_t critic_step, int32_t actor_phase, int32_t actor_step, int32_t do_polyak,
                        int32_t w_kind, float w_given, float warm, const HxSample* next, const HxBatch* next_tiles, int32_t c_in_front, void* stream) {
@@ -379,7 +395,8 @@
     HX_REQUIRE(critic_step >= 1 && (!actor_phase || actor_step >= 1), "hx_hirl_learn_back: Adam steps are 1-based");
     SampleDev SD{};
     if (next) if (int rc = make_predraw(N, Bt, next, next_tiles, stream, &SD)) return rc;
-    int rc = critic_back(N, Bt, Hy, stream, critic_step, do_polyak != 0, next ? &SD : nullptr, front_has_c(c_in_front != 0));
+    int rc = critic_back(N, Bt, Hy, stream, critic_step, do_polyak != 0, next ? &SD : nullptr, front_has_c(c_in_front != 0), next ? next->idx_bc_ahead : nullptr,
+                         next ? next->bc_rows_ahead : nullptr);
     if (rc || !actor_phase) return rc;
     if ((rc = hx_hirl_actor_backward(N, Bt, Hy, w_kind == 1, 1, stream))) return rc;
     return actor_wgrad_impl(N, Hy, Bt->batch, Bt->batch, w_kind, w_given, warm, stream, actor_step, do_polyak != 0);
diff --git a/hirl4ucav_amd/csrc/hx_update.h b/hirl4ucav_amd/csrc/hx_update.h
--- a/hirl4ucav_amd/csrc/hx_update.h
+++ b/hirl4ucav_amd/csrc/hx_update.h
@@ -268,14 +268,15 @@
 constexpr int kFusedSlots = 1024, kFusedBatchMax = 256;
 __device__ __forceinline__ uint32_t fused_hash(uint32_t k) { return (k * 2654435761u) >> 22; }
 
+template <bool BC_ONLY = false>
 __device__ __forceinline__ void draw_fused(const SampleDev& S, int B, uint32_t (*hkey)[kFusedSlots], int (*hown)[kFusedSlots], int (*fin)[kFusedBatchMax]) {
     const int tid = threadIdx.x;
     const int t = tid & 511, stream = tid >> 9;
-    const unsigned long long tot = *S.total;
+    const unsigned long long tot = BC_ONLY ? 0ull : *S.total;
     const DrawMap dm = draw_map(tot, (unsigned long long)S.cap, S.guard);
     const uint32_t len_main = dm.live;
     const uint32_t k0 = (uint32_t)S.seed, k1 = (uint32_t)(S.seed >> 32);
-    const bool live = (stream == 0 || S.idx_bc != nullptr) && t < B;
+    const bool live = (stream == 0 ? !BC_ONLY : S.idx_bc != nullptr) && t < B;
     const bool main_grp = t < S.n_main;
     const uint32_t len = stream == 1 ? S.bc_len : (main_grp ? len_main : S.expert_len);
     const uint32_t grp = (stream == 1 || main_grp) ? 0u : 0x80000000u;
@@ -335,6 +336,19 @@
     }
 }
 
+__device__ __forceinline__ void bc_ahead_wg(const SampleDev& S, int B, int* idx_out, float* rows_out, float* scratch) {
+    auto hkey = reinterpret_cast<uint32_t (*)[kFusedSlots]>(scratch);
+    auto hown = reinterpret_cast<int (*)[kFusedSlots]>(scratch + 2 * kFusedSlots);
+    auto fin = reinterpret_cast<int (*)[kFusedBatchMax]>(scratch + 4 * kFusedSlots);
+    SampleDev A = S;
+    A.call = S.call + 1u;
+    draw_fused<true>(A, B, hkey, hown, fin);
+    const int tid = threadIdx.x;
+    if (tid < B) idx_out[tid] = fin[1][tid];
+    for (int e = tid; e < B * 8; e += kWide)
+        reinterpret_cast<float4*>(rows_out)[e] = reinterpret_cast<const float4*>(S.bc_table + (size_t)fin[1][e >> 3] * 32)[e & 7];
+}
+
 struct FwdJob {
     const float* net;
     Mlp m;
@@ -526,6 +540,7 @@
     float* count_out;
     const SampleDev* predraw;
     int predraw_batch;
+    int* ahead_idx; float* ahead_rows;
 };
 
 #pragma clang fp contract(off)
diff --git a/hirl4ucav_amd/csrc/hx_wgrad.hip b/hirl4ucav_amd/csrc/hx_wgrad.hip
--- a/hirl4ucav_amd/csrc/hx_wgrad.hip
+++ b/hirl4ucav_amd/csrc/hx_wgrad.hip
@@ -25,6 +25,7 @@
     WgJobC job[2];
     int has_pre, pre_batch;
     SampleDev pre;
+    int* ahead_idx; float* ahead_rows;
 };
 
 struct AdamElem {
@@ -120,6 +121,7 @@
         static_assert(sizeof(lds) >= (4 * kFusedSlots + 2 * kFusedBatchMax) * 4, "predraw_wg's tables fit");
         if (AC.has_pre && blockIdx.x >= kWgPerJob) {
             if (blockIdx.x == kWgPerJob && blockIdx.y == 0) predraw_wg(AC.pre, AC.pre_batch, lds);
+            else if (blockIdx.x == kWgPerJob + 1 && blockIdx.y == 0 && AC.ahead_idx) bc_ahead_wg(AC.pre, AC.pre_batch, AC.ahead_idx, AC.ahead_rows, lds);
             return;
         }
     }
@@ -632,7 +634,7 @@
     for (int j = 0; j < W.njobs; ++j) C.job[j] = pack_wg(W.job[j], W);
     const bool pre = W.predraw != nullptr;
     C.has_pre = pre ? 1 : 0;
-    if (pre) { C.pre = *W.predraw; C.pre_batch = W.predraw_batch; }
+    if (pre) { C.pre = *W.predraw; C.pre_batch = W.predraw_batch; C.ahead_idx = W.ahead_idx; C.ahead_rows = W.ahead_idx ? W.ahead_rows : nullptr; }
     const dim3 grid(kWgPerJob + (pre ? 8 : 0), W.njobs);
     const bool relu = W.slope == 0.0f;
 #define HX_WG(ADAM_, RELU_, BF16_) hipLaunchKernelGGL((wgrad_kernel<ADAM_, RELU_, BF16_>), grid, dim3(kWide), 0, st, C)
diff --git a/include/hirl4ucav.h b/include/hirl4ucav.h
--- a/include/hirl4ucav.h
+++ b/include/hirl4ucav.h
@@ -38,9 +38,10 @@
 #define HX_STAT_PITCH 16
 
 const char* hx_last_error(void);
-#define HX_ABI_VERSION 117
+#define HX_ABI_VERSION 118
 int hx_version(void);
 int hx_abi_sizes(int32_t* sizes8);
+int hx_abi_size_front(void);
 void* hx_event_create(void);
 int hx_event_destroy(void* ev);
 int hx_event_elapsed_us(void* start, void* stop, float* us );
@@ -184,6 +185,7 @@
     uint64_t seed; uint32_t call; float sigma;
     int32_t* idx; int32_t* idx_bc;
     uint32_t guard;
+    int32_t* idx_bc_ahead; float* bc_rows_ahead;
 } HxSample;
 int hx_hirl_critic_grads_sampled(const HxNets* nets, const HxBatch* batch, const HxHyper* hyper, const HxSample* sample, int32_t actor_fwd,
                                  void* stream);
@@ -195,6 +197,9 @@
     uint32_t* status;
     uint32_t epoch;
     uint32_t with_c;
+    const float* bc_rows_ahead;
+    uint32_t abc_ready;
+    uint32_t pad_;
 } HxFront;
 int hx_hirl_front(float* state, int64_t n, int64_t stride, float* obs_io, float* actions, int32_t noise_mode,
                   const float* noise, float sigma, uint64_t seed, uint32_t row0, uint32_t call, float* reward, uint8_t* done, int8_t* success,
```
